# aniketntnu/WordDiffusion

Hardware: AMD Instinct MI355X
Metric: denoised 64x256 word images/sec (1000-step DDPM), whole job (higher is better)
Workload: dtype bf16x3; 1 GPU; BASELINE configs[1]: batch 64 per GPU of 64x256 crops = [64,4,8,32] latents, 1000-step DDPM (999 executed steps), base unet.py UNetModel (320 ch, mult (1,1), 4 heads, 339 writers), random-init synthetic weights; variant=base, batch_per_gpu=64, noise_steps=1000, executed_steps_per_image=999, precision=split-bf16 MFMA x3, fp32 accumulate (<=1e-4 of the fp32 reference), output_finite=True

## Files before the change

include/wdiff_hip.h:

```cpp
#ifndef WDIFF_HIP_H
#define WDIFF_HIP_H

#include <stdint.h>

#ifdef __cplusplus
extern "C" {
#endif

#define WD_OK 0
#define WD_EINVAL (-1)
#define WD_ELAUNCH (-2)
#define WD_ESTATE (-3)

#define WD_ACT_NONE 0
#define WD_ACT_SILU 1
#define WD_ACT_GEGLU 2

typedef uint16_t wd_bf16;

#define WD_MAX_KSPLIT 64

typedef struct wd_src {
    const wd_bf16* hi;
    const wd_bf16* lo;
    const int32_t* gather;
    int32_t ld;
    int32_t c;
    int32_t ntaps;
    int32_t hw_src;
} wd_src;

typedef struct wd_gemm_args {
    wd_src src[2];
    int32_t nsrc;
    int32_t npass;
    const wd_bf16* w_hi;
    const wd_bf16* w_lo;
    int32_t m, n, ktot;
    int32_t hw_out;
    const float* bias;
    const float* rowvec;
    int32_t rowvec_ld;
    const float* resid;
    int32_t resid_ld;
    const int64_t* resid_rows;
    int32_t act;
    float* out_f32;
    int32_t out_ld;
    wd_bf16* out_hi;
    wd_bf16* out_lo;
    int32_t out_pl_ld;
    int32_t tile;
    int32_t w_layout;
    int32_t slab_rows;
    int32_t ksplit;
    float* ws;
    int64_t ws_floats;
    double* stat_part;
    int32_t stat_cpg;
    int32_t dbg;
    int32_t* tickets;
    int32_t ntickets;
    const float* gn_gamma;
    const float* gn_beta;
    float gn_eps;
    int32_t gn_silu;
    int32_t gn_cpg;
    const float* a32;
    int32_t a32_ld;
    const double* a32_part;
    int32_t a32_nchunk;
    int32_t a32_pcpg;
    int32_t a32_cpg;
    const float* a32_gamma;
    const float* a32_beta;
    float a32_eps;
    int32_t a32_silu;
    const float* ln_gamma;
    const float* ln_beta;
    float ln_eps;
    int32_t w_ngroups;
    int64_t w_group_stride;
} wd_gemm_args;

int wd_gemm(const wd_gemm_args* args, void* stream);

int wd_gemm_check(const wd_gemm_args* args, wd_gemm_args* out);
const char* wd_gemm_check_kernel(const wd_gemm_args* args);

int wd_gemm_pack_w(const wd_bf16* hi, const wd_bf16* lo, int n, int ktot, wd_bf16* out_hi, wd_bf16* out_lo, void* stream);

typedef struct wd_ff_args {
    const wd_bf16* x_hi;
    const wd_bf16* x_lo;
    int32_t x_ld;
    int32_t m, c, inner;
    const wd_bf16* w1_hi;
    const wd_bf16* w1_lo;
    const float* b1;
    const wd_bf16* w2_hi;
    const wd_bf16* w2_lo;
    const float* b2;
    const float* resid;
    int32_t resid_ld;
    float* out_f32;
    int32_t out_ld;
    wd_bf16* out_hi;
    wd_bf16* out_lo;
    int32_t out_pl_ld;
    const wd_bf16* w3_hi;
    const wd_bf16* w3_lo;
    const float* b3;
    const float* resid3;
    int32_t resid3_ld;
    double* stat_part;
    int32_t stat_cpg;
    int32_t hw_out;
    int32_t npass;
    const float* x_in;
    int32_t x_in_ld;
    int32_t hw;
    const double* gn_part;
    int32_t gn_nchunk, gn_pcpg, gn_cpg;
    float gn_eps;
    const float* gn_gamma;
    const float* gn_beta;
    const wd_bf16* pi_hi;
    const wd_bf16* pi_lo;
    const float* pi_b;
    const float* ln2_gamma;
    const float* ln2_beta;
    const wd_bf16* mq_a;
    const wd_bf16* mot_a;
    const float* xb_a;
    const wd_bf16* mq_b;
    const wd_bf16* mot_b;
    const float* xb_b;
    const float* ln3_gamma;
    const float* ln3_beta;
    float ln_eps;
    int32_t heads, L;
    float* tok2;
} wd_ff_args;
int wd_ff_fused(const wd_ff_args* args, void* stream);
int wd_ff_supported(int c, int inner);
int wd_ff_args_bytes(void);

int wd_gemm_auto_ksplit(int m, int n, int ktot, int64_t ws_floats);
int wd_gemm_args_bytes(void);
int wd_gemm_experimental(void);

int wd_gn_nchunk(int hw);
int wd_gn_stats(const float* x, int ld, int batch, int hw, int c, int cpg, double* part, void* stream);
int wd_gn_fold_chunks(const double* part, int batch, int nchunk, int ngroups, double* out, void* stream);

int wd_gn_apply(const float* x, int ld, int batch, int hw, int c, int cpg, const double* part, int nchunk, int part_cpg,
                const float* gamma, const float* beta, float eps, int silu,
                wd_bf16* out_hi, wd_bf16* out_lo, int out_ld, int c_off,
                wd_bf16* raw_hi, wd_bf16* raw_lo, void* stream);

int wd_gn_apply2(const float* xa, int lda, int ca, const double* part_a, int nchunk_a, int part_cpg_a, int c_off_a,
                 const float* xb, int ldb, int cb, const double* part_b, int nchunk_b, int part_cpg_b, int c_off_b,
                 int batch, int hw, int cpg, const float* gamma, const float* beta, float eps, int silu,
                 wd_bf16* out_hi, wd_bf16* out_lo, int out_ld, wd_bf16* raw_hi, wd_bf16* raw_lo, const int32_t* perm_a, void* stream);

int wd_gn_conv3x3_few_supported(int c, int w, int oc);
int wd_gn_conv3x3_few(const float* x, int ld, int batch, int h, int w, int c, int cpg, const double* part, int nchunk, int part_cpg,
                      const float* gamma, const float* beta, float eps, int silu, const float* weight, const float* bias, int oc,
                      float* out, void* stream);

int wd_layernorm(const float* x, int ld, int rows, int c, const float* gamma, const float* beta, float eps,
                 wd_bf16* out_hi, wd_bf16* out_lo, int out_ld, void* stream);

int wd_split(const float* x, int ld, int rows, int c, int silu, wd_bf16* out_hi, wd_bf16* out_lo, int out_ld,
             void* stream);

int wd_attention(const float* q, int ldq, const float* k, int ldk, const float* v, int ldv,
                 int batch, int heads, int nq, int nk, int d, float scale,
                 float* out_f32, wd_bf16* out_hi, wd_bf16* out_lo, int out_ld, int out_rows, int out_row0,
                 void* stream);

int64_t wd_attention_packed_elems(int batch, int heads, int nk, int d);
int wd_attention_pack_kv(const float* k, int ldk, const float* v, int ldv, int batch, int heads, int nk, int d,
                         wd_bf16* img, void* stream);
int wd_attention_packed(const float* q, int ldq, const wd_bf16* img, int batch, int heads, int nq, int nk, int d,
                        float scale, float* out_f32, wd_bf16* out_hi, wd_bf16* out_lo, int out_ld, int out_rows,
                        int out_row0, void* stream);

int wd_timestep_embedding(const int64_t* t, int batch, const float* freqs, int half,
                          wd_bf16* out_hi, wd_bf16* out_lo, int out_ld, void* stream);

int wd_xattn_supported(int c, int heads, int L);
int wd_xattn_fold(const float* k, int ldk, const float* v, int ldv, int batch, int heads, int L, int d, float scale,
                  const float* wq, const float* wo, int c, float* mq, float* mo, wd_bf16* mq_pl, wd_bf16* mot_pl, void* stream);
int wd_xattn_fused(const float* x, int ld, int batch, int hw, int c, const float* gamma, const float* beta, float eps,
                   const float* mq, const float* mo, int heads, int L, const float* bias, float* out, int out_ld,
                   const float* gamma2, const float* beta2, float eps2, wd_bf16* n_hi, wd_bf16* n_lo, int n_ld,
                   const wd_bf16* mq_pl, const wd_bf16* mot_pl, void* stream);

int wd_emb_combine(const float* time, const float* label, const int64_t* y, int num_classes, int T, int B, int ted,
                   wd_bf16* out_hi, wd_bf16* out_lo, int out_ld, void* stream);
int wd_select_rows(const float* table, const int32_t* t_dev, int batch, int64_t row_floats, int chunk, float* out,
                   void* stream);

int wd_emb_combine_mix(const float* time, const float* label, const int32_t* pairs, const float* mix, int num_classes, int T, int B,
                       int ted, wd_bf16* out_hi, wd_bf16* out_lo, int out_ld, void* stream);
int wd_label_mix(const float* label, const int32_t* pairs, const float* mix, int num_classes, int B, int ted, float* out,
                 void* stream);

int wd_xattn_pair(const float* x, int ld, int batch, int hw, int c, float eps, int heads, int L, const float* gamma_a,
                  const float* beta_a, const wd_bf16* mq_pl_a, const wd_bf16* mot_pl_a, const float* bias_a, const float* gamma_b,
                  const float* beta_b, const wd_bf16* mq_pl_b, const wd_bf16* mot_pl_b, const float* bias_b, float* out, int out_ld,
                  const float* gamma2, const float* beta2, float eps2, wd_bf16* n_hi, wd_bf16* n_lo, int n_ld, void* stream);

int wd_embed_tokens(const void* ids, int ids_are_i64, int rows, int seq_len, const float* table, int vocab, int c,
                    const float* pe, wd_bf16* out_hi, wd_bf16* out_lo, int out_ld, void* stream);

int wd_im2col3x3(const float* x, int batch, int cin, int h, int w, wd_bf16* out_hi, wd_bf16* out_lo, int kpad,
                 void* stream);

int wd_conv3x3_in_supported(int cin, int h, int w, int cout);
int wd_conv3x3_in_nchunk(int hw);
int wd_conv3x3_in(const float* x, int batch, int cin, int h, int w, const float* weight, const float* bias, int cout, float* out,
                  int ld, double* part, int stat_cpg, void* stream);

int wd_nchw_to_tokens(const float* x, int batch, int c, int hw, float* out, int ld, void* stream);
int wd_tokens_to_nchw(const float* x, int ld, int batch, int c, int hw, float* out, void* stream);

int wd_ddpm_step(float* x, const float* eps, int batch, int n_per_sample, const float* ca, const float* cb,
                 const float* cs, const int32_t* t_dev, const float* noise, uint64_t seed, uint64_t sample_offset,
                 void* stream);

int wd_ddpm_step_cfg(float* x, const float* first, const float* second, float scale, float* eps_out, int batch, int n_per_sample,
                     const float* ca, const float* cb, const float* cs, const int32_t* t_dev, const float* noise, uint64_t seed,
                     uint64_t sample_offset, void* stream);

int wd_advance_timestep(int32_t* t_dev, int delta, int64_t* t64, int batch, void* stream);

int wd_ddim_step(float* x, const float* eps, const float* second, float scale, float* eps_out, int batch, int n_per_sample,
                 const float* c1, const float* c2, const float* c3, const float* c4, const float* c5, const int32_t* k_dev,
                 const int32_t* t_dev, const float* noise, uint64_t seed, uint64_t sample_offset, void* stream);

int wd_next_timestep(int32_t* k_dev, const int32_t* tau, int S, int32_t* t_dev, int64_t* t64, int batch, void* stream);

int wd_randn(float* out, int batch, int n_per_sample, uint64_t seed, uint64_t sample_offset, uint32_t stream_id,
             void* stream);

#define WD_VAE_MAX_LATENT 8
#define WD_STREAM_VAE_POSTERIOR 3
#define WD_STREAM_DROPOUT0 0x100
int wd_vae_posterior(const float* moments_tok, int ld, const float* w, const float* bias, int batch, int L, int hw, float* mean,
                     float* logvar, float* sample, float scale, const float* noise, uint64_t seed, uint64_t sample_offset,
                     void* stream);

int wd_posterior_sample(const float* mean, const float* logvar, int batch, int n_per_sample, float* sample, float scale,
                        const float* noise, uint64_t seed, uint64_t sample_offset, void* stream);

int wd_noise_images(const float* x, const float* eps, const int64_t* t, const float* sqrt_ah, const float* sqrt_1m_ah,
                    int batch, int n_per_sample, float* out, void* stream);

int wd_copy2d(void* dst, int64_t dst_pitch, const void* src, int64_t src_pitch, int64_t width_bytes, int64_t rows,
              void* stream);

int wd_ema_update(float* ema, const float* p, int64_t n, double beta, void* stream);

int wd_adamw_table_entry_bytes(void);
int wd_adamw_chunk(void);
int wd_adamw_multi(const void* table, int ntensor, int64_t total_chunks, double lr, double beta1, double beta2, double eps,
                   double weight_decay, int64_t step, int ema_mode, double ema_beta, void* stream);

int wd_repack_entry_bytes(void);
int wd_repack_tile(void);
int wd_repack_vchunk(void);
int wd_repack_multi(const void* table, int nentries, int64_t total_chunks, void* stream);

int wd_mse_loss(const float* pred, const float* target, int64_t n, float* grad, float* loss, double* scratch,
                int scratch_len, void* stream);


int wd_transpose_planes(const void* in_hi, const void* in_lo, int in_is_f32, int ld, int c, const int32_t* gather, int ntaps,
                        int hw_out, int hw_src, int m, int mpad, int tap_minor, wd_bf16* out_hi, wd_bf16* out_lo,
                        void* stream);

typedef struct wd_dw_item {
    const wd_bf16* d_hi;
    const wd_bf16* d_lo;
    const wd_bf16* x_hi;
    const wd_bf16* x_lo;
    float* grad;
    int32_t d_ld, x_ld, grad_ld, accumulate;
} wd_dw_item;
typedef struct wd_dw_args {
    const wd_bf16* d_hi;
    const wd_bf16* d_lo;
    const wd_bf16* x_hi;
    const wd_bf16* x_lo;
    const int32_t* gather;
    float* grad;
    float* ws;
    int64_t ws_floats;
    int32_t d_ld, x_ld, grad_ld;
    int32_t ntaps, hw_out, hw_src;
    int32_t m, n, c;
    int32_t npass;
    int32_t accumulate;
    int32_t nslice;
    int32_t dbg;
    int32_t reserved;
    void* stamps;
    const wd_dw_item* items;
    int32_t nitems;
    int32_t reserved2;
} wd_dw_args;
int wd_dw(const wd_dw_args* a, void* stream);
int wd_dw_group(const wd_dw_args* a, const wd_dw_item* items_host, const wd_dw_item* items_dev, int nitems, void* stream);
int wd_dw_group_slices(int m, int n, int c, int ntaps, int nitems);
int wd_dw_item_bytes(void);
int wd_dw_supported(int m, int n, int c, int ntaps, int hw_out);
int wd_dw_slices(int m, int n, int c, int ntaps);
int wd_dw_args_bytes(void);

int wd_colsum(const float* x, int ld, int rows, int c, int seg, float* out, int out_ld, int accumulate, float scale,
              float* scratch, int64_t scratch_floats, void* stream);

int wd_gn_bwd_nchunk(int hw);
int wd_gn_bwd_stats(const float* x, int ld, const float* dz, int dz_ld, int dz_off, int batch, int hw, int c, int cpg,
                    const double* part, int nchunk_f, int part_cpg, const float* gamma, const float* beta, int c_off, float eps,
                    int silu, float* sums, void* stream);
int wd_gn_bwd_apply(const float* x, int ld, const float* dz, int dz_ld, int dz_off, int batch, int hw, int c, int cpg,
                    const double* part, int nchunk_f, int part_cpg, const float* gamma, const float* beta, int c_off, float eps,
                    int silu, const float* sums, float* dx, int dx_ld, int accumulate, void* stream);

int wd_gn_bwd_fused_supported(int hw, int c, int cpg);
int wd_gn_bwd_fused(const float* x, int ld, const float* dz, int dz_ld, int dz_off, int batch, int hw, int c, int cpg,
                    const double* part, int nchunk_f, int part_cpg, const float* gamma, const float* beta, int c_off, float eps,
                    int silu, float* sums, float* dx, int dx_ld, int accumulate, void* stream);

typedef struct {
    uint64_t seed;
    uint64_t row_base;
    const uint64_t* row_base_dev;
    uint32_t tag, thr;
    float scale;
} wd_dropout;
int wd_gn_apply_dropout(const float* x, int ld, int batch, int hw, int c, int cpg, const double* part, int nchunk, int part_cpg,
                        const float* gamma, const float* beta, float eps, int silu,
                        wd_bf16* out_hi, wd_bf16* out_lo, int out_ld, int c_off,
                        wd_bf16* raw_hi, wd_bf16* raw_lo, const wd_dropout* d, void* stream);
int wd_gn_bwd_stats_dropout(const float* x, int ld, const float* dz, int dz_ld, int dz_off, int batch, int hw, int c, int cpg,
                            const double* part, int nchunk_f, int part_cpg, const float* gamma, const float* beta, int c_off, float eps,
                            int silu, float* sums, const wd_dropout* d, void* stream);
int wd_gn_bwd_apply_dropout(const float* x, int ld, const float* dz, int dz_ld, int dz_off, int batch, int hw, int c, int cpg,
                            const double* part, int nchunk_f, int part_cpg, const float* gamma, const float* beta, int c_off, float eps,
                            int silu, const float* sums, float* dx, int dx_ld, int accumulate, const wd_dropout* d, void* stream);
int wd_gn_bwd_fused_dropout(const float* x, int ld, const float* dz, int dz_ld, int dz_off, int batch, int hw, int c, int cpg,
                            const double* part, int nchunk_f, int part_cpg, const float* gamma, const float* beta, int c_off, float eps,
                            int silu, float* sums, float* dx, int dx_ld, int accumulate, const wd_dropout* d, void* stream);

int wd_layernorm_bwd_nblk(int rows);
int wd_layernorm_bwd(const float* x, int ld, const float* dy, int dy_ld, int rows, int c, const float* gamma, float eps,
                     float* dx, int dx_ld, int accumulate, float* colpart, void* stream);

int wd_attention_bwd_small_nwg(int heads, int nq, int nk, int d);
int wd_attention_bwd_small(const float* q, int ldq, const float* k, int ldk, const float* v, int ldv, const float* dout,
                           int ldo, int batch, int heads, int nq, int nk, int d, float scale, float* dq, int lddq,
                           float* dkv_part, int* nwg_out, void* stream);

int wd_dout_prep_rows(void);
int wd_dout_prep(const float* d, int ld, int m, int n, int npad, int mpad, wd_bf16* pl_hi, wd_bf16* pl_lo, wd_bf16* t_hi,
                 wd_bf16* t_lo, float* colpart, void* stream);
int wd_dout_prep_geglu(const float* u, int u_ld, const float* dh, int dh_ld, int m, int inner, int mpad, wd_bf16* pl_hi, wd_bf16* pl_lo,
                       wd_bf16* t_hi, wd_bf16* t_lo, float* colpart, void* stream);
int wd_colsum_finish(const float* part, int nblk, int c, int nseg, float* out, int out_ld, int accumulate, float scale,
                     void* stream);
int wd_colsum_entry_bytes(void);
int wd_colsum_finish_multi(const void* table, int n, int max_c, void* stream);

int64_t wd_attention_bwd_scratch_floats(int batch, int heads, int nq, int nk);
int wd_attention_bwd(const float* q, int ldq, const float* k, int ldk, const float* v, int ldv, const float* dout, int ldo,
                     int batch, int heads, int nq, int nk, int d, float scale, float* dq, int lddq, float* dk, int lddk,
                     float* dv, int lddv, float* scratch, int64_t scratch_floats, void* stream);

int wd_add(float* dst, const float* src, int64_t n, void* stream);

int wd_permute_dw(const float* packed, int ld, int n, int c, int ntaps, float* out, void* stream);
// ... 27 lines not shown
```

worddiffusion_amd/_native.py:

```python
from __future__ import annotations

import ctypes as C
import os
import re

_HERE = os.path.dirname(os.path.abspath(__file__))
LIB_PATH = os.environ.get("WDIFF_LIB") or os.path.join(_HERE, "libwdiff_hip.so")
HEADER_PATH = os.path.join(os.path.dirname(_HERE), "include", "wdiff_hip.h")

WD_OK, WD_EINVAL, WD_ELAUNCH, WD_ESTATE = 0, -1, -2, -3
ACT_NONE, ACT_SILU, ACT_GEGLU = 0, 1, 2
VAE_MAX_LATENT, STREAM_VAE_POSTERIOR = 8, 3
NCLASS = 13
CLASS_NAMES = ("gemm", "gn_stats", "gn_apply", "layernorm", "attention", "other", "gemm_other_tiles", "gemm_splitk_reduce",
               "gemm_two_per_cu", "gemm_weights_to_registers", "feed_forward_fused", "weight_gradient", "gemm_small_maps_whole_k")

_vp = C.c_void_p
_i = C.c_int
_f = C.c_float
_u64 = C.c_uint64


class WdSrc(C.Structure):
    _fields_ = [("hi", _vp), ("lo", _vp), ("gather", _vp), ("ld", C.c_int32), ("c", C.c_int32),
                ("ntaps", C.c_int32), ("hw_src", C.c_int32)]


class WdGemmArgs(C.Structure):
    _fields_ = [("src", WdSrc * 2), ("nsrc", C.c_int32), ("npass", C.c_int32), ("w_hi", _vp), ("w_lo", _vp),
                ("m", C.c_int32), ("n", C.c_int32), ("ktot", C.c_int32), ("hw_out", C.c_int32),
                ("bias", _vp), ("rowvec", _vp), ("rowvec_ld", C.c_int32), ("resid", _vp), ("resid_ld", C.c_int32),
                ("resid_rows", _vp), ("act", C.c_int32), ("out_f32", _vp), ("out_ld", C.c_int32),
                ("out_hi", _vp), ("out_lo", _vp), ("out_pl_ld", C.c_int32), ("tile", C.c_int32),
                ("w_layout", C.c_int32), ("slab_rows", C.c_int32), ("ksplit", C.c_int32), ("ws", _vp),
                ("ws_floats", C.c_int64), ("stat_part", _vp), ("stat_cpg", C.c_int32), ("dbg", C.c_int32),
                ("tickets", _vp), ("ntickets", C.c_int32), ("gn_gamma", _vp), ("gn_beta", _vp), ("gn_eps", C.c_float),
                ("gn_silu", C.c_int32), ("gn_cpg", C.c_int32), ("a32", _vp), ("a32_ld", C.c_int32), ("a32_part", _vp),
                ("a32_nchunk", C.c_int32), ("a32_pcpg", C.c_int32), ("a32_cpg", C.c_int32), ("a32_gamma", _vp), ("a32_beta", _vp),
                ("a32_eps", C.c_float), ("a32_silu", C.c_int32), ("ln_gamma", _vp), ("ln_beta", _vp), ("ln_eps", C.c_float),
                ("w_ngroups", C.c_int32), ("w_group_stride", C.c_int64)]


class WdFfArgs(C.Structure):
    _fields_ = [("x_hi", _vp), ("x_lo", _vp), ("x_ld", C.c_int32), ("m", C.c_int32), ("c", C.c_int32), ("inner", C.c_int32),
                ("w1_hi", _vp), ("w1_lo", _vp), ("b1", _vp), ("w2_hi", _vp), ("w2_lo", _vp), ("b2", _vp), ("resid", _vp),
                ("resid_ld", C.c_int32), ("out_f32", _vp), ("out_ld", C.c_int32), ("out_hi", _vp), ("out_lo", _vp),
                ("out_pl_ld", C.c_int32), ("w3_hi", _vp), ("w3_lo", _vp), ("b3", _vp), ("resid3", _vp), ("resid3_ld", C.c_int32),
                ("stat_part", _vp), ("stat_cpg", C.c_int32), ("hw_out", C.c_int32), ("npass", C.c_int32),
                ("x_in", _vp), ("x_in_ld", C.c_int32), ("hw", C.c_int32), ("gn_part", _vp), ("gn_nchunk", C.c_int32),
                ("gn_pcpg", C.c_int32), ("gn_cpg", C.c_int32), ("gn_eps", C.c_float), ("gn_gamma", _vp), ("gn_beta", _vp),
                ("pi_hi", _vp), ("pi_lo", _vp), ("pi_b", _vp), ("ln2_gamma", _vp), ("ln2_beta", _vp), ("mq_a", _vp), ("mot_a", _vp),
                ("xb_a", _vp), ("mq_b", _vp), ("mot_b", _vp), ("xb_b", _vp), ("ln3_gamma", _vp), ("ln3_beta", _vp),
                ("ln_eps", C.c_float), ("heads", C.c_int32), ("L", C.c_int32), ("tok2", _vp)]


class WdDwArgs(C.Structure):
    _fields_ = [("d_hi", _vp), ("d_lo", _vp), ("x_hi", _vp), ("x_lo", _vp), ("gather", _vp), ("grad", _vp), ("ws", _vp),
                ("ws_floats", C.c_int64), ("d_ld", C.c_int32), ("x_ld", C.c_int32), ("grad_ld", C.c_int32), ("ntaps", C.c_int32),
                ("hw_out", C.c_int32), ("hw_src", C.c_int32), ("m", C.c_int32), ("n", C.c_int32), ("c", C.c_int32),
                ("npass", C.c_int32), ("accumulate", C.c_int32), ("nslice", C.c_int32), ("dbg", C.c_int32), ("reserved", C.c_int32),
                ("stamps", _vp), ("items", _vp), ("nitems", C.c_int32), ("reserved2", C.c_int32)]


class WdDwItem(C.Structure):
    _fields_ = [("d_hi", _vp), ("d_lo", _vp), ("x_hi", _vp), ("x_lo", _vp), ("grad", _vp), ("d_ld", C.c_int32), ("x_ld", C.c_int32),
                ("grad_ld", C.c_int32), ("accumulate", C.c_int32)]


_SIGS = {
    "wd_gemm": (_i, [C.POINTER(WdGemmArgs), _vp]),
    "wd_gemm_check": (_i, [C.POINTER(WdGemmArgs), C.POINTER(WdGemmArgs)]),
    "wd_gemm_check_kernel": (C.c_char_p, [C.POINTER(WdGemmArgs)]),
    "wd_dw": (_i, [C.POINTER(WdDwArgs), _vp]),
    "wd_dw_supported": (_i, [_i, _i, _i, _i, _i]),
    "wd_dw_slices": (_i, [_i, _i, _i, _i]),
    "wd_dw_args_bytes": (_i, []),
    "wd_dw_group": (_i, [C.POINTER(WdDwArgs), _vp, _vp, _i, _vp]),
    "wd_dw_group_slices": (_i, [_i, _i, _i, _i, _i]),
    "wd_dw_item_bytes": (_i, []),
    "wd_gemm_auto_ksplit": (_i, [_i, _i, _i, C.c_int64]),
    "wd_gemm_pack_w": (_i, [_vp, _vp, _i, _i, _vp, _vp, _vp]),
    "wd_ff_fused": (_i, [C.POINTER(WdFfArgs), _vp]),
    "wd_ff_supported": (_i, [_i, _i]),
    "wd_ff_args_bytes": (_i, []),
    "wd_gemm_args_bytes": (_i, []),
    "wd_gemm_experimental": (_i, []),
    "wd_gn_nchunk": (_i, [_i]),
    "wd_gn_stats": (_i, [_vp, _i, _i, _i, _i, _i, _vp, _vp]),
    "wd_gn_fold_chunks": (_i, [_vp, _i, _i, _i, _vp, _vp]),
    "wd_gn_conv3x3_few_supported": (_i, [_i, _i, _i]),
    "wd_gn_conv3x3_few": (_i, [_vp, _i, _i, _i, _i, _i, _i, _vp, _i, _i, _vp, _vp, _f, _i, _vp, _vp, _i, _vp, _vp]),
    "wd_gn_apply": (_i, [_vp, _i, _i, _i, _i, _i, _vp, _i, _i, _vp, _vp, _f, _i, _vp, _vp, _i, _i, _vp, _vp, _vp]),
    "wd_gn_apply_dropout": (_i, [_vp, _i, _i, _i, _i, _i, _vp, _i, _i, _vp, _vp, _f, _i, _vp, _vp, _i, _i, _vp, _vp, _vp, _vp]),
    "wd_gn_apply2": (_i, [_vp, _i, _i, _vp, _i, _i, _i, _vp, _i, _i, _vp, _i, _i, _i, _i, _i, _i, _vp, _vp, _f, _i, _vp, _vp, _i, _vp,
                          _vp, _vp, _vp]),
    "wd_layernorm": (_i, [_vp, _i, _i, _i, _vp, _vp, _f, _vp, _vp, _i, _vp]),
    "wd_split": (_i, [_vp, _i, _i, _i, _i, _vp, _vp, _i, _vp]),
    "wd_attention": (_i, [_vp, _i, _vp, _i, _vp, _i, _i, _i, _i, _i, _i, _f, _vp, _vp, _vp, _i, _i, _i, _vp]),
    "wd_attention_packed_elems": (C.c_int64, [_i, _i, _i, _i]),
    "wd_attention_pack_kv": (_i, [_vp, _i, _vp, _i, _i, _i, _i, _i, _vp, _vp]),
    "wd_attention_packed": (_i, [_vp, _i, _vp, _i, _i, _i, _i, _i, _f, _vp, _vp, _vp, _i, _i, _i, _vp]),
    "wd_timestep_embedding": (_i, [_vp, _i, _vp, _i, _vp, _vp, _i, _vp]),
    "wd_embed_tokens": (_i, [_vp, _i, _i, _i, _vp, _i, _i, _vp, _vp, _vp, _i, _vp]),
    "wd_im2col3x3": (_i, [_vp, _i, _i, _i, _i, _vp, _vp, _i, _vp]),
    "wd_conv3x3_in_supported": (_i, [_i, _i, _i, _i]),
    "wd_conv3x3_in_nchunk": (_i, [_i]),
    "wd_conv3x3_in": (_i, [_vp, _i, _i, _i, _i, _vp, _vp, _i, _vp, _i, _vp, _i, _vp]),
    "wd_nchw_to_tokens": (_i, [_vp, _i, _i, _i, _vp, _i, _vp]),
    "wd_tokens_to_nchw": (_i, [_vp, _i, _i, _i, _i, _vp, _vp]),
    "wd_ddpm_step": (_i, [_vp, _vp, _i, _i, _vp, _vp, _vp, _vp, _vp, _u64, _u64, _vp]),
    "wd_advance_timestep": (_i, [_vp, _i, _vp, _i, _vp]),
    "wd_randn": (_i, [_vp, _i, _i, _u64, _u64, C.c_uint32, _vp]),
    "wd_vae_posterior": (_i, [_vp, _i, _vp, _vp, _i, _i, _i, _vp, _vp, _vp, _f, _vp, _u64, _u64, _vp]),
    "wd_posterior_sample": (_i, [_vp, _vp, _i, _i, _vp, _f, _vp, _u64, _u64, _vp]),
    "wd_noise_images": (_i, [_vp, _vp, _vp, _vp, _vp, _i, _i, _vp, _vp]),
    "wd_copy2d": (_i, [_vp, C.c_int64, _vp, C.c_int64, C.c_int64, C.c_int64, _vp]),
    "wd_ema_update": (_i, [_vp, _vp, C.c_int64, C.c_double, _vp]),
    "wd_adamw_table_entry_bytes": (_i, []),
    "wd_adamw_chunk": (_i, []),
    "wd_adamw_multi": (_i, [_vp, _i, C.c_int64, C.c_double, C.c_double, C.c_double, C.c_double, C.c_double, C.c_int64, _i,
                           C.c_double, _vp]),
    "wd_mse_loss": (_i, [_vp, _vp, C.c_int64, _vp, _vp, _vp, _i, _vp]),
    "wd_transpose_planes": (_i, [_vp, _vp, _i, _i, _i, _vp, _i, _i, _i, _i, _i, _i, _vp, _vp, _vp]),
    "wd_repack_entry_bytes": (_i, []),
    "wd_repack_tile": (_i, []),
    "wd_repack_vchunk": (_i, []),
    "wd_repack_multi": (_i, [_vp, _i, C.c_int64, _vp]),
    "wd_attention_bwd_scratch_floats": (C.c_int64, [_i, _i, _i, _i]),
    "wd_attention_bwd": (_i, [_vp, _i, _vp, _i, _vp, _i, _vp, _i, _i, _i, _i, _i, _i, _f, _vp, _i, _vp, _i, _vp, _i, _vp, C.c_int64, _vp]),
    "wd_xattn_supported": (_i, [_i, _i, _i]),
    "wd_xattn_fold": (_i, [_vp, _i, _vp, _i, _i, _i, _i, _i, _f, _vp, _vp, _i, _vp, _vp, _vp, _vp, _vp]),
    "wd_xattn_fused": (_i, [_vp, _i, _i, _i, _i, _vp, _vp, _f, _vp, _vp, _i, _i, _vp, _vp, _i, _vp, _vp, _f, _vp, _vp, _i, _vp, _vp, _vp]),
    "wd_dout_prep_rows": (_i, []),
    "wd_dout_prep": (_i, [_vp, _i, _i, _i, _i, _i, _vp, _vp, _vp, _vp, _vp, _vp]),
    "wd_dout_prep_geglu": (_i, [_vp, _i, _vp, _i, _i, _i, _i, _vp, _vp, _vp, _vp, _vp, _vp]),
    "wd_colsum_finish": (_i, [_vp, _i, _i, _i, _vp, _i, _i, _f, _vp]),
    "wd_colsum_entry_bytes": (_i, []),
    "wd_colsum_finish_multi": (_i, [_vp, _i, _i, _vp]),
    "wd_emb_combine": (_i, [_vp, _vp, _vp, _i, _i, _i, _i, _vp, _vp, _i, _vp]),
    "wd_select_rows": (_i, [_vp, _vp, _i, C.c_int64, _i, _vp, _vp]),
    "wd_emb_combine_mix": (_i, [_vp, _vp, _vp, _vp, _i, _i, _i, _i, _vp, _vp, _i, _vp]),
    "wd_label_mix": (_i, [_vp, _vp, _vp, _i, _i, _i, _vp, _vp]),
    "wd_ddpm_step_cfg": (_i, [_vp, _vp, _vp, _f, _vp, _i, _i, _vp, _vp, _vp, _vp, _vp, _u64, _u64, _vp]),
    "wd_ddim_step": (_i, [_vp, _vp, _vp, _f, _vp, _i, _i, _vp, _vp, _vp, _vp, _vp, _vp, _vp, _vp, _u64, _u64, _vp]),
    "wd_next_timestep": (_i, [_vp, _vp, _i, _vp, _vp, _i, _vp]),
    "wd_xattn_pair": (_i, [_vp, _i, _i, _i, _i, _f, _i, _i, _vp, _vp, _vp, _vp, _vp, _vp, _vp, _vp, _vp, _vp, _vp, _i, _vp, _vp, _f,
                           _vp, _vp, _i, _vp]),
    "wd_add": (_i, [_vp, _vp, C.c_int64, _vp]),
    "wd_permute_dw": (_i, [_vp, _i, _i, _i, _i, _vp, _vp]),
    "wd_colsum": (_i, [_vp, _i, _i, _i, _i, _vp, _i, _i, _f, _vp, C.c_int64, _vp]),
    "wd_gn_bwd_nchunk": (_i, [_i]),
    "wd_gn_bwd_stats": (_i, [_vp, _i, _vp, _i, _i, _i, _i, _i, _i, _vp, _i, _i, _vp, _vp, _i, _f, _i, _vp, _vp]),
    "wd_gn_bwd_apply": (_i, [_vp, _i, _vp, _i, _i, _i, _i, _i, _i, _vp, _i, _i, _vp, _vp, _i, _f, _i, _vp, _vp, _i, _i, _vp]),
    "wd_gn_bwd_fused_supported": (_i, [_i, _i, _i]),
    "wd_gn_bwd_fused": (_i, [_vp, _i, _vp, _i, _i, _i, _i, _i, _i, _vp, _i, _i, _vp, _vp, _i, _f, _i, _vp, _vp, _i, _i, _vp]),
    "wd_gn_bwd_stats_dropout": (_i, [_vp, _i, _vp, _i, _i, _i, _i, _i, _i, _vp, _i, _i, _vp, _vp, _i, _f, _i, _vp, _vp, _vp]),
    "wd_gn_bwd_apply_dropout": (_i, [_vp, _i, _vp, _i, _i, _i, _i, _i, _i, _vp, _i, _i, _vp, _vp, _i, _f, _i, _vp, _vp, _i, _i, _vp, _vp]),
    "wd_gn_bwd_fused_dropout": (_i, [_vp, _i, _vp, _i, _i, _i, _i, _i, _i, _vp, _i, _i, _vp, _vp, _i, _f, _i, _vp, _vp, _i, _i, _vp, _vp]),
    "wd_layernorm_bwd_nblk": (_i, [_i]),
    "wd_layernorm_bwd": (_i, [_vp, _i, _vp, _i, _i, _i, _vp, _f, _vp, _i, _i, _vp, _vp]),
    "wd_attention_bwd_small_nwg": (_i, [_i, _i, _i, _i]),
    "wd_attention_bwd_small": (_i, [_vp, _i, _vp, _i, _vp, _i, _vp, _i, _i, _i, _i, _i, _i, _f, _vp, _i, _vp,
                                   C.POINTER(_i), _vp]),
    "wd_geglu_fwd": (_i, [_vp, _i, C.c_int64, _i, _vp, _vp, _i, _vp]),
    "wd_geglu_bwd": (_i, [_vp, _i, _vp, _i, C.c_int64, _i, _vp, _i, _vp]),
    "wd_silu_bwd": (_i, [_vp, _vp, C.c_int64, _vp, _vp]),
    "wd_pool2x2_sum": (_i, [_vp, _i, _i, _i, _i, _vp, _vp]),
    "wd_embedding_bwd": (_i, [_vp, _i, _i, _vp, _i, _i, _i, _vp, _i, _vp]),
    "wd_graph_begin": (_i, [_vp]),
    "wd_graph_end": (_i, [_vp, C.POINTER(_vp)]),
    "wd_graph_launch": (_i, [_vp, _vp]),
    "wd_graph_destroy": (_i, [_vp]),
    "wd_prof_enable": (_i, [_i]),
    "wd_prof_collect": (_i, [C.POINTER(C.c_double), C.POINTER(C.c_int64), C.POINTER(C.c_double)]),
    "wd_prof_collect_flops": (_i, [C.POINTER(C.c_double), C.POINTER(C.c_int64), C.POINTER(C.c_double)]),
    "wd_version": (C.c_char_p, []),
    "wd_device_info": (_i, [C.POINTER(_i), C.POINTER(_i), C.c_char_p, _i]),
}


def header_symbols() -> list:
    txt = open(HEADER_PATH).read()
    txt = re.sub(r"/\*.*?\*/", "", txt, flags=re.S)
    return sorted(set(re.findall(r"\b(wd_[a-z0-9_]+)\s*\(", txt)))


class NativeError(RuntimeError):
    pass


_lib = None


def lib() -> C.CDLL:
    global _lib
    if _lib is not None:
        return _lib
    if not os.path.exists(LIB_PATH):
        raise NativeError(f"{LIB_PATH} is missing: build it with `python -m worddiffusion_amd.build` "
                          "(hipcc --offload-arch=gfx950); worddiffusion_amd has no CPU/eager fallback")
    l = C.CDLL(LIB_PATH)
    for name, (res, args) in _SIGS.items():
        fn = getattr(l, name)
        fn.restype = res
        fn.argtypes = args
    if l.wd_gemm_args_bytes() != C.sizeof(WdGemmArgs):
        raise NativeError(f"{LIB_PATH}: wd_gemm_args is {l.wd_gemm_args_bytes()} bytes in the library, {C.sizeof(WdGemmArgs)} in "
                          "worddiffusion_amd/_native.py - rebuild with `python -m worddiffusion_amd.build`")
    if l.wd_ff_args_bytes() != C.sizeof(WdFfArgs):
        raise NativeError(f"{LIB_PATH}: wd_ff_args is {l.wd_ff_args_bytes()} bytes in the library, {C.sizeof(WdFfArgs)} in "
                          "worddiffusion_amd/_native.py - rebuild with `python -m worddiffusion_amd.build`")
    if l.wd_dw_item_bytes() != C.sizeof(WdDwItem):
        raise NativeError(f"{LIB_PATH}: wd_dw_item is {l.wd_dw_item_bytes()} bytes in the library, {C.sizeof(WdDwItem)} in "
                          "worddiffusion_amd/_native.py - rebuild with `python -m worddiffusion_amd.build`")
    if l.wd_dw_args_bytes() != C.sizeof(WdDwArgs):
        raise NativeError(f"{LIB_PATH}: wd_dw_args is {l.wd_dw_args_bytes()} bytes in the library, {C.sizeof(WdDwArgs)} in "
                          "worddiffusion_amd/_native.py - rebuild with `python -m worddiffusion_amd.build`")
    _lib = l
    return l


_ERR = {WD_EINVAL: "invalid argument", WD_ELAUNCH: "HIP launch/runtime error", WD_ESTATE: "bad call order"}


def check(rc: int, what: str) -> None:
    if rc != WD_OK:
        raise NativeError(f"{what} failed: {_ERR.get(rc, rc)}")
```

worddiffusion_amd/csrc/wd_gemm.hip:

```cpp
#include <stdlib.h>

#include "wd_common.h"
#include "wd_gemm_epi.h"
#include "wd_gemm_priv.h"


namespace {

constexpr int BK = 32;

__device__ __forceinline__ int lds_off(int row, int ch) { return row * 64 + ((ch ^ ((row >> 2) & 3)) << 4); }
__device__ __forceinline__ int lds_off16(int row, int ch) { return row * 64 + ((ch ^ ((0 - (row >> 2)) & 3)) << 4); }


template <int BM, int BN, int TN, int NT>
__device__ __forceinline__ void wd_epilogue_lds(const wd_gemm_args& a, const f32x16 (&acc)[TN], char* smem, const int m0,
                                                const int n0, const int wm, const int wn, const int wcols, const int kh,
                                                const int nkh, const int tid, const int sidx = 0) {
    constexpr int LDE = BN + 4;
    float* ep = reinterpret_cast<float*>(smem);
    const int lane = tid & 63;
    const int frow = lane & 31, fhalf = lane >> 5;
    asm volatile("s_waitcnt vmcnt(0)" ::: "memory");
    __syncthreads();
// ... 1739 lines not shown
    const int r0w = (cw >> 1) * 32, c0w = (cw & 1) * 80;

    if (wave >= 8) {
        const int L = wave - 8;
        const int lrow = lane >> 2, lpos = lane & 3;
        const int sw = (lpos ^ ((0 - (lane >> 4)) & 3)) * 8;
        auto make_srd = [](const wd_bf16* p) {
            return __builtin_amdgcn_make_buffer_rsrc(const_cast<wd_bf16*>(p), 0, 0x7FFFFFF0, 0x00020000);
        };
        const int x_piece = NPL == 2 ? 8 + (L >> 1) : 8 + (L & 1), x_plane = NPL == 2 ? (L & 1) : 0;
        uint32_t b_voff[3];
        {
            const int pcs[3] = {L, L + 4, x_piece};
#pragma unroll
            for (int i = 0; i < 3; ++i) {
                const int n = n0 + pcs[i] * 16 + lrow;
                b_voff[i] = n < a.n ? (uint32_t)(((long)n * a.ktot + sw) * 2) : WD_OOB;
            }
        }
        const __amdgpu_buffer_rsrc_t srd_w_hi = make_srd(a.w_hi), srd_w_lo = make_srd(a.w_lo ? a.w_lo : a.w_hi);
        const __amdgpu_buffer_rsrc_t srd_w_x = (x_plane ? srd_w_lo : srd_w_hi);
        int s = 0, tap = 0, kc = 0;
        int cur_ld = a.src[0].ld, cur_cpt = a.src[0].c / BKS, cur_nt = a.src[0].ntaps;
        const wd_bf16* cur_hi = a.src[0].hi;
        const wd_bf16* cur_lo = a.src[0].lo;
        {
            const int cpt = a.src[0].c / BKS, n0st = a.src[0].ntaps * cpt;
            if (k_begin < n0st) {
                tap = k_begin / cpt;
                kc = k_begin - tap * cpt;
            } else {
                s = 1;
                kc = k_begin - n0st;
                cur_hi = a.src[1].hi;
                cur_lo = a.src[1].lo;
                cur_ld = a.src[1].ld;
                cur_cpt = a.src[1].c / BKS;
                cur_nt = a.src[1].ntaps;
            }
        }
        __amdgpu_buffer_rsrc_t srd_a_hi = make_srd(cur_hi), srd_a_lo = make_srd(cur_lo ? cur_lo : cur_hi);
        uint32_t a_voff[2];
        auto locate = [&]() {
#pragma unroll
            for (int i = 0; i < 2; ++i) {
                const int row = (2 * L + i) * 16 + lrow;
                int r;
                if (s == 0) r = s_tab[tap * BM + row];
                else r = (m0 + row < a.m) ? m0 + row : -1;
                a_voff[i] = r >= 0 ? (uint32_t)r * (uint32_t)(cur_ld * 2) + (uint32_t)(sw * 2) : WD_OOB;
            }
        };
        locate();
        int soff_a = kc * BKS * 2, soff_b = k_begin * BKS * 2;
        int wr_off = 0;
        auto issue_stage = [&]() {
            char* sbase = smem + wr_off;
#pragma unroll
            for (int i = 0; i < 2; ++i) {
                __builtin_amdgcn_raw_ptr_buffer_load_lds(srd_a_hi, (wd_lds_ptr)(sbase + (2 * L + i) * 1024), 16, a_voff[i], soff_a, 0, 0);
                if (NPL == 2)
                    __builtin_amdgcn_raw_ptr_buffer_load_lds(srd_a_lo, (wd_lds_ptr)(sbase + A_PL + (2 * L + i) * 1024), 16, a_voff[i],
                                                             soff_a, 0, 0);
            }
#pragma unroll
            for (int i = 0; i < 2; ++i) {
                __builtin_amdgcn_raw_ptr_buffer_load_lds(srd_w_hi, (wd_lds_ptr)(sbase + NPL * A_PL + (L + 4 * i) * 1024), 16, b_voff[i],
                                                         soff_b, 0, 0);
                if (NPL == 2)
                    __builtin_amdgcn_raw_ptr_buffer_load_lds(srd_w_lo, (wd_lds_ptr)(sbase + NPL * A_PL + B_PL + (L + 4 * i) * 1024), 16,
                                                             b_voff[i], soff_b, 0, 0);
            }
            __builtin_amdgcn_raw_ptr_buffer_load_lds(srd_w_x, (wd_lds_ptr)(sbase + NPL * A_PL + x_plane * B_PL + x_piece * 1024), 16,
                                                     b_voff[2], soff_b, 0, 0);
            soff_b += BKS * 2;
            soff_a += BKS * 2;
            wr_off += STAGE;
            if (wr_off == RING) wr_off = 0;
            ++kc;
            if (kc == cur_cpt) {
                kc = 0;
                soff_a = 0;
                ++tap;
                if (tap == cur_nt) {
                    tap = 0;
                    ++s;
                    if (s < a.nsrc) {
                        cur_hi = a.src[1].hi;
                        cur_lo = a.src[1].lo;
                        cur_ld = a.src[1].ld;
                        cur_cpt = a.src[1].c / BKS;
                        cur_nt = a.src[1].ntaps;
                        srd_a_hi = make_srd(cur_hi);
                        srd_a_lo = make_srd(cur_lo ? cur_lo : cur_hi);
                    }
                }
                if (s < a.nsrc) locate();
            }
        };
        auto wait_keep1 = [&]() {
            if (NPL == 2) asm volatile("s_waitcnt vmcnt(9)" ::: "memory");
            else asm volatile("s_waitcnt vmcnt(5)" ::: "memory");
        };
        __builtin_amdgcn_s_setprio(2);
        int issued = 0;
        for (; issued < 3 && issued < nk; ++issued) issue_stage();
        if (nk > 0) {
            if (issued >= 2) {
                if (issued == 3) {
                    if (NPL == 2) asm volatile("s_waitcnt vmcnt(18)" ::: "memory");
                    else asm volatile("s_waitcnt vmcnt(10)" ::: "memory");
                } else {
                    wait_keep1();
                }
            } else {
                asm volatile("s_waitcnt vmcnt(0)" ::: "memory");
            }
            __builtin_amdgcn_s_barrier();
        }
        int kit = 0;
        for (; kit + 3 < nk; ++kit) {
            wait_keep1();
            __builtin_amdgcn_s_barrier();
            issue_stage();
        }
        for (; kit < nk; ++kit) {
            if (kit + 1 < nk) {
                if (kit + 2 < nk) wait_keep1();
                else asm volatile("s_waitcnt vmcnt(0)" ::: "memory");
            }
            __builtin_amdgcn_s_barrier();
        }
    } else {
        const int ao0 = lds_off16(r0w + l15, lq), bo0 = NPL * A_PL + lds_off16(c0w + l15, lq);
        bf16x8 fa0[2][NPL], fb0[5][NPL], fa1[2][NPL], fb1[5][NPL];
        auto read_a = [&](auto& fa_, const char* base, int i) {
#pragma unroll
            for (int p = 0; p < NPL; ++p) fa_[i][p] = *reinterpret_cast<const bf16x8*>(base + ao0 + p * A_PL + i * 1024);
        };
        auto read_b = [&](auto& fb_, const char* base, int t) {
#pragma unroll
            for (int p = 0; p < NPL; ++p) fb_[t][p] = *reinterpret_cast<const bf16x8*>(base + bo0 + p * B_PL + t * 1024);
        };
        auto mfma_pass = [&](auto& fa_, auto& fb_, int pass, int g) {
            const int i = g / 5, t = g % 5;
            if (NPL == 2) {
                if (pass == 0) acc[i][t] = __builtin_amdgcn_mfma_f32_16x16x32_bf16(fa_[i][NPL - 1], fb_[t][0], acc[i][t], 0, 0, 0);
                else if (pass == 1) acc[i][t] = __builtin_amdgcn_mfma_f32_16x16x32_bf16(fa_[i][0], fb_[t][NPL - 1], acc[i][t], 0, 0, 0);
                else acc[i][t] = __builtin_amdgcn_mfma_f32_16x16x32_bf16(fa_[i][0], fb_[t][0], acc[i][t], 0, 0, 0);
            } else {
                if (pass == 2) acc[i][t] = __builtin_amdgcn_mfma_f32_16x16x32_bf16(fa_[i][0], fb_[t][0], acc[i][t], 0, 0, 0);
            }
        };
        if (nk > 0) {
            __builtin_amdgcn_s_barrier();
#pragma unroll
            for (int i = 0; i < 2; ++i) read_a(fa0, smem, i);
#pragma unroll
            for (int t = 0; t < 5; ++t) read_b(fb0, smem, t);
        }
        int rd_off = STAGE;
        auto step = [&](bool have1, auto& ma, auto& mb, auto& ra, auto& rb) {
            __builtin_amdgcn_s_barrier();
            const char* nb = smem + rd_off;
#pragma unroll
            for (int pass = (NPL == 2 ? 0 : 2); pass < 3; ++pass) {
#pragma unroll
                for (int g = 0; g < 10; ++g) {
                    if (have1 && pass == (NPL == 2 ? 0 : 2)) {
                        if (g < 2) read_a(ra, nb, g);
                        else if (g < 7) read_b(rb, nb, g - 2);
                    }
                    mfma_pass(ma, mb, pass, g);
                }
                __builtin_amdgcn_sched_barrier(0);
            }
            rd_off += STAGE;
            if (rd_off == RING) rd_off = 0;
        };
        for (int kit = 0; kit < nk; kit += 2) {
            step(kit + 1 < nk, fa0, fb0, fa1, fb1);
            if (kit + 1 < nk) step(kit + 2 < nk, fa1, fb1, fa0, fb0);
        }
    }

    constexpr int LDE = BN + 4;
    float* ep = reinterpret_cast<float*>(smem);
    asm volatile("s_waitcnt vmcnt(0)" ::: "memory");
    __syncthreads();
    if (wave < 8) {
#pragma unroll
        for (int i = 0; i < 2; ++i)
#pragma unroll
            for (int t = 0; t < 5; ++t)
#pragma unroll
                for (int r = 0; r < 4; ++r) ep[(r0w + i * 16 + 4 * lq + r) * LDE + c0w + t * 16 + l15] = acc[i][t][r];
    }
    __syncthreads();
    wd_epilogue_tail<BM, BN, 768>(a, ep, m0, n0, tid, sidx);
#endif
}

template <int NPASS>
int launch8(const wd_gemm_args& a, hipStream_t st) {
    constexpr int NPL = (NPASS == 1) ? 1 : 2;
    constexpr int loop_smem = 4 * NPL * (128 + 160) * 64 + 9 * 128 * 4;
    constexpr int red_smem = 128 * (160 + 4) * 4 + WD_STAT_SCRATCH;
    constexpr int smem = loop_smem > red_smem ? loop_smem : red_smem;
    static_assert(smem <= 160 * 1024, "LDS budget");
    static bool attr_done = false;
    if (!attr_done) {
        if (hipFuncSetAttribute(reinterpret_cast<const void*>(&wd_gemm8_kernel<NPASS>), hipFuncAttributeMaxDynamicSharedMemorySize,
                                smem) != hipSuccess)
            return WD_ELAUNCH;
        attr_done = true;
    }
    const int nbn = (a.n + 159) / 160, nbm = (a.m + 127) / 128;
    {
        WdLaunchScope scope(WD_CLS_GEMM, st, 2.0 * (double)a.m * (double)a.n * (double)a.ktot);
        hipLaunchKernelGGL((wd_gemm8_kernel<NPASS>), dim3(nbn * nbm * a.ksplit), dim3(768), smem, st, a, nbn, nbm);
    }
    if (a.ksplit > 1) return launch_reduce_any<128, 160>(a, st);
    return wd_check_launch();
}

#endif

}

int wd_gemm_launch_reduce(const wd_gemm_args& a, hipStream_t st, int bm) {
    if (bm == 64) {
        if (reduce_flat_ok(a)) return launch_reduce_any<64, 64>(a, st);
        const int cpg = a.stat_part ? a.stat_cpg : 1;
        if (40 % cpg == 0 && a.n % 40 == 0) return launch_reduce<64, 40>(a, st);
        if (32 % cpg == 0 && a.n % 32 == 0) return launch_reduce<64, 32>(a, st);
        return launch_reduce<64, 64>(a, st);
    }
    return launch_reduce_any<128, 160>(a, st);
}

static int wd_auto_ksplit(const int tile, const int m, const int n, const int nk64, const long ws_floats) {
    const int bn = tile % 1000, bm = tile / 1000;
    const long tiles = (long)((m + bm - 1) / bm) * ((n + bn - 1) / bn);
    if (!((tiles < 128 || (tiles == 128 && nk64 >= 32)) && nk64 >= 8)) return 1;
    long sp = 256 / tiles;
    if (sp > nk64 / 4) sp = nk64 / 4;
    static const long cap_env = getenv("WDIFF_KSPLIT_CAP") ? atol(getenv("WDIFF_KSPLIT_CAP")) : WD_MAX_KSPLIT;
    const long cap = nk64 >= 64 ? cap_env : 8;
    if (sp > cap) sp = cap;
    while (sp > 1 && sp * m * n > ws_floats) --sp;
    return sp > 1 ? (int)sp : 1;
}

static int wd_auto_tile(const int m, const int n, const int nk64, const bool can_split_base, const long ws_floats) {
    int tile = (n % 160 == 0) ? 128160 : 128064;
    const long tiles = (long)((m + 127) / 128) * ((n + (tile % 1000) - 1) / (tile % 1000));
    const bool can_split = can_split_base && nk64 >= 8 && (long)2 * m * n <= ws_floats;
    if (tiles < 128 && !can_split && m > 64) tile = 64064;
    return tile;
}

extern "C" int wd_gemm_experimental(void) {
#ifdef WDIFF_EXPERIMENTAL
    return 1;
#else
    return 0;
#endif
}

extern "C" int wd_gemm_args_bytes(void) { return (int)sizeof(wd_gemm_args); }

extern "C" int wd_gemm_auto_ksplit(int m, int n, int ktot, int64_t ws_floats) {
    if (m <= 0 || n <= 0 || ktot <= 0 || ktot % BK2 || ws_floats <= 0) return 1;
    const int nk64 = ktot / BK2;
    return wd_auto_ksplit(wd_auto_tile(m, n, nk64, true, (long)ws_floats), m, n, nk64, (long)ws_floats);
}

namespace {
enum WdKernel {
    K_GEMMQ,
    K_GEMMW,
    K_V4,
    K_M16,
    K_V2,
    K_V1,
    K_SLAB,
    K_CONV3,
    K_V8,
    K_PP,
};

struct WdResolved {
    wd_gemm_args a;
    WdKernel kernel;
    int ks;
};
}

static int wd_gemm_resolve(const wd_gemm_args& in, WdResolved& r) {
    wd_gemm_args a = in;
    static const int ks_env = getenv("WDIFF_GEMM_KS") ? atoi(getenv("WDIFF_GEMM_KS")) : 2;
    r.ks = ks_env == 1 ? 1 : 2;
    if (a.ksplit < 0 || a.ksplit > WD_MAX_KSPLIT) return WD_EINVAL;
    if (a.w_layout == 3) {
        if (a.n % 80 || a.act == WD_ACT_GEGLU || (a.tile && a.tile != 64320 && a.tile != 128160 && a.tile != 64080) || a.ktot % 64)
            return WD_EINVAL;
        if (a.tile == 0) a.tile = (a.a32 || a.ln_gamma) ? 64320 : 128160;
        if (a.n % (a.tile % 1000)) return WD_EINVAL;
        if (a.tile == 64080) a.ksplit = 1;
    }
    if (a.w_ngroups > 1) {
        if (a.w_layout != 3 || a.tile != 64320 || a.ksplit > 1 || a.hw_out % (64 * a.w_ngroups) || a.w_group_stride <= 0 || (a.w_group_stride & 7))
            return WD_EINVAL;
        a.ksplit = 1;
    }
    if (a.stat_part) {
        if (a.stat_cpg <= 0 || a.n % a.stat_cpg || a.act == WD_ACT_GEGLU) return WD_EINVAL;
        const int bn = (a.tile ? a.tile % 1000 : (a.n % 160 == 0 ? 160 : 64));
        const int bm = (a.tile ? a.tile / 1000 : 128);
        if (!((a.hw_out % bm == 0) || (bm % a.hw_out == 0 && bm / a.hw_out <= WD_STAT_MAXNS))) return WD_EINVAL;
        if ((bm != 128 && a.w_layout != 3) || bn % a.stat_cpg) return WD_EINVAL;
        if (!wd_epilogue_vec_ok(a)) return WD_EINVAL;
        if (a.tile == 0) a.tile = bm * 1000 + bn;
    }
    if (a.ksplit > 1 && (!a.ws || a.act == WD_ACT_GEGLU || a.w_layout == 1)) return WD_EINVAL;
    if (a.ln_gamma) {
        if (a.w_layout != 3 || (a.tile && a.tile != 64320) || a.n != 320 || a.ksplit > 1 || !a.ln_beta || !a.out_hi || (a.out_pl_ld & 3) ||
            ((reinterpret_cast<uintptr_t>(a.ln_gamma) | reinterpret_cast<uintptr_t>(a.ln_beta)) & 15) ||
            ((reinterpret_cast<uintptr_t>(a.out_hi) | reinterpret_cast<uintptr_t>(a.out_lo)) & 7) || a.act == WD_ACT_GEGLU)
            return WD_EINVAL;
        a.tile = 64320;
        a.ksplit = 1;
    }
    if (a.gn_gamma) {
        if (!a.gn_beta || !a.stat_part || !a.out_hi || (!a.ws && a.tile != 64080) || a.hw_out != 64 || a.m % 64 || a.n % 160 || a.gn_cpg <= 0 ||
            40 % a.gn_cpg || a.stat_cpg <= 0 || a.gn_cpg % a.stat_cpg || a.act != WD_ACT_NONE || a.resid_rows || a.w_layout == 1)
            return WD_EINVAL;
        if (!wd_epilogue_vec_ok(a) ||
            ((reinterpret_cast<uintptr_t>(a.ws) | reinterpret_cast<uintptr_t>(a.gn_gamma) | reinterpret_cast<uintptr_t>(a.gn_beta)) & 15))
            return WD_EINVAL;
        a.tickets = nullptr;
    }
    if (a.w_layout == 1) {
        a.ksplit = 1;
        a.tickets = nullptr;
    }
    if (a.nsrc < 1 || a.nsrc > 2 || (a.npass != 1 && a.npass != 3)) return WD_EINVAL;
    if (a.m <= 0 || a.n <= 0 || a.hw_out <= 0 || !a.w_hi || (a.npass == 3 && !a.w_lo)) return WD_EINVAL;
    if (!a.out_f32 && !a.out_hi) return WD_EINVAL;
    long k = 0;
    for (int s = 0; s < a.nsrc; ++s) {
        const wd_src& q = a.src[s];
        if (s == 0 && a.a32) {
            if (a.w_layout != 3 || a.npass != 3 || (a.tile && a.tile != 64320) || a.n % 320 || a.hw_out % 64 || !a.a32_part || !a.a32_gamma ||
                !a.a32_beta || a.a32_nchunk <= 0 || a.a32_pcpg <= 0 || a.a32_cpg <= 0 || a.a32_cpg % a.a32_pcpg || q.c % a.a32_cpg ||
                q.c > 1024 || a.a32_ld < q.c || (a.a32_ld & 3) || (reinterpret_cast<uintptr_t>(a.a32) & 15) || q.hw_src <= 0)
                return WD_EINVAL;
        } else if (!q.hi || (a.npass == 3 && !q.lo)) return WD_EINVAL;
        if (q.c <= 0 || q.c % BK || q.ld % 8 || q.ntaps < 1) return WD_EINVAL;
        if (!q.gather && q.ntaps != 1) return WD_EINVAL;
        if (q.gather && q.hw_src <= 0) return WD_EINVAL;
        k += (long)q.ntaps * q.c;
    }
    if (k != a.ktot) return WD_EINVAL;
    {
        const long lim = 0x7FFFFFF0L;
        if ((long)a.n * a.ktot * 2 >= lim) return WD_EINVAL;
        for (int s = 0; s < a.nsrc; ++s) {
            const wd_src& q = a.src[s];
            const long rows = q.gather ? (long)((a.m + a.hw_out - 1) / a.hw_out) * q.hw_src : (long)a.m;
            if ((s == 0 && a.a32) ? rows * a.a32_ld * 4 >= lim : rows * q.ld * 2 >= lim) return WD_EINVAL;
        }
    }
    if (a.act == WD_ACT_GEGLU && (a.n % 64 || a.tile == 0)) return WD_EINVAL;
    if (a.rowvec && a.rowvec_ld <= 0) return WD_EINVAL;
    if (a.resid && a.resid_ld <= 0) return WD_EINVAL;
    {
        const int nout = a.act == WD_ACT_GEGLU ? a.n / 2 : a.n;
        if ((a.out_f32 && a.out_ld < nout) || (a.out_hi && a.out_pl_ld < nout) || (a.resid && a.resid_ld < nout) ||
            (a.rowvec && a.rowvec_ld < nout))
            return WD_EINVAL;
        for (int s = 0; s < a.nsrc; ++s)
            if (!(s == 0 && a.a32) && a.src[s].ld < a.src[s].c) return WD_EINVAL;
    }

    if (a.w_layout == 3) {
        bool ok = a.src[0].ntaps <= 9 && (a.nsrc == 1 || (a.src[1].gather == nullptr && a.src[1].ntaps == 1));
        for (int s = 0; s < a.nsrc; ++s) ok = ok && (a.src[s].c % 64 == 0);
        if (!ok) return WD_EINVAL;
        const wd_src& q0 = a.src[0];
        const bool same3 = q0.ntaps == 9 && q0.gather && a.slab_rows > 0 && q0.hw_src == a.hw_out && a.hw_out % a.slab_rows == 0;
        const bool down3 = a.tile == 64080 && q0.ntaps == 9 && q0.gather && a.slab_rows > 0 && q0.hw_src == 4 * a.hw_out;
        if (!same3 && !down3) a.slab_rows = 0;
        a.tickets = nullptr;
        if (a.tile == 64080) {
            if (!wd_gemmq_applies(a)) return WD_EINVAL;
            if (a.gn_gamma && (40 % a.gn_cpg || 80 % a.gn_cpg)) return WD_EINVAL;
            r.a = a, r.kernel = K_GEMMQ;
            return WD_OK;
        }
        const int nk64 = a.ktot / 64;
        if (a.ksplit == 0) a.ksplit = a.ws ? wd_auto_ksplit(a.tile, a.m, a.n, nk64, a.ws_floats) : 1;
        if (a.ksplit > 1 && (nk64 < a.ksplit || (long)a.ksplit * a.m * a.n > a.ws_floats)) a.ksplit = 1;
        if (a.gn_gamma && a.ksplit <= 1) return WD_EINVAL;
        r.a = a, r.kernel = K_GEMMW;
        return WD_OK;
    }
#ifndef WDIFF_EXPERIMENTAL
    if (a.w_layout == 1) return WD_EINVAL;
#else
    if (a.w_layout == 1) {
        if (a.src[0].ntaps > 9 || a.slab_rows <= 0) return WD_EINVAL;
        if (a.nsrc == 2 && (a.src[1].gather || a.src[1].ntaps != 1)) return WD_EINVAL;
        if (a.tile == 0) a.tile = (a.act == WD_ACT_GEGLU || a.n % 160) ? 128064 : 128160;
        if (a.act == WD_ACT_GEGLU && a.n % (a.tile % 1000)) return WD_EINVAL;
        if (a.slab_rows > 192) return WD_EINVAL;
        if (a.tile != 128064 && a.tile != 128128 && a.tile != 128160) return WD_EINVAL;
        r.a = a, r.kernel = K_SLAB;
        return WD_OK;
    }
#endif
    bool conv3 = false;
    if (a.w_layout == 2) {
        const wd_src& q0 = a.src[0];
        static const int conv3_mode = getenv("WDIFF_CONV3") ? atoi(getenv("WDIFF_CONV3")) : 0;
#ifdef WDIFF_EXPERIMENTAL
        const bool conv3_env = conv3_mode != 0 || (a.dbg & 0x1000);
#else
        const bool conv3_env = false;
        (void)conv3_mode;
#endif
        const bool same3 = q0.ntaps == 9 && q0.gather && a.slab_rows > 0 && q0.hw_src == a.hw_out && a.hw_out % a.slab_rows == 0;
        conv3 = conv3_env && same3 && q0.c % 64 == 0 && a.act != WD_ACT_GEGLU && (a.tile == 0 || a.tile == 128160) &&
                (a.nsrc == 1 || (!a.src[1].gather && a.src[1].ntaps == 1 && a.src[1].c % 64 == 0));
        if (conv3) a.tile = 128160;
        a.w_layout = 0;
        static const bool arith_env = getenv("WDIFF_GEMM_ARITH_TAB") ? atoi(getenv("WDIFF_GEMM_ARITH_TAB")) != 0 : true;
        if (!same3 || !arith_env) a.slab_rows = 0;
    } else if (a.w_layout == 0) {
        a.slab_rows = 0;
    } else if (a.w_layout != 0) {
        return WD_EINVAL;
    }
    bool v2ok = (a.ktot % BK2 == 0) && !getenv("WDIFF_GEMM_V1");
    for (int s = 0; s < a.nsrc; ++s) v2ok = v2ok && (a.src[s].c % BK2 == 0);
    v2ok = v2ok && a.src[0].ntaps <= 9 && (a.nsrc == 1 || (a.src[1].gather == nullptr && a.src[1].ntaps == 1));
    const int nk64 = a.ktot / BK2;
    int tile = a.tile;
    if (tile == 0)
        tile = wd_auto_tile(a.m, a.n, nk64, v2ok && a.ws && a.ksplit == 0 && a.act != WD_ACT_GEGLU, a.ws_floats);
    if (a.ksplit == 0) {
        a.ksplit = (v2ok && a.ws && a.act != WD_ACT_GEGLU) ? wd_auto_ksplit(tile, a.m, a.n, nk64, a.ws_floats) : 1;
    }
    if (a.act == WD_ACT_GEGLU && a.n % (tile % 1000)) return WD_EINVAL;
    if (a.ksplit > 1 && (!v2ok || nk64 < a.ksplit || (long)a.ksplit * a.m * a.n > a.ws_floats)) a.ksplit = 1;
    bool use_v4 = false;
    if (tile == 128160) {
        static const int v4_env = getenv("WDIFF_GEMM_V4") ? atoi(getenv("WDIFF_GEMM_V4")) : 2;
        const long wgs = (long)((a.m + 127) / 128) * ((a.n + 159) / 160) * a.ksplit;
        use_v4 = v2ok && !a.stat_part && (v4_env == 1 || (v4_env == 2 && wgs >= 512) || (a.dbg & 0x400));
    }
    {
        static const bool fuse_env = getenv("WDIFF_GEMM_FUSE_COMBINE") ? atoi(getenv("WDIFF_GEMM_FUSE_COMBINE")) != 0 : false;
        const int bn = tile % 1000, bm = tile / 1000;
        const long ntile = (long)((a.m + bm - 1) / bm) * ((a.n + bn - 1) / bn);
        const bool aligned = (a.n & 3) == 0 && a.n % bn == 0 && wd_epilogue_vec_ok(a) && (reinterpret_cast<uintptr_t>(a.ws) & 15) == 0;
        if (!((fuse_env || (a.dbg & 0x2000)) && a.tickets && a.ksplit > 1 && v2ok && !use_v4 && !conv3 && aligned && ntile <= a.ntickets))
            a.tickets = nullptr;
    }
    if (a.gn_gamma && !(a.ksplit > 1 && tile == 128160 && v2ok && !use_v4 && !conv3)) return WD_EINVAL;
    static const int stagger_min = getenv("WDIFF_GEMM_STAGGER_MIN") ? atoi(getenv("WDIFF_GEMM_STAGGER_MIN")) : 10;
    static const bool stagger = getenv("WDIFF_GEMM_STAGGER") ? atoi(getenv("WDIFF_GEMM_STAGGER")) != 0 : true;
    static const bool m16 = getenv("WDIFF_GEMM_M16") ? atoi(getenv("WDIFF_GEMM_M16")) != 0 : true;
    static const bool pp = getenv("WDIFF_GEMM_PP") ? atoi(getenv("WDIFF_GEMM_PP")) != 0 : false;
    a.tile = tile;
#ifdef WDIFF_EXPERIMENTAL
    if (conv3 && v2ok) return r.a = a, r.kernel = K_CONV3, WD_OK;
#endif
    if (tile != 128064 && tile != 128160 && tile != 128128 && tile != 64064) return WD_EINVAL;
    if (tile == 128160) {
        if (use_v4) return r.a = a, r.kernel = K_V4, WD_OK;
#ifdef WDIFF_EXPERIMENTAL
        static const int v8_env = getenv("WDIFF_GEMM_V8") ? atoi(getenv("WDIFF_GEMM_V8")) : 0;
        bool v8ok = a.ktot % 32 == 0 && a.src[0].ntaps <= 9 && !a.stat_part && !a.gn_gamma && a.act != WD_ACT_GEGLU &&
                    (a.nsrc == 1 || (a.src[1].gather == nullptr && a.src[1].ntaps == 1));
        for (int s8 = 0; s8 < a.nsrc; ++s8) v8ok = v8ok && (a.src[s8].c % 32 == 0);
        if (v8ok && (v8_env == 1 || (a.dbg & 0x80000))) {
            if (a.ksplit > 1 && (a.ktot / 32 < a.ksplit || (long)a.ksplit * a.m * a.n > a.ws_floats)) a.ksplit = 1;
            a.tickets = nullptr;
            return r.a = a, r.kernel = K_V8, WD_OK;
        }
#endif
        if (v2ok && r.ks == 2 && m16 && stagger && nk64 / a.ksplit >= stagger_min) a.dbg |= 0x200;
        if (v2ok && r.ks == 2 && m16) return r.a = a, r.kernel = K_M16, WD_OK;
    }
#ifdef WDIFF_EXPERIMENTAL
    if (v2ok && r.ks == 2 && pp) return r.a = a, r.kernel = K_PP, WD_OK;
#else
    (void)pp;
#endif
    if (v2ok) return r.a = a, r.kernel = K_V2, WD_OK;
    a.ksplit = 1;
    a.tickets = nullptr;
    r.a = a, r.kernel = K_V1;
    return WD_OK;
}

extern "C" int wd_gemm_check(const wd_gemm_args* in, wd_gemm_args* out) {
    if (!in) return WD_EINVAL;
    WdResolved r;
    const int rc = wd_gemm_resolve(*in, r);
    if (rc == WD_OK && out) *out = r.a;
    return rc;
}

extern "C" const char* wd_gemm_check_kernel(const wd_gemm_args* in) {
    if (!in) return nullptr;
    WdResolved r;
    if (wd_gemm_resolve(*in, r) != WD_OK) return nullptr;
    switch (r.kernel) {
        case K_GEMMQ: return "K_GEMMQ";
        case K_GEMMW: return "K_GEMMW";
        case K_V4: return "K_V4";
        case K_M16: return "K_M16";
        case K_V2: return "K_V2";
        case K_V1: return "K_V1";
        case K_SLAB: return "K_SLAB";
        case K_CONV3: return "K_CONV3";
        case K_V8: return "K_V8";
        case K_PP: return "K_PP";
    }
    return nullptr;
}

extern "C" int wd_gemm(const wd_gemm_args* pa, void* stream) {
    if (!pa) return WD_EINVAL;
    WdResolved r;
    const int rc = wd_gemm_resolve(*pa, r);
    if (rc != WD_OK) return rc;
    const wd_gemm_args& a = r.a;
    const bool p3 = a.npass == 3;
    hipStream_t st = reinterpret_cast<hipStream_t>(stream);
    if (r.kernel == K_GEMMQ) return wd_gemmq_launch(a, st);
    if (r.kernel == K_GEMMW) return wd_gemmw_launch(a, st);
#ifdef WDIFF_EXPERIMENTAL
    if (r.kernel == K_SLAB) {
#define WD_DISPATCH3(BM_, BN_)                                                                                   \
    if (r.ks == 1) return p3 ? launch3<BM_, BN_, 3, 192, 1>(a, st) : launch3<BM_, BN_, 1, 192, 1>(a, st); \
    return p3 ? launch3<BM_, BN_, 3, 192, 2>(a, st) : launch3<BM_, BN_, 1, 192, 2>(a, st)
        switch (a.tile) {
            case 128064: WD_DISPATCH3(128, 64);
            case 128128: WD_DISPATCH3(128, 128);
            case 128160: WD_DISPATCH3(128, 160);
            default: return WD_EINVAL;
        }
#undef WD_DISPATCH3
    }
    if (r.kernel == K_CONV3) return p3 ? launch_conv3<3>(a, st) : launch_conv3<1>(a, st);
#define WD_DISPATCH_PP(BM_, BN_) \
    if (r.kernel == K_PP) return p3 ? launch2<BM_, BN_, 3, 2, true>(a, st) : launch2<BM_, BN_, 1, 2, true>(a, st);
#else
#define WD_DISPATCH_PP(BM_, BN_)
#endif
#define WD_DISPATCH(BM_, BN_)                                                                       \
    WD_DISPATCH_PP(BM_, BN_)                                                                        \
    if (r.kernel == K_V2 && r.ks == 2) return p3 ? launch2<BM_, BN_, 3, 2>(a, st) : launch2<BM_, BN_, 1, 2>(a, st); \
    if (r.kernel == K_V2) return p3 ? launch2<BM_, BN_, 3, 1>(a, st) : launch2<BM_, BN_, 1, 1>(a, st);             \
    return p3 ? launch<BM_, BN_, 3>(a, st) : launch<BM_, BN_, 1>(a, st)
    switch (a.tile) {
        case 128064: WD_DISPATCH(128, 64);
        case 128160:
            if (r.kernel == K_V4) return p3 ? launch4<3>(a, st) : launch4<1>(a, st);
#ifdef WDIFF_EXPERIMENTAL
            if (r.kernel == K_V8) return p3 ? launch8<3>(a, st) : launch8<1>(a, st);
#endif
            if (r.kernel == K_M16) return p3 ? launch2<128, 160, 3, 2, false, true>(a, st) : launch2<128, 160, 1, 2, false, true>(a, st);
            WD_DISPATCH(128, 160);
        case 128128: WD_DISPATCH(128, 128);
        case 64064: WD_DISPATCH(64, 64);
        default: return WD_EINVAL;
    }
#undef WD_DISPATCH
#undef WD_DISPATCH_PP
}
```

worddiffusion_amd/csrc/wd_gemmq.hip:

```cpp
#include "wd_gemm_epi.h"
#include "wd_gemm_priv.h"

namespace {

constexpr int QNT = 512;
constexpr int QBM = 64, QBN = 80;
constexpr int QLDE = QBN + 4;
constexpr uint32_t Q_OOB = 0x80000000u;

typedef __attribute__((ext_vector_type(4))) unsigned q_u32x4;

__device__ __forceinline__ int q_lds_off(int row, int ch) { return row * 128 + ((ch ^ ((row >> 1) & 7)) << 4); }

__global__ void __launch_bounds__(QNT, 1) wd_gemmq_kernel(const wd_gemm_args a, const int nbn, const int nbm, const int nchp) {
#if defined(__HIP_DEVICE_COMPILE__)
    extern __shared__ __attribute__((aligned(16))) char smem[];
    const int ntile = nbn * nbm;
    int wg;
    {
        const int bid = blockIdx.x;
        const int q = ntile >> 3, r = ntile & 7, xcd = bid & 7, loc = bid >> 3;
        wg = (xcd < r ? xcd * (q + 1) : r * (q + 1) + (xcd - r) * q) + loc;
    }
    const int bn_i = wg % nbn, bm_i = wg / nbn;
    const int m0 = bm_i * QBM, n0 = bn_i * QBN;
    const int tid = threadIdx.x;
    const int lane = tid & 63;
    const int wave = __builtin_amdgcn_readfirstlane(tid >> 6);
    const int l15 = lane & 15, lq = lane >> 4;

    const int W = a.src[0].ntaps == 9 ? a.slab_rows : 0;
    const int wsh = W ? __builtin_ctz(W) : 0;
    const int ST = (W && a.src[0].hw_src == 4 * a.hw_out) ? 2 : 1;
    const int Ws = W * ST, wss = wsh + ST - 1;
    const int Hs = W ? (a.hw_out >> wsh) * ST : 0;
    const int TR = W ? QBM >> wsh : 0;
    const int NR = W ? (TR - 1) * ST + 3 : 0;
    const int SW = Ws + 2;
    const int bsm = m0 / a.hw_out;
    const int y0 = W ? (m0 - bsm * a.hw_out) >> wsh : 0;

    auto make_srd = [](const void* p) {
        return __builtin_amdgcn_make_buffer_rsrc(const_cast<void*>(p), 0, 0x7FFFFFF0, 0x00020000);
    };
    const __amdgpu_buffer_rsrc_t srd_w_hi = make_srd(a.w_hi), srd_w_lo = make_srd(a.w_lo);

    const int nct = a.n >> 4;
    const uint32_t b_voff = (uint32_t)((n0 >> 4) * 1024 + lane * 16);
    const uint32_t kstep_bytes = (uint32_t)nct * 1024u;
    auto load_b = [&](bf16x8 (&fb)[5][2], const int kabs, const bool live) {
        const uint32_t so = live ? (uint32_t)kabs * kstep_bytes : 0u;
        const uint32_t vo = live ? b_voff : Q_OOB;
#pragma unroll
        for (int t = 0; t < 5; ++t)
#pragma unroll
            for (int p = 0; p < 2; ++p)
                fb[t][p] = __builtin_bit_cast(bf16x8, __builtin_amdgcn_raw_buffer_load_b128(p ? srd_w_lo : srd_w_hi, vo + t * 1024, so, 0));
    };
    f32x4 acc[4][5];
#pragma unroll
    for (int i = 0; i < 4; ++i)
#pragma unroll
        for (int t = 0; t < 5; ++t)
#pragma unroll
            for (int r = 0; r < 4; ++r) acc[i][t][r] = 0.0f;
    auto mfma_step = [&](const char* base, const int cpl, const int (&rb)[4], const int shift0, const int lm, const int half,
                         const bf16x8 (&fb)[5][2], const int skip) {
        const int ach = half * 4 + lq;
        const int shift = shift0 + lm * l15 - l15;
        bf16x8 xa[2][2];
        {
            const int ao = q_lds_off(rb[0] + shift + l15, ach);
            xa[0][0] = *reinterpret_cast<const bf16x8*>(base + ao);
            xa[0][1] = *reinterpret_cast<const bf16x8*>(base + cpl + ao);
        }
#pragma unroll
        for (int i = 0; i < 4; ++i) {
            if (i < 3) {
                const int ao = q_lds_off(rb[i + 1] + shift + l15, ach);
                xa[(i + 1) & 1][0] = *reinterpret_cast<const bf16x8*>(base + ao);
                xa[(i + 1) & 1][1] = *reinterpret_cast<const bf16x8*>(base + cpl + ao);
            }
            if (skip & (1 << i)) continue;
#pragma unroll
            for (int t = 0; t < 5; ++t) {
                acc[i][t] = __builtin_amdgcn_mfma_f32_16x16x32_bf16(xa[i & 1][1], fb[t][0], acc[i][t], 0, 0, 0);
                acc[i][t] = __builtin_amdgcn_mfma_f32_16x16x32_bf16(xa[i & 1][0], fb[t][1], acc[i][t], 0, 0, 0);
                acc[i][t] = __builtin_amdgcn_mfma_f32_16x16x32_bf16(xa[i & 1][0], fb[t][0], acc[i][t], 0, 0, 0);
            }
        }
    };
#ifdef WD_Q_STAMPS
    unsigned long long* qst = (a.dbg & 0x100) && a.ws && blockIdx.x == 0 ? reinterpret_cast<unsigned long long*>(a.ws) + wave * 8 : nullptr;
#define Q_STAMP(i) if (qst && lane == 0) qst[i] = __builtin_amdgcn_s_memtime()
#else
#define Q_STAMP(i)
#endif
    Q_STAMP(0);
    bf16x8 xb[5][2], yb[5][2];
    bool first_pass = true;

    auto run_source = [&](const wd_src& q, const bool conv, const int kbase) {
        const int cpt = q.c >> 6;
        const int slr = conv ? NR * SW : QBM;
        const int cpl = slr * 128, chb = 2 * cpl;
        const int pchunks = min(conv ? 5 : 8, (140 * 1024) / chb);
        const int kpc = conv ? 18 : 2;
        const int ntok = conv ? NR * Ws : QBM;
        const int lm = conv ? ST : 1;
        const __amdgpu_buffer_rsrc_t srd_a_hi = make_srd(q.hi), srd_a_lo = make_srd(q.lo);
        int rb[4];
        int skm0 = 0, skm2 = 0;
#pragma unroll
        for (int i = 0; i < 4; ++i) {
            const int p = 16 * i;
            rb[i] = conv ? ST * (p >> wsh) * SW + ST * (p & (W - 1)) : p;
            if (conv) {
                const int ys = ST * (y0 + (p >> wsh)) - 1;
                if (ys < 0) skm0 |= 1 << i;
                if (ys + 2 >= Hs) skm2 |= 1 << i;
            }
        }
        for (int c_lo = 0; c_lo < cpt; c_lo += pchunks) {
            const int nch = min(pchunks, cpt - c_lo);
            const int nks = kpc * nch;
            if (!first_pass) __syncthreads();
            first_pass = false;
            auto kabs_of = [&](const int c, const int r) {
                return kbase + (conv ? 2 * ((r >> 1) * cpt + c_lo + c) + (r & 1) : 2 * (c_lo + c) + r);
            };
            auto advance = [&](int& c, int& r) {
                if (conv) {
                    r += 8;
                    const bool wrap = r >= 18;
                    r = __builtin_amdgcn_readfirstlane(wrap ? r - 18 : r);
                    c = __builtin_amdgcn_readfirstlane(wrap ? c + 1 : c);
                } else {
                    c += 4;
                }
            };
            auto skip_of = [&](const int r) {
                if (!conv) return 0;
                const int ky = (r >> 1) / 3;
                return __builtin_amdgcn_readfirstlane(ky == 0 ? skm0 : ky == 2 ? skm2 : 0);
            };
            auto shift_of = [&](const int r) {
                if (!conv) return 0;
                const int tap = r >> 1, ky = tap / 3;
                return ky * SW + (tap - 3 * ky);
            };
            int nc = conv ? 0 : wave >> 1, nr = conv ? wave : wave & 1;
            int cc = nc, cr = nr;
            load_b(xb, kabs_of(nc, nr), kpc * nc + nr < nks);
            advance(nc, nr);
            if (conv) {
                for (int i = tid; i < nch * 2 * NR * 2 * 8; i += QNT) {
                    const int pc = i & 7, side = (i >> 3) & 1;
                    int rest = i >> 4;
                    const int ry = rest % NR;
                    rest /= NR;
                    const int pl = rest & 1, ch = rest >> 1;
                    const int row = ry * SW + (side ? SW - 1 : 0);
                    *reinterpret_cast<q_u32x4*>(smem + ch * chb + pl * cpl + row * 128 + pc * 16) = q_u32x4{0u, 0u, 0u, 0u};
                }
            }
            const int nitems = nch * ntok * 8;
            for (int i0 = 0; i0 < nitems; i0 += 8 * QNT) {
                q_u32x4 v[2][8];
                int dst[8];
#pragma unroll
                for (int k = 0; k < 8; ++k) {
                    const int i = i0 + k * QNT + tid;
                    const int pc = i & 7;
                    const int rest = i >> 3;
                    const int chl = rest / ntok, tq = rest - chl * ntok;
                    int grow, srow;
                    bool ok = i < nitems;
                    if (conv) {
                        const int ry = tq >> wss, x = tq & (Ws - 1);
                        const int gy = ST * y0 - 1 + ry;
                        ok = ok && gy >= 0 && gy < Hs;
                        grow = bsm * q.hw_src + gy * Ws + x;
                        srow = ry * SW + x + 1;
                    } else {
                        grow = m0 + tq;
                        srow = tq;
                    }
                    const uint32_t vo = ok ? (uint32_t)grow * (uint32_t)(q.ld * 2) + (uint32_t)((c_lo + chl) * 128 + pc * 16) : Q_OOB;
                    v[0][k] = __builtin_amdgcn_raw_buffer_load_b128(srd_a_hi, vo, 0, 0);
                    v[1][k] = __builtin_amdgcn_raw_buffer_load_b128(srd_a_lo, vo, 0, 0);
                    dst[k] = i < nitems ? chl * chb + q_lds_off(srow, pc) : -1;
                }
#pragma unroll
                for (int k = 0; k < 8; ++k)
                    if (dst[k] >= 0) {
                        *reinterpret_cast<q_u32x4*>(smem + dst[k]) = v[0][k];
                        *reinterpret_cast<q_u32x4*>(smem + dst[k] + cpl) = v[1][k];
                    }
            }
            __syncthreads();
            Q_STAMP(1);
            for (int ks = wave; ks < nks; ks += 16) {
                load_b(yb, kabs_of(nc, nr), kpc * nc + nr < nks);
                advance(nc, nr);
                __builtin_amdgcn_sched_barrier(0);
                mfma_step(smem + cc * chb, cpl, rb, shift_of(cr), lm, cr & 1, xb, skip_of(cr));
                __builtin_amdgcn_sched_barrier(0);
                advance(cc, cr);
                load_b(xb, kabs_of(nc, nr), kpc * nc + nr < nks);
                advance(nc, nr);
                __builtin_amdgcn_sched_barrier(0);
                if (kpc * cc + cr < nks) mfma_step(smem + cc * chb, cpl, rb, shift_of(cr), lm, cr & 1, yb, skip_of(cr));
                __builtin_amdgcn_sched_barrier(0);
                advance(cc, cr);
            }
        }
    };
    const bool conv0 = a.src[0].ntaps == 9;
    run_source(a.src[0], conv0, 0);
    if (a.nsrc > 1) run_source(a.src[1], false, 2 * a.src[0].ntaps * (a.src[0].c >> 6));

    Q_STAMP(4);
    __syncthreads();
    Q_STAMP(5);
    constexpr int IMG = QBM * QLDE;
    constexpr int CLD = QBM + 4;
    constexpr int PIMG = QBN * CLD;
    float* res = reinterpret_cast<float*>(smem);
    float* part = res + IMG;
    auto pcol = [&](float* b, const int i, const int t) -> f32x4* {
        return reinterpret_cast<f32x4*>(b + (t * 16 + l15) * CLD + i * 16 + 4 * lq);
    };
    if (wave >= 4) {
        float* b = part + (wave - 4) * PIMG;
#pragma unroll
        for (int i = 0; i < 4; ++i)
#pragma unroll
            for (int t = 0; t < 5; ++t) *pcol(b, i, t) = acc[i][t];
    }
    __syncthreads();
    if (wave < 4) {
        float* b = part + wave * PIMG;
#pragma unroll
        for (int i = 0; i < 4; ++i)
#pragma unroll
            for (int t = 0; t < 5; ++t) {
                acc[i][t] += *pcol(b, i, t);
                *pcol(b, i, t) = acc[i][t];
            }
    }
    __syncthreads();
    for (int e = tid; e < QBN * (QBM / 4); e += QNT) {
        const int col = e >> 4, r4 = (e & 15) * 4;
        const float* p = part + col * CLD + r4;
        f32x4 v = *reinterpret_cast<const f32x4*>(p);
        v += *reinterpret_cast<const f32x4*>(p + PIMG);
        v += *reinterpret_cast<const f32x4*>(p + 2 * PIMG);
        v += *reinterpret_cast<const f32x4*>(p + 3 * PIMG);
#pragma unroll
        for (int r = 0; r < 4; ++r) res[(r4 + r) * QLDE + col] = v[r];
    }
    __syncthreads();
    float* buf = res;
    Q_STAMP(6);
    if (a.gn_gamma) wd_gn_tile<QBN, QNT, false>(a, buf, buf + IMG, m0, n0, tid);
    else wd_epilogue_tail<QBM, QBN, QNT>(a, buf, m0, n0, tid, 0);
    Q_STAMP(7);
#endif
}

}

bool wd_gemmq_applies(const wd_gemm_args& a) {
    const int W = a.slab_rows;
    if (!(a.w_layout == 3 && a.tile == 64080 && !a.a32 && !a.ln_gamma && a.npass == 3 && a.ksplit <= 1 && a.m % 64 == 0 && a.n % QBN == 0 &&
          a.act == WD_ACT_NONE && !a.resid_rows && a.nsrc >= 1 && a.nsrc <= 2))
        return false;
    for (int s = 0; s < a.nsrc; ++s) {
        const wd_src& q = a.src[s];
        if (!q.hi || !q.lo || q.c % 64 || (q.ld & 7)) return false;
        const bool conv = s == 0 && q.ntaps == 9 && q.gather && a.hw_out == 64 &&
                          (((W == 16 || W == 32) && q.hw_src == 64) || (W == 16 && q.hw_src == 256));
        const bool ident = q.ntaps == 1 && !q.gather;
        if (!conv && !ident) return false;
    }
    return true;
}

int wd_gemmq_launch(const wd_gemm_args& a, hipStream_t st) {
    const int loop_smem = 140 * 1024;
    const int red_smem = (QBM * QLDE + 4 * QBN * (QBM + 4)) * 4 + WD_STAT_SCRATCH;
    const int smem = loop_smem > red_smem ? loop_smem : red_smem;
    const int nchp = 0;
    static int attr_max = 0;
    if (smem > attr_max) {
        if (hipFuncSetAttribute(reinterpret_cast<const void*>(&wd_gemmq_kernel), hipFuncAttributeMaxDynamicSharedMemorySize, smem) != hipSuccess)
            return WD_ELAUNCH;
        attr_max = smem;
    }
    const int nbn = a.n / QBN, nbm = a.m / QBM;
    {
        WdLaunchScope scope(WD_CLS_GEMM_Q, st, 2.0 * (double)a.m * (double)a.n * (double)a.ktot);
        hipLaunchKernelGGL(wd_gemmq_kernel, dim3(nbn * nbm), dim3(QNT), smem, st, a, nbn, nbm, nchp);
    }
    return wd_check_launch();
}
```

worddiffusion_amd/csrc/wd_gemmw.hip:

```cpp
#include "wd_gemm_epi.h"
#include "wd_gemm_priv.h"

namespace {

constexpr int WNT = 512;

typedef __attribute__((ext_vector_type(4))) unsigned w_u32x4;

__device__ __forceinline__ int w_lds_off(int row, int ch) { return row * 128 + ((ch ^ ((row >> 1) & 7)) << 4); }

template <int NPASS, int RH, bool A32>
__global__ void __launch_bounds__(WNT, 1) wd_gemmw_kernel(const wd_gemm_args a, const int nbn, const int nbm) {
#if defined(__HIP_DEVICE_COMPILE__)
    constexpr int NPL = (NPASS == 1) ? 1 : 2;
    constexpr int BM = 64 * RH, BN = 320 / RH;
    constexpr int A_PL = BM * 128;
    constexpr int STAGE = NPL * A_PL;
    constexpr uint32_t WD_OOB = 0x80000000u;

    extern __shared__ __attribute__((aligned(16))) char smem[];
    int* s_tab = reinterpret_cast<int*>(smem + 2 * STAGE);

    const int ntile = nbn * nbm;
    const int nwg = ntile * a.ksplit;
    int wg;
    {
        const int bid = blockIdx.x;
        const int q = nwg >> 3, r = nwg & 7, xcd = bid & 7, loc = bid >> 3;
        wg = (xcd < r ? xcd * (q + 1) : r * (q + 1) + (xcd - r) * q) + loc;
    }
    const int sidx = wg % a.ksplit;
    wg /= a.ksplit;
    const int bn_i = wg % nbn, bm_i = wg / nbn;
    const int m0 = bm_i * BM, n0 = bn_i * BN;

    const int tid = threadIdx.x;
    const int lane = tid & 63;
    const int wave = __builtin_amdgcn_readfirstlane(tid >> 6);
    const int kh = wave >> 2;
    const int rh = RH == 2 ? (wave >> 1) & 1 : 0;
    const int cg = RH == 2 ? wave & 1 : wave & 3;
    const int l15 = lane & 15, lq = lane >> 4;

    {
        const int nt0 = a.src[0].ntaps;
        const int32_t* g0 = a.src[0].gather;
        const int hw_src0 = a.src[0].hw_src;
        const int Wimg = a.slab_rows;
        for (int idx = tid; idx < nt0 * BM; idx += WNT) {
            const int t = idx / BM, row = idx - t * BM;
            const int m = m0 + row;
            int v = -1;
            if (m < a.m) {
                if (g0 && Wimg > 0) {
                    const int b = m / a.hw_out, p = m - b * a.hw_out;
                    const int y = p / Wimg, x = p - y * Wimg;
                    const int ky = t / 3, dy = ky - 1, dx = t - ky * 3 - 1;
                    const int sy = y + dy, sx = x + dx;
                    if (sy >= 0 && sy * Wimg < a.hw_out && sx >= 0 && sx < Wimg) v = b * hw_src0 + sy * Wimg + sx;
                } else if (g0) {
                    const int b = m / a.hw_out, p = m - b * a.hw_out;
                    const int g = g0[t * a.hw_out + p];
                    if (g >= 0) v = b * hw_src0 + g;
                } else {
                    v = m;
                }
            }
            s_tab[idx] = v;
        }
    }
    float* s_aff = reinterpret_cast<float*>(s_tab + 9 * BM);
    if constexpr (A32) {
        const int c0 = a.src[0].c;
        const int b = m0 / a.hw_out;
        const int ngp = c0 / a.a32_pcpg, ratio = a.a32_cpg / a.a32_pcpg;
        for (int c = tid; c < c0; c += WNT) {
            const int g = c / a.a32_cpg;
            double su = 0.0, sq = 0.0;
            for (int k = 0; k < ratio; ++k)
                for (int ck = 0; ck < a.a32_nchunk; ++ck) {
                    const double* pp = a.a32_part + (((long)b * a.a32_nchunk + ck) * ngp + g * ratio + k) * 2;
                    su += pp[0];
                    sq += pp[1];
                }
            const double n = (double)a.src[0].hw_src * a.a32_cpg;
            const double mu = su / n;
            double var = sq / n - mu * mu;
            if (var < 0.0) var = 0.0;
            const float rstd = (float)(1.0 / sqrt(var + (double)a.a32_eps));
            const float sc = rstd * a.a32_gamma[c];
            s_aff[2 * c] = sc;
            s_aff[2 * c + 1] = a.a32_beta[c] - (float)mu * sc;
        }
    }
    __syncthreads();
    unsigned long long skipmask = 0;
    if (RH == 1 && a.src[0].gather) {
        for (int t = 0; t < a.src[0].ntaps; ++t) {
            const unsigned long long oob = __ballot(s_tab[t * BM + lane] < 0);
#pragma unroll
            for (int i = 0; i < 4; ++i)
                if (((oob >> (16 * i)) & 0xFFFFull) == 0xFFFFull) skipmask |= 1ull << (4 * t + i);
        }
    }

    auto make_srd = [](const wd_bf16* p) {
        return __builtin_amdgcn_make_buffer_rsrc(const_cast<wd_bf16*>(p), 0, 0x7FFFFFF0, 0x00020000);
    };
    const int nct = a.n >> 4;
    const long wgrp = a.w_ngroups > 1 ? (long)((m0 % a.hw_out) / (a.hw_out / a.w_ngroups)) * a.w_group_stride : 0;
    const __amdgpu_buffer_rsrc_t srd_w_hi = make_srd(a.w_hi + wgrp), srd_w_lo = make_srd((a.w_lo ? a.w_lo : a.w_hi) + wgrp);
    const uint32_t b_voff = (uint32_t)(((n0 >> 4) + 5 * cg) * 1024 + lane * 16);
    const uint32_t kstep_bytes = (uint32_t)nct * 1024u;

    const int arow = tid >> 3, ach = tid & 7;
    const int a_dst = w_lds_off(arow, ach);

    const int nk_all = a.ktot / 64;
    const int k_begin = __builtin_amdgcn_readfirstlane((int)((long)nk_all * sidx / a.ksplit));
    const int k_end = __builtin_amdgcn_readfirstlane((int)((long)nk_all * (sidx + 1) / a.ksplit));
    const int nk = k_end - k_begin;
    const int cpt0 = a.src[0].c >> 6, n0st = a.src[0].ntaps * cpt0;
    int s = 0, tap = 0, kc = 0, left;
    int cur_ld = a.src[0].ld, cur_cpt = cpt0;
    if (k_begin < n0st) {
        tap = __builtin_amdgcn_readfirstlane(k_begin / cpt0);
        kc = k_begin - tap * cpt0;
        left = n0st - k_begin;
    } else {
        s = 1;
        kc = k_begin - n0st;
        cur_ld = a.src[1].ld;
        cur_cpt = a.src[1].c >> 6;
        left = cur_cpt - kc;
    }
    const __amdgpu_buffer_rsrc_t srd0_hi = make_srd(A32 ? reinterpret_cast<const wd_bf16*>(a.a32) : a.src[0].hi),
                                 srd0_lo = make_srd(A32 ? reinterpret_cast<const wd_bf16*>(a.a32) : (a.src[0].lo ? a.src[0].lo : a.src[0].hi));
    const wd_bf16* p1h = a.nsrc > 1 ? a.src[1].hi : a.src[0].hi;
    const wd_bf16* p1l = a.nsrc > 1 ? (a.src[1].lo ? a.src[1].lo : a.src[1].hi) : p1h;
    const __amdgpu_buffer_rsrc_t srd1_hi = make_srd(p1h), srd1_lo = make_srd(p1l);
    uint32_t a_voff[RH];
    auto locate = [&]() {
        int ln;
        asm volatile("v_mbcnt_lo_u32_b32 %0, -1, 0\n\tv_mbcnt_hi_u32_b32 %0, -1, %0" : "=v"(ln));
#pragma unroll
        for (int j = 0; j < RH; ++j) {
            const int row = wave * 8 + (ln >> 3) + 64 * j;
            int r;
            if (s == 0) r = s_tab[tap * BM + row];
            else r = (m0 + row < a.m) ? m0 + row : -1;
            if (A32 && s == 0) a_voff[j] = r >= 0 ? (uint32_t)r * (uint32_t)(a.a32_ld * 4) + (uint32_t)(ach * 32) : WD_OOB;
            else a_voff[j] = r >= 0 ? (uint32_t)r * (uint32_t)(cur_ld * 2) + (uint32_t)(ach * 16) : WD_OOB;
        }
    };
    locate();
    auto kabs = [&]() { return s == 0 ? tap * cpt0 + kc : n0st + kc; };
    auto advance = [&]() {
        --left;
        const bool sw1 = left == 0 && (s + 1 < a.nsrc);
        ++kc;
        bool relocate = false;
        if (kc == cur_cpt) {
            kc = 0;
            ++tap;
            relocate = true;
        }
        if (sw1) {
            s = 1;
            tap = 0;
            kc = 0;
            cur_ld = a.src[1].ld;
            cur_cpt = a.src[1].c >> 6;
            left = cur_cpt;
            relocate = true;
        }
        if (relocate) locate();
    };
    int kb = 0;

    w_u32x4 ra[RH][NPL];
    int ra_ch = 0;
    bool ra_ok[RH];
    auto load_a = [&](const bool live) {
        if (A32) ra_ch = (s == 0) ? kc * 64 + ach * 8 : -1;
#pragma unroll
        for (int j = 0; j < RH; ++j) {
            const uint32_t vo = live ? a_voff[j] : WD_OOB;
            if (A32) ra_ok[j] = vo != WD_OOB;
            if (A32 && s == 0) {
                static_assert(!A32 || NPL == 2, "the fp32 source path holds eight floats in the two plane registers");
                ra[j][0] = __builtin_amdgcn_raw_buffer_load_b128(srd0_hi, vo, kc * 256, 0);
                ra[j][NPL - 1] = __builtin_amdgcn_raw_buffer_load_b128(srd0_hi, vo + 16, kc * 256, 0);
            } else {
#pragma unroll
                for (int p = 0; p < NPL; ++p) {
                    if (s == 0) ra[j][p] = __builtin_amdgcn_raw_buffer_load_b128(p ? srd0_lo : srd0_hi, vo, kc * 128, 0);
                    else ra[j][p] = __builtin_amdgcn_raw_buffer_load_b128(p ? srd1_lo : srd1_hi, vo, kc * 128, 0);
                }
            }
        }
    };
    auto store_a = [&](char* base) {
        if (A32 && ra_ch >= 0) {
            const float4* tab = reinterpret_cast<const float4*>(s_aff + 2 * ra_ch);
            const float4 t0 = tab[0], t1 = tab[1], t2 = tab[2], t3 = tab[3];
            const bool silu = a.a32_silu != 0;
#pragma unroll
            for (int j = 0; j < RH; ++j) {
                const float4 x0 = __builtin_bit_cast(float4, ra[j][0]), x1 = __builtin_bit_cast(float4, ra[j][NPL - 1]);
                float4 y0, y1;
                y0.x = x0.x * t0.x + t0.y; y0.y = x0.y * t0.z + t0.w; y0.z = x0.z * t1.x + t1.y; y0.w = x0.w * t1.z + t1.w;
                y1.x = x1.x * t2.x + t2.y; y1.y = x1.y * t2.z + t2.w; y1.z = x1.z * t3.x + t3.y; y1.w = x1.w * t3.z + t3.w;
                if (silu) {
                    y0.x = wd_silu(y0.x); y0.y = wd_silu(y0.y); y0.z = wd_silu(y0.z); y0.w = wd_silu(y0.w);
                    y1.x = wd_silu(y1.x); y1.y = wd_silu(y1.y); y1.z = wd_silu(y1.z); y1.w = wd_silu(y1.w);
                }
                if (!ra_ok[j]) y0 = y1 = make_float4(0.f, 0.f, 0.f, 0.f);
                uint2 h0, l0, h1, l1;
                wd_split4(y0, h0, l0);
                wd_split4(y1, h1, l1);
                *reinterpret_cast<w_u32x4*>(base + j * 8192 + a_dst) = w_u32x4{h0.x, h0.y, h1.x, h1.y};
                *reinterpret_cast<w_u32x4*>(base + (NPL - 1) * A_PL + j * 8192 + a_dst) = w_u32x4{l0.x, l0.y, l1.x, l1.y};
            }
        } else {
#pragma unroll
            for (int j = 0; j < RH; ++j)
#pragma unroll
                for (int p = 0; p < NPL; ++p) *reinterpret_cast<w_u32x4*>(base + p * A_PL + j * 8192 + a_dst) = ra[j][p];
        }
    };
    auto load_b = [&](bf16x8 (&fb)[5][NPL], const bool live) {
        const uint32_t so = live ? (uint32_t)(2 * kb + kh) * kstep_bytes : 0u;
        const uint32_t vo = live ? b_voff : WD_OOB;
#pragma unroll
        for (int t = 0; t < 5; ++t)
#pragma unroll
            for (int p = 0; p < NPL; ++p)
                fb[t][p] = __builtin_bit_cast(bf16x8, __builtin_amdgcn_raw_buffer_load_b128(p ? srd_w_lo : srd_w_hi, vo + t * 1024, so, 0));
    };

    f32x4 acc[4][5];
#pragma unroll
    for (int i = 0; i < 4; ++i)
#pragma unroll
        for (int t = 0; t < 5; ++t)
#pragma unroll
            for (int r = 0; r < 4; ++r) acc[i][t][r] = 0.0f;

    bf16x8 xb[5][NPL], yb[5][NPL];
    bf16x8 xa[4][NPL];
    auto read_a = [&](const char* base) {
        const int ch = kh * 4 + lq;
#pragma unroll
        for (int i = 0; i < 4; ++i) {
            const int ao = w_lds_off(rh * 64 + i * 16 + l15, ch);
#pragma unroll
            for (int p = 0; p < NPL; ++p) xa[i][p] = *reinterpret_cast<const bf16x8*>(base + p * A_PL + ao);
        }
    };
    auto mfma_all = [&](const bf16x8 (&fb)[5][NPL], const int skip) {
        if constexpr (RH == 1) {
#pragma unroll
            for (int i = 0; i < 4; ++i) {
                if (skip & (1 << i)) continue;
#pragma unroll
                for (int t = 0; t < 5; ++t) {
                    if (NPL == 2) {
                        acc[i][t] = __builtin_amdgcn_mfma_f32_16x16x32_bf16(xa[i][NPL - 1], fb[t][0], acc[i][t], 0, 0, 0);
                        acc[i][t] = __builtin_amdgcn_mfma_f32_16x16x32_bf16(xa[i][0], fb[t][NPL - 1], acc[i][t], 0, 0, 0);
                    }
                    acc[i][t] = __builtin_amdgcn_mfma_f32_16x16x32_bf16(xa[i][0], fb[t][0], acc[i][t], 0, 0, 0);
                }
            }
        } else {
#pragma unroll
            for (int t = 0; t < 5; ++t) {
#pragma unroll
                for (int i = 0; i < 4; ++i) {
                    if (NPL == 2) {
                        acc[i][t] = __builtin_amdgcn_mfma_f32_16x16x32_bf16(xa[i][NPL - 1], fb[t][0], acc[i][t], 0, 0, 0);
                        acc[i][t] = __builtin_amdgcn_mfma_f32_16x16x32_bf16(xa[i][0], fb[t][NPL - 1], acc[i][t], 0, 0, 0);
                    }
                    acc[i][t] = __builtin_amdgcn_mfma_f32_16x16x32_bf16(xa[i][0], fb[t][0], acc[i][t], 0, 0, 0);
                }
            }
        }
    };
    const uint32_t cpt0_inv = (65536u + (uint32_t)cpt0 - 1u) / (uint32_t)cpt0;
    auto skip_of = [&](const int kit) {
        if constexpr (RH != 1) return 0;
        const int ka = k_begin + kit;
        const int tp = (int)(((uint32_t)ka * cpt0_inv) >> 16);
        int sk = (ka < n0st && ka < 1024) ? (int)((skipmask >> (4 * tp)) & 15ull) : 0;
        if (kit >= nk) sk = 15;
        return __builtin_amdgcn_readfirstlane(sk);
    };

    kb = kabs();
    load_a(nk > 0);
    if (nk > 0) advance();
    load_b(xb, nk > 0);
    store_a(smem);
    kb = kabs();
    load_a(nk > 1);
    if (nk > 1) advance();
#ifdef WD_GEMMW_STAMPS
    const bool stamp = (a.dbg & 0x100) && blockIdx.x == 0 && lane == 0 && a.ws;
    unsigned long long* sb = reinterpret_cast<unsigned long long*>(a.ws) + (long)wave * ((nk + 1) & ~1) * 4;
#define WD_STAMP(i) if (stamp) sb[kit * 4 + (i)] = __builtin_amdgcn_s_memtime()
#define WD_STAMP_LGKM() if (stamp) asm volatile("s_waitcnt lgkmcnt(0)" ::: "memory")
#else
#define WD_STAMP(i)
#define WD_STAMP_LGKM()
#endif
    if (kh == 0 || (a.dbg & 0x4000)) {
        auto half_step = [&](const int kit, const bf16x8 (&bcur)[5][NPL], bf16x8 (&bnext)[5][NPL]) {
            __builtin_amdgcn_sched_barrier(0);
            WD_STAMP(0);
            __syncthreads();
            WD_STAMP(1);
            const char* base = smem + (kit & 1) * STAGE;
            char* nbase = smem + ((kit + 1) & 1) * STAGE;
            store_a(nbase);
            load_b(bnext, kit + 1 < nk);
            kb = kabs();
            load_a(kit + 2 < nk);
            if (kit + 2 < nk) advance();
            read_a(base);
            __builtin_amdgcn_sched_barrier(0);
            WD_STAMP_LGKM();
            WD_STAMP(2);
            mfma_all(bcur, skip_of(kit));
            __builtin_amdgcn_sched_barrier(0);
            WD_STAMP(3);
        };
        for (int kit = 0; kit < nk; kit += 2) {
            half_step(kit, xb, yb);
            half_step(kit + 1, yb, xb);
        }
    } else {
        auto late_step = [&](const int kit, bf16x8 (&bset)[5][NPL]) {
            __builtin_amdgcn_sched_barrier(0);
            WD_STAMP(0);
            __syncthreads();
            WD_STAMP(1);
            const char* base = smem + (kit & 1) * STAGE;
            char* nbase = smem + ((kit + 1) & 1) * STAGE;
            if (kit > 0) mfma_all(bset, skip_of(kit - 1));
            __builtin_amdgcn_sched_barrier(0);
            WD_STAMP(2);
            store_a(nbase);
            load_b(bset, kit + 1 < nk);
            kb = kabs();
            load_a(kit + 2 < nk);
            if (kit + 2 < nk) advance();
            read_a(base);
            __builtin_amdgcn_sched_barrier(0);
            WD_STAMP_LGKM();
            WD_STAMP(3);
        };
        for (int kit = 0; kit < nk; kit += 2) {
            late_step(kit, yb);
            late_step(kit + 1, xb);
        }
        if (nk > 0) mfma_all(yb, skip_of(((nk + 1) & ~1) - 1));
    }
#undef WD_STAMP
#undef WD_STAMP_LGKM

    constexpr int LDE = BN + 4;
    float* ep = reinterpret_cast<float*>(smem);
    __syncthreads();
    for (int hh = 0; hh < 2; ++hh) {
        if (kh == hh) {
#pragma unroll
            for (int i = 0; i < 4; ++i)
#pragma unroll
                for (int t = 0; t < 5; ++t)
#pragma unroll
                    for (int r = 0; r < 4; ++r) {
                        float* pe = ep + (rh * 64 + i * 16 + 4 * lq + r) * LDE + cg * 80 + t * 16 + l15;
                        *pe = (hh == 0) ? acc[i][t][r] : *pe + acc[i][t][r];
                    }
        }
        __syncthreads();
    }
    wd_epilogue_tail<BM, BN, WNT>(a, ep, m0, n0, tid, sidx);
#endif
}

__global__ void __launch_bounds__(256) wd_pack_w_kernel(const wd_bf16* __restrict__ hi, const wd_bf16* __restrict__ lo, const int n,
                                                        const int ktot, wd_bf16* __restrict__ out_hi, wd_bf16* __restrict__ out_lo) {
    const long i = (long)blockIdx.x * 256 + threadIdx.x;
    const long total = (long)n * ktot / 8;
    if (i >= total) return;
    const int nct = n >> 4;
    const int l = (int)(i & 63);
    const long blk = i >> 6;
    const int ct = (int)(blk % nct);
    const long ks = blk / nct;
    const long src = (long)(ct * 16 + (l & 15)) * ktot + ks * 32 + (l >> 4) * 8;
    reinterpret_cast<uint4*>(out_hi)[i] = *reinterpret_cast<const uint4*>(hi + src);
    if (lo) reinterpret_cast<uint4*>(out_lo)[i] = *reinterpret_cast<const uint4*>(lo + src);
}

template <int NPASS, int RH, bool A32 = false>
int launchw(const wd_gemm_args& a, hipStream_t st) {
    constexpr int NPL = (NPASS == 1) ? 1 : 2;
    constexpr int BM = 64 * RH, BN = 320 / RH;
    constexpr int loop_smem = 2 * NPL * BM * 128 + 9 * BM * 4 + (A32 ? 2 * 1024 * 4 : 0);
    constexpr int red_smem = BM * (BN + 4) * 4 + WD_STAT_SCRATCH;
    constexpr int smem = loop_smem > red_smem ? loop_smem : red_smem;
    static bool attr_done = false;
    if (!attr_done) {
        if (hipFuncSetAttribute(reinterpret_cast<const void*>(&wd_gemmw_kernel<NPASS, RH, A32>), hipFuncAttributeMaxDynamicSharedMemorySize,
                                smem) != hipSuccess)
            return WD_ELAUNCH;
        attr_done = true;
    }
    const int nbn = a.n / BN, nbm = (a.m + BM - 1) / BM;
    {
        WdLaunchScope scope(WD_CLS_GEMM_WDIRECT, st, 2.0 * (double)a.m * (double)a.n * (double)a.ktot);
        hipLaunchKernelGGL((wd_gemmw_kernel<NPASS, RH, A32>), dim3(nbn * nbm * a.ksplit), dim3(WNT), smem, st, a, nbn, nbm);
    }
    if (a.ksplit > 1) return wd_gemm_launch_reduce(a, st, BM);
    return wd_check_launch();
}

}

int wd_gemmw_launch(const wd_gemm_args& a, hipStream_t st) {
    if (a.a32) return launchw<3, 1, true>(a, st);
    if (a.tile == 128160) return a.npass == 3 ? launchw<3, 2>(a, st) : launchw<1, 2>(a, st);
    return a.npass == 3 ? launchw<3, 1>(a, st) : launchw<1, 1>(a, st);
}

extern "C" int wd_gemm_pack_w(const wd_bf16* hi, const wd_bf16* lo, int n, int ktot, wd_bf16* out_hi, wd_bf16* out_lo, void* stream) {
    if (!hi || !out_hi || (lo && !out_lo) || n <= 0 || ktot <= 0 || n % 16 || ktot % 32) return WD_EINVAL;
    const long total = (long)n * ktot / 8;
    hipStream_t st = reinterpret_cast<hipStream_t>(stream);
    WdLaunchScope scope(WD_CLS_OTHER, st);
    hipLaunchKernelGGL(wd_pack_w_kernel, dim3((unsigned)((total + 255) / 256)), dim3(256), 0, st, hi, lo, n, ktot, out_hi, out_lo);
    return wd_check_launch();
}
```

worddiffusion_amd/engine.py:

```python
from __future__ import annotations

import ctypes as C
import math
import os
from typing import Dict, List, Optional, Tuple

import numpy as np
import torch

from . import _native as N
from .layers import (DownsampleParams, ResBlockParams, SpatialTransformerParams, UpsampleParams)


def conv_gather_table(h: int, w: int, mode: str) -> Tuple[np.ndarray, int, int]:
    if mode == "same":
        ho, wo = h, w
    elif mode == "down":
        ho, wo = (h + 2 - 3) // 2 + 1, (w + 2 - 3) // 2 + 1
    elif mode == "up":
        ho, wo = 2 * h, 2 * w
    elif mode == "down_rb":
        ho, wo = (h - 2) // 2 + 1, (w - 2) // 2 + 1
    else:
        raise ValueError(mode)
    yy, xx = np.meshgrid(np.arange(ho), np.arange(wo), indexing="ij")
    tab = np.full((9, ho * wo), -1, dtype=np.int32)
    for tap in range(9):
        dy, dx = tap // 3 - 1, tap % 3 - 1
        if mode == "same":
            sy, sx = yy + dy, xx + dx
            ok = (sy >= 0) & (sy < h) & (sx >= 0) & (sx < w)
        elif mode == "down":
            sy, sx = 2 * yy + dy, 2 * xx + dx
            ok = (sy >= 0) & (sy < h) & (sx >= 0) & (sx < w)
        elif mode == "down_rb":
            sy, sx = 2 * yy + dy + 1, 2 * xx + dx + 1
            ok = (sy < h) & (sx < w)
        else:
            uy, ux = yy + dy, xx + dx
            ok = (uy >= 0) & (uy < ho) & (ux >= 0) & (ux < wo)
            sy, sx = uy // 2, ux // 2
        idx = sy * w + sx
        tab[tap] = np.where(ok, idx, -1).reshape(-1)
    return tab, ho, wo


def upsample_phase_tables(h: int, w: int) -> Tuple[np.ndarray, np.ndarray]:
    hw = h * w
    tab = np.full((4, 4 * hw), -1, dtype=np.int32)
    yy, xx = np.meshgrid(np.arange(h), np.arange(w), indexing="ij")
    for py in range(2):
        for px in range(2):
            ph = 2 * py + px
            for dy in range(2):
                for dx in range(2):
                    sy, sx = yy + dy - 1 + py, xx + dx - 1 + px
                    ok = (sy >= 0) & (sy < h) & (sx >= 0) & (sx < w)
                    tab[2 * dy + dx, ph * hw:(ph + 1) * hw] = np.where(ok, sy * w + sx, -1).reshape(-1)
    Y, X = np.meshgrid(np.arange(2 * h), np.arange(2 * w), indexing="ij")
    perm = ((2 * (Y % 2) + (X % 2)) * hw + (Y // 2) * w + (X // 2)).reshape(-1).astype(np.int32)
    return tab, perm


def upsample_phase_weights(w: torch.Tensor) -> torch.Tensor:
    sel = torch.tensor([[[1., 0., 0.], [0., 1., 1.]], [[1., 1., 0.], [0., 0., 1.]]], dtype=torch.float32, device=w.device)
    out = torch.einsum("pdk,qel,nckl->pqdenc", sel, sel, w.detach().float())
    n, c = w.shape[0], w.shape[1]
    return out.reshape(4, 4, n, c).contiguous()


def geglu_interleave(w: torch.Tensor, g: int = 32) -> torch.Tensor:
    inner = w.shape[0] // 2
    assert inner % g == 0
    x = w[:inner].reshape(inner // g, g, *w.shape[1:])
    gt = w[inner:].reshape(inner // g, g, *w.shape[1:])
    return torch.stack([x, gt], dim=1).reshape(w.shape)


def wdirect_fills_chip(m: int, n: int) -> bool:
    return ((m + 63) // 64) * (n // 320) >= 256


def geglu_tile(inner: int) -> int:
    return 128160 if inner % 80 == 0 else 128064


def slab_order(wp: torch.Tensor, ntaps0: int, c0: int, c1: int = 0) -> torch.Tensor:
    lead = wp.shape[:-2]
    n = wp.shape[-2]
    k0 = ntaps0 * c0
    w0 = wp[..., :k0].reshape(*lead, n, ntaps0, c0 // 32, 32)
    nl = len(lead)
    w0 = w0.permute(*range(nl), nl + 2, nl + 1, nl, nl + 3).reshape(*lead, (c0 // 32) * ntaps0, n, 32)
    if c1:
        w1 = wp[..., k0:].reshape(*lead, n, c1 // 32, 32).permute(*range(nl), nl + 1, nl, nl + 2)
        w0 = torch.cat([w0, w1], dim=nl)
    return w0.contiguous()


def slab_span(tab: Optional[np.ndarray], hw_out: int, hw_src: int, m: int, bm: int = 128) -> int:
    if tab is None:
        return bm
    period = int(np.lcm(bm, hw_out))
    mt = min(m, 2 * period)
    rows = np.arange(mt)
    b, p = rows // hw_out, rows % hw_out
    src = np.where(tab[:, p] >= 0, b[None, :] * hw_src + tab[:, p], -1)
    span = 0
    for r0 in range(0, mt, bm):
        blk = src[:, r0:r0 + bm]
        valid = blk[blk >= 0]
        if valid.size:
            span = max(span, int(valid.max() - valid.min() + 1))
    return span


_PARAM_GEN = [0]
_NATIVE_WRITES = [0]


def note_native_write():
    _NATIVE_WRITES[0] += 1

PLAN_CACHE_SIZE = int(os.environ.get("WDIFF_PLAN_CACHE", "4"))


def _bump_param_gen(*_a):
    _PARAM_GEN[0] += 1


torch.nn.modules.module.register_module_parameter_registration_hook(_bump_param_gen)

FILM_CHUNK_ROWS = int(os.environ.get("WDIFF_FILM_CHUNK_ROWS", "8192"))


class _Recipe:
    __slots__ = ("name", "planes", "rows", "cols", "shape", "pieces")

    def __init__(self, name, planes, rows=0, cols=0, shape=None):
        self.name, self.planes, self.rows, self.cols, self.shape, self.pieces = name, planes, rows, cols, shape, []

    @staticmethod
    def _nct(w):
        return w.shape[0], w.shape[1], (w.shape[2] * w.shape[3] if w.dim() == 4 else 1)

    def fwd(self, w, row_off=0, col_off=0, g=0):
        n, c, t = self._nct(w)
        assert row_off + n <= self.rows and col_off + t * c <= self.cols, self.name
        self.pieces.append((0, w, None, n, c, t, row_off, col_off, 0, g))
        return self

    def bwd(self, w, col_off=0, npad=None):
        n, c, t = self._nct(w)
        npad = n if npad is None else npad
        assert c <= self.rows and col_off + t * npad <= self.cols, self.name
        self.pieces.append((1, w, None, n, c, t, 0, col_off, npad, 0))
        return self

    def vec(self, p, p2=None, off=0, g=0):
        self.pieces.append((2, p, p2, p.numel(), 1, 1, 0, off, 0, g))
        return self

    def host(self) -> torch.Tensor:
        first = self.pieces[0][1]
        out = torch.zeros((self.rows, self.cols) if self.planes else (int(torch.tensor(self.shape).prod()),),
                          dtype=torch.float32, device=first.device)
        for (mode, p, p2, n, c, t, row_off, col_off, npad, g) in self.pieces:
            src = p.detach().float()
            if mode == 2:
                v = src.reshape(-1) + (p2.detach().float().reshape(-1) if p2 is not None else 0)
                out[col_off:col_off + n] = geglu_interleave(v, g) if g else v
                continue
            w3 = src.reshape(n, c, t)
            if mode == 0:
                blk = w3.permute(0, 2, 1).reshape(n, t * c)
                out[row_off:row_off + n, col_off:col_off + t * c] = geglu_interleave(blk, g) if g else blk
            else:
                blk = torch.zeros(c, t, npad, dtype=torch.float32, device=first.device)
                blk[:, :, :n] = w3.permute(1, 2, 0)
                out[:c, col_off:col_off + t * npad] = blk.reshape(c, t * npad)
        return out if self.planes else out.reshape(self.shape)


class RecipeBook(dict):

    def matrix(self, name, rows, cols) -> _Recipe:
        self[name] = _Recipe(name, True, rows, cols)
        return self[name]

    def vector(self, name, p, p2=None, g=0) -> _Recipe:
        self[name] = _Recipe(name, False, shape=tuple(p.shape)).vec(p, p2, 0, g)
        return self[name]

    def vector_cat(self, name, ps) -> _Recipe:
        r = _Recipe(name, False, shape=(sum(p.numel() for p in ps),))
        off = 0
        for p in ps:
            r.vec(p, None, off)
            off += p.numel()
        self[name] = r
        return r

    def linear(self, name, lin):
        self.matrix(name + ".w", lin.weight.shape[0], lin.weight.shape[1]).fwd(lin.weight)
        if lin.bias is not None:
            self.vector(name + ".b", lin.bias)

    @staticmethod
    def frag_ok(r) -> bool:
        return r.planes and r.rows % 16 == 0 and r.cols % 32 == 0 and all(
            mode == 0 and c % 32 == 0 and t in (1, 9) and col_off % 2 == 0 and row_off >= 0
            for (mode, p, p2, n, c, t, row_off, col_off, npad, g) in r.pieces)

    def device_table(self, lib, dst: Dict[str, torch.Tensor], dev, frag: Optional[Dict[str, torch.Tensor]] = None):
        import struct
        assert lib.wd_repack_entry_bytes() == 80
        tile, vchunk = lib.wd_repack_tile(), lib.wd_repack_vchunk()
        recs, c0 = [], 0
        for name, r in self.items():
            d = dst[name]
            for (mode, p, p2, n, c, t, row_off, col_off, npad, g) in r.pieces:
                assert p.is_cuda and p.dtype == torch.float32 and p.is_contiguous(), name
                if mode == 2:
                    hi, lo, ld, ntc = d.data_ptr() + 4 * col_off, 0, 0, 1
                    nch = (n + vchunk - 1) // vchunk
                else:
                    ld = r.cols
                    o = 2 * (row_off * ld + col_off)
                    hi, lo = d[0].data_ptr() + o, d[1].data_ptr() + o
                    ntc = (c + tile - 1) // tile
                    nch = (((npad if mode == 1 else n) + tile - 1) // tile) * ntc
                recs.append(struct.pack("<QQQQiiiiiiiiqii", p.data_ptr(), p2.data_ptr() if p2 is not None else 0, hi, lo, n, c, t,
                                        mode, npad, ld, g, ntc, c0, 0, 0))
                c0 += nch
                if frag is not None and name in frag and self.frag_ok(r):
                    f = frag[name]
                    recs.append(struct.pack("<QQQQiiiiiiiiqii", p.data_ptr(), 0, f[0].data_ptr(), f[1].data_ptr(), n, c, t, 3, 0,
                                            r.rows, g, ntc, c0, row_off, col_off))
                    c0 += nch
        raw = torch.frombuffer(bytearray(b"".join(recs)), dtype=torch.uint8).to(dev)
        return raw, c0, len(recs)


class Act:
    __slots__ = ("t", "c", "h", "w", "stats", "prod", "perm")

    def __init__(self, t, c, h, w, stats=None, prod=None, perm=None):
        self.t, self.c, self.h, self.w = t, c, h, w
        self.perm = perm
        self.stats = stats
        self.prod = prod


class Plan:
    def __init__(self):
        self.cond: List[tuple] = []
        self.step: List[tuple] = []
        self.keep: List[object] = []
        self.out: Optional[torch.Tensor] = None

    @staticmethod
    def _run(ops, stream):
        for fn, args, what in ops:
            rc = fn(*args, stream)
            if rc != 0:
                N.check(rc, what)

    def run_cond(self, stream):
        self._run(self.cond, stream)

    def run_film(self, stream):
        self._run(getattr(self, "film", []), stream)
        self.film_loaded = -1

    @staticmethod
    def film_prepare(t, stream):
        return False

    def run_step(self, stream):
        self._run(self.step, stream)

    def run_step1(self, stream):
        self._run(self.step1, stream)


def _ptr(t: Optional[torch.Tensor], byte_off: int = 0):
    return None if t is None else t.data_ptr() + byte_off


class UNetEngine:

    def __init__(self, model, variant: str):
        self.model = model
        self.variant = variant
        self.lib = N.lib()
        self.npass = 3
        self._sig = None
        self._ps, self._ps_gen = None, -1
        self._pack = None
        self._w: Dict[str, torch.Tensor] = {}
        self._w3: Dict[str, torch.Tensor] = {}
        self._w3_meta: Dict[str, tuple] = {}
        self._wf: Dict[str, torch.Tensor] = {}
        self.use_wdirect = os.environ.get("WDIFF_GEMM_WDIRECT", "1") != "0"
        self.use_up_phases = os.environ.get("WDIFF_UPSAMPLE_PHASES", "1") != "0"
        self._derived: Dict[str, tuple] = {}
        self.use_smallmap = os.environ.get("WDIFF_GEMM_SMALLMAP", "1") != "0"
        self.fuse_ff = os.environ.get("WDIFF_FUSE_FF", "1") != "0"
        self.fuse_proj = os.environ.get("WDIFF_FUSE_PROJ", "1") != "0"
        self.fuse_ln = os.environ.get("WDIFF_FUSE_LN", "1") != "0"
        self.fuse_gn_in = int(os.environ.get("WDIFF_FUSE_GN_IN", "1"))
        self.use_slab = os.environ.get("WDIFF_SLAB", "0") != "0"
        self.fuse_stats = os.environ.get("WDIFF_FUSE_STATS", "1") != "0"
        self.fuse_xattn = os.environ.get("WDIFF_FUSE_XATTN", "1") != "0"
        self.use_conv3 = os.environ.get("WDIFF_CONV3", "0") != "0"
        if (self.use_slab or self.use_conv3) and not self.lib.wd_gemm_experimental():
            raise N.NativeError("WDIFF_SLAB / WDIFF_CONV3 need a library built with WDIFF_EXPERIMENTAL=1 "
                                "(python -m worddiffusion_amd.build --force)")
        self.fuse_xattn_pair = os.environ.get("WDIFF_FUSE_XATTN_PAIR", "1") != "0"
        self.fuse_st = os.environ.get("WDIFF_FUSE_ST", "1") != "0"
        self.fuse_out = os.environ.get("WDIFF_FUSE_OUT", "1") != "0"
        self.fuse_in = os.environ.get("WDIFF_FUSE_IN", "1") != "0"
        self.pack_kv = os.environ.get("WDIFF_PACK_KV", "1") != "0"
        self.fuse_gn2 = os.environ.get("WDIFF_FUSE_GN2", "1") != "0"
        self.fuse_gn = os.environ.get("WDIFF_FUSE_GN", "1") != "0"
        self.fuse_split = os.environ.get("WDIFF_FUSE_SPLIT", "1") != "0"
        self._plans: Dict[tuple, Plan] = {}
        self._tabs: Dict[tuple, torch.Tensor] = {}
        self._tab_np: Dict[int, np.ndarray] = {}
        self._same_w: Dict[int, int] = {}
        self._down_w: Dict[int, int] = {}
        self._ws = None
        self.device = None

    def set_precision(self, mode: str):
        npass = {"bf16x3": 3, "fp32": 3, "bf16": 1}[mode]
        if npass != self.npass:
            self.npass = npass
            self._plans.clear()

    def _recipes(self) -> "RecipeBook":
        m = self.model
        R = RecipeBook()
        film_w = []
        self.film_off = {}
        off = 0
        cin_conv = m.input_blocks[0][0]
        self.kpad_in = ((9 * cin_conv.in_channels + 31) // 32) * 32
        R.matrix("in.w", cin_conv.out_channels, self.kpad_in).fwd(cin_conv.weight)
        R.vector("in.b", cin_conv.bias)
        R.vector("in.w.f32", cin_conv.weight)
        R.linear("te0", m.time_embed[0])
        R.linear("te2", m.time_embed[2])
        if m.num_classes is not None:
            R.vector("label", m.label_emb.weight)
        we = m.word_emb
        cd = we.embedding.weight.shape[1]
        R.vector("we.table", we.embedding.weight)
        qkv = (we.attention.linear_query, we.attention.linear_key, we.attention.linear_value)
        R.matrix("we.qkv.w", 3 * cd, cd)
        R.vector_cat("we.qkv.b", [l.bias for l in qkv])
        for i, l in enumerate(qkv):
            R["we.qkv.w"].fwd(l.weight, row_off=i * cd)
        kv_w = []
        self.kv_off = {}
        kvo = 0
        for name, mod in self._walk():
            if isinstance(mod, ResBlockParams):
                R.vector(name + ".gn1.g", mod.in_layers[0].weight)
                R.vector(name + ".gn1.b", mod.in_layers[0].bias)
                R.matrix(name + ".c1.w", mod.cout, 9 * mod.cin).fwd(mod.in_layers[2].weight)
                R.vector(name + ".c1.b", mod.in_layers[2].bias)
                R.vector(name + ".gn2.g", mod.out_layers[0].weight)
                R.vector(name + ".gn2.b", mod.out_layers[0].bias)
                if mod.cin != mod.cout:
                    R.matrix(name + ".c2.w", mod.cout, 9 * mod.cout + mod.cin).fwd(mod.out_layers[3].weight) \
                        .fwd(mod.skip_connection.weight, col_off=9 * mod.cout)
                    R.vector(name + ".c2.b", mod.out_layers[3].bias, mod.skip_connection.bias)
                else:
                    R.matrix(name + ".c2.w", mod.cout, 9 * mod.cout).fwd(mod.out_layers[3].weight)
                    R.vector(name + ".c2.b", mod.out_layers[3].bias)
                film_w.append(mod.emb_layers[1])
                self.film_off[name] = off
                off += mod.cout
            elif isinstance(mod, (DownsampleParams, UpsampleParams)):
                conv = mod.op if isinstance(mod, DownsampleParams) else mod.conv
                R.matrix(name + ".w", mod.cout, 9 * mod.cin).fwd(conv.weight)
                R.vector(name + ".b", conv.bias)
                if isinstance(mod, UpsampleParams) and self._up_phases_ok(mod):
                    key = name + ".wph"
                    if key not in self._derived or self._derived[key][0].device != conv.weight.device:
                        self._derived[key] = (torch.empty((4, 4, mod.cout, mod.cin), dtype=torch.float32, device=conv.weight.device),
                                              (lambda cv=conv: upsample_phase_weights(cv.weight)))
                    wph = self._derived[key][0]
                    for ph in range(4):
                        r = R.matrix(f"{name}.wph{ph}", mod.cout, 4 * mod.cin)
                        for t in range(4):
                            r.fwd(wph[ph, t], col_off=t * mod.cin)
            elif isinstance(mod, SpatialTransformerParams):
                inner = mod.heads * mod.d_head
                R.vector(name + ".gn.g", mod.norm.weight)
                R.vector(name + ".gn.b", mod.norm.bias)
                R.matrix(name + ".pi.w", inner, mod.ch).fwd(mod.proj_in.weight)
                R.vector(name + ".pi.b", mod.proj_in.bias)
                R.matrix(name + ".po.w", mod.ch, inner).fwd(mod.proj_out.weight)
                R.vector(name + ".po.b", mod.proj_out.bias)
                for d, tb in enumerate(mod.transformer_blocks):
                    p = f"{name}.tb{d}"
                    for ln in ("norm1", "norm2", "norm3"):
                        R.vector(f"{p}.{ln}.g", getattr(tb, ln).weight)
                        R.vector(f"{p}.{ln}.b", getattr(tb, ln).bias)
                    if self.variant == "phosc":
                        R.matrix(p + ".a1.qkv.w", 3 * inner, inner)
                        for i, l in enumerate((tb.attn1.to_q, tb.attn1.to_k, tb.attn1.to_v)):
                            R[p + ".a1.qkv.w"].fwd(l.weight, row_off=i * inner)
                        cross = [("a2", tb.attn2)]
                    else:
                        R.matrix(p + ".a1.q.w", inner, inner).fwd(tb.attn1.to_q.weight)
                        cross = [("a1", tb.attn1), ("a2", tb.attn2)]
                    R.matrix(p + ".a2.q.w", inner, inner).fwd(tb.attn2.to_q.weight)
                    for tag, at in cross:
                        kv_w.append(at)
                        self.kv_off[f"{p}.{tag}"] = kvo
                        kvo += 2 * at.to_k.weight.shape[0]
                        R.vector(f"{p}.{tag}.q.f32", at.to_q.weight)
                        R.vector(f"{p}.{tag}.o.f32", at.to_out[0].weight)
                    for tag, at in (("a1", tb.attn1), ("a2", tb.attn2)):
                        R.linear(f"{p}.{tag}.o", at.to_out[0])
                    ffi = tb.ff.net[2].in_features
                    g = geglu_tile(ffi) % 1000 // 2
                    R.matrix(p + ".ff1.w", 2 * ffi, inner).fwd(tb.ff.net[0].proj.weight, g=g)
                    R.vector(p + ".ff1.b", tb.ff.net[0].proj.bias, g=g)
                    R.linear(p + ".ff2", tb.ff.net[2])
                    if N.lib().wd_ff_supported(inner, ffi):
                        R.matrix(p + ".ff1f.w", 2 * ffi, inner).fwd(tb.ff.net[0].proj.weight, g=16)
                        R.vector(p + ".ff1f.b", tb.ff.net[0].proj.bias, g=16)
        self.film_total = off
        self.kv_total = kvo
        ted = m.time_embed[2].out_features
        R.matrix("film.w", off, ted)
        R.vector_cat("film.b", [l.bias for l in film_w])
        r0 = 0
        for l in film_w:
            R["film.w"].fwd(l.weight, row_off=r0)
            r0 += l.weight.shape[0]
        if kv_w:
            R.matrix("kv.w", kvo, kv_w[0].to_k.weight.shape[1])
            r0 = 0
            for at in kv_w:
                for l in (at.to_k, at.to_v):
                    R["kv.w"].fwd(l.weight, row_off=r0)
                    r0 += l.weight.shape[0]
        self._film_mods, self._kv_mods = film_w, kv_w
        R.vector("out.gn.g", m.out[0].weight)
        R.vector("out.gn.b", m.out[0].bias)
        R.matrix("out.w", m.out[2].out_channels, 9 * m.out[2].in_channels).fwd(m.out[2].weight)
        R.vector("out.b", m.out[2].bias)
        R.vector("out.w.f32", m.out[2].weight)
        return R

    def _walk(self):
        m = self.model
        for i, blk in enumerate(m.input_blocks):
            for j, mod in enumerate(blk):
                yield f"in{i}.{j}", mod
        for j, mod in enumerate(m.middle_block):
            yield f"mid.{j}", mod
        for i, blk in enumerate(m.output_blocks):
            for j, mod in enumerate(blk):
                yield f"out{i}.{j}", mod

    def _signature(self):
        if self._ps is None or self._ps_gen != _PARAM_GEN[0]:
            self._ps, self._ps_gen = list(self.model.parameters()), _PARAM_GEN[0]
        ps = self._ps
        return (sum(p._version for p in ps) + (_NATIVE_WRITES[0] << 32), hash(tuple(p.data_ptr() for p in ps)), str(ps[0].device))

    def refresh_weights(self, force: bool = False):
        sig = self._signature()
        if not force and sig == self._sig:
            return
        dev = next(self.model.parameters()).device
        if dev.type != "cuda":
            raise N.NativeError("worddiffusion_amd runs on an MI355X only: move the model to cuda "
                                "(there is no CPU / eager fallback)")
        if self.device is not None and dev != self.device:
            self._w.clear()
            self._w3.clear()
            self._wf.clear()
            self._w3_meta.clear()
            self._plans.clear()
            self._tabs.clear()
            self._tab_np.clear()
            self._ws = None
            self._pack = None
        self.device = dev
        if self._pack is None or self._pack[0] != sig[1:]:
            book = self._recipes()
            for p in self.model.parameters():
                if p.dtype != torch.float32 or not p.is_contiguous():
                    raise N.NativeError("parameters must be contiguous fp32 (the reference never retypes them, unet.py:415)")
            for name, r in book.items():
                if name not in self._w:
                    self._w[name] = (torch.zeros((2, r.rows, r.cols), dtype=torch.bfloat16, device=dev) if r.planes
                                     else torch.zeros(r.shape, dtype=torch.float32, device=dev))
            table, chunks, n = book.device_table(self.lib, self._w, dev, self._wf)
            self._pack = (sig[1:], table, chunks, n, [k for k in self._wf if k not in book or not book.frag_ok(book[k])])
        _, table, chunks, n, wf_left = self._pack
        stream = torch.cuda.current_stream(dev).cuda_stream
        with torch.no_grad():
            for buf, fn in self._derived.values():
                buf.copy_(fn())
        N.check(self.lib.wd_repack_multi(table.data_ptr(), n, chunks, stream), "wd_repack_multi")
        for name in wf_left:
            self._pack_wf(name, self._wf[name], stream)
        with torch.no_grad():
            for name, meta in self._w3_meta.items():
                self._w3[name].copy_(slab_order(self._w[name], *meta))
            if "freqs" not in self._w and hasattr(self.model, "word_emb"):
                half = self.model.model_channels // 2
                freqs = torch.exp(-math.log(10000) * torch.arange(0, half, dtype=torch.float32) / half)
                self._w["freqs"] = freqs.to(dev)
                self._w["pe"] = self.model.word_emb.positional_encoding.to(dev).contiguous()
        self._sig = sig

    def _pack_wf(self, name, wf, stream):
        wp = self._w[name]
        N.check(self.lib.wd_gemm_pack_w(wp[0].data_ptr(), wp[1].data_ptr(), wp.shape[1], wp.shape[2], wf[0].data_ptr(),
                                        wf[1].data_ptr(), stream), "wd_gemm_pack_w")

    def _table(self, h, w, mode):
        key = (h, w, mode)
        if key not in self._tabs:
            tab, ho, wo = conv_gather_table(h, w, mode)
            dt = torch.from_numpy(tab).to(self.device)
            self._tabs[key] = (dt, ho, wo)
            self._tab_np[dt.data_ptr()] = tab
            if mode == "down":
                self._down_w[dt.data_ptr()] = wo
            if mode == "same":
                self._same_w[dt.data_ptr()] = w
        return self._tabs[key]

    def _f32(self, P: Plan, *shape):
        t = torch.empty(shape, dtype=torch.float32, device=self.device)
        P.keep.append(t)
        return t

    def _planes(self, P: Plan, rows, ld):
        t = torch.zeros((2, rows, ld), dtype=torch.bfloat16, device=self.device)
        P.keep.append(t)
        return t

    def _hilo(self, planes: Optional[torch.Tensor], byte_off: int = 0):
        if planes is None:
            return None, None
        return planes[0].data_ptr() + byte_off, (planes[1].data_ptr() + byte_off if self.npass == 3 else None)

    def _src(self, planes: torch.Tensor, c: int, ntaps: int = 1, gather: Optional[torch.Tensor] = None,
             hw_src: int = 0, col_off: int = 0) -> N.WdSrc:
        s = N.WdSrc()
        s._tab_np = self._tab_np.get(gather.data_ptr()) if gather is not None else None
        s._same_w = self._same_w.get(gather.data_ptr(), 0) if gather is not None else 0
        s._down_w = self._down_w.get(gather.data_ptr(), 0) if gather is not None else 0
        ld = planes.shape[2]
        s.hi = planes[0].data_ptr() + 2 * col_off
        s.lo = planes[1].data_ptr() + 2 * col_off
        s.gather = _ptr(gather)
        s.ld, s.c, s.ntaps, s.hw_src = ld, c, ntaps, hw_src
        return s

    def _gemm(self, ops, what, srcs, wname, m, hw_out, bias=None, rowvec=None, rowvec_ld=0, resid=None,
              resid_ld=0, resid_rows=None, act=N.ACT_NONE, out_f32=None, out_ld=0, out_pl=None, n=None, tile=0,
              w_row_off=0, want_stats=False, a32=None, ln=None, w_groups=None):
        a = N.WdGemmArgs()
        for i, s in enumerate(srcs):
            a.src[i] = s
        a.nsrc = len(srcs)
        a.npass = self.npass
        wp = self._w[wname]
        ktot = wp.shape[2]
        assert ktot == sum(s.ntaps * s.c for s in srcs), (what, ktot, [(s.ntaps, s.c) for s in srcs])
        nrows = wp.shape[1] if n is None else n
        a.w_hi = wp[0].data_ptr() + 2 * w_row_off * ktot
        a.w_lo = wp[1].data_ptr() + 2 * w_row_off * ktot
        a.m, a.n, a.ktot, a.hw_out = m, nrows, ktot, hw_out
        a.bias = _ptr(bias)
        a.rowvec, a.rowvec_ld = rowvec, rowvec_ld
        a.resid, a.resid_ld, a.resid_rows = resid, resid_ld, resid_rows
        a.act = act
        a.out_f32, a.out_ld = _ptr(out_f32), out_ld
        if out_pl is not None:
            a.out_hi, a.out_lo, a.out_pl_ld = out_pl[0].data_ptr(), out_pl[1].data_ptr(), out_pl.shape[2]
        if a32 is not None:
            self._set_a32(a, *a32)
        if w_groups is not None:
            a.w_ngroups, a.w_group_stride = w_groups
        a.tile = tile
        if self._ws is None:
            self._ws = torch.empty(128 * 128 * 160 * 8, dtype=torch.float32, device=self.device)
        a.ksplit, a.ws, a.ws_floats = 0, self._ws.data_ptr(), self._ws.numel()
        self._give_tickets(a, m, nrows)
        span = 0
        if self.use_slab and w_row_off == 0 and (len(srcs) == 1 or (srcs[1].ntaps == 1 and not srcs[1].gather)):
            tabnp = getattr(srcs[0], "_tab_np", None)
            span = slab_span(tabnp, hw_out, srcs[0].hw_src, m)
            if span > 192 or ((m + 127) // 128) * max(1, nrows // 160) < 96:
                span = 0
        s0 = srcs[0]
        frag = not span and not self.use_conv3 and w_row_off == 0 and n is None and act == N.ACT_NONE and tile == 0
        width = (getattr(s0, "_down_w", 0) or getattr(s0, "_same_w", 0)) if s0.ntaps == 9 else 0
        wdirect = (frag and self.use_wdirect and wdirect_fills_chip(m, nrows) and
                   self._legal(a, w_layout=3, tile=64320, slab_rows=getattr(s0, "_same_w", 0) if s0.ntaps == 9 else 0))
        smallmap = (frag and not wdirect and self.use_smallmap and hw_out == 64 and 128 <= (m // 64) * (nrows // 80) <= 512 and
                    self._legal(a, w_layout=3, tile=64080, slab_rows=width))
        assert (a32 is None and w_groups is None) or wdirect, what
        if wdirect or smallmap:
            wf = self._wfrag(wname)
            a.w_hi, a.w_lo = wf[0].data_ptr(), wf[1].data_ptr()
        elif span:
            meta = (srcs[0].ntaps, srcs[0].c, srcs[1].c if len(srcs) > 1 else 0)
            if wname not in self._w3:
                self._w3[wname] = slab_order(wp, *meta)
                self._w3_meta[wname] = meta
            assert self._w3_meta[wname] == meta, wname
            w3 = self._w3[wname]
            a.w_hi, a.w_lo = w3[0].data_ptr(), w3[1].data_ptr()
            a.w_layout, a.slab_rows = 1, span
        else:
            same_w = getattr(srcs[0], "_same_w", 0)
            if (same_w and srcs[0].ntaps == 9 and srcs[0].c % 64 == 0 and act == N.ACT_NONE and tile == 0 and
                    (len(srcs) == 1 or (srcs[1].ntaps == 1 and not srcs[1].gather and srcs[1].c % 64 == 0))):
                a.w_layout, a.slab_rows = 2, same_w
        a._ln_pl = None
        if ln is not None and self.fuse_ln and not self.use_slab:
            pl = torch.zeros((2, m, nrows), dtype=torch.bfloat16, device=self.device)
            if self._legal(a, out_hi=pl[0].data_ptr(), out_lo=pl[1].data_ptr(), out_pl_ld=nrows, ln_gamma=self._w[ln + ".g"].data_ptr(),
                           ln_beta=self._w[ln + ".b"].data_ptr(), ln_eps=1e-5):
                self._cur_plan.keep.append(pl)
                a._ln_pl = pl
        stats = None
        if want_stats and self.fuse_stats and nrows % 32 == 0 and (hw_out % 128 == 0 or hw_out == 64) and not span:
            cpg = nrows // 32
            r = self._resolved(a, stat_part=a.ws, stat_cpg=cpg)
            if r is not None:
                nchunk = max(1, hw_out // (r.tile // 1000))
                part = torch.zeros((m // hw_out, nchunk, 32, 2), dtype=torch.float64, device=self.device)
                self._cur_plan.keep.append(part)
                a.stat_part, a.stat_cpg = part.data_ptr(), cpg
                stats = (part, nchunk, cpg)
        a._stats = stats
        self._cur_plan.keep.append(a)
        ops.append((self.lib.wd_gemm, (C.byref(a),), what))
        return a

    def _resolved(self, a, **fields) -> Optional[N.WdGemmArgs]:
        b = N.WdGemmArgs.from_buffer_copy(a)
        for k, v in fields.items():
            setattr(b, k, v)
        out = N.WdGemmArgs()
        return out if self.lib.wd_gemm_check(C.byref(b), C.byref(out)) == N.WD_OK else None

    def _legal(self, a, apply=True, **fields) -> bool:
        if self._resolved(a, **fields) is None:
            return False
        if apply:
            for k, v in fields.items():
                setattr(a, k, v)
        return True

    def _set_a32(self, a, x32: "Act", gname, eps, silu):
        part, nchunk, pc = x32.stats
        a.a32, a.a32_ld, a.a32_part = x32.t.data_ptr(), x32.c, part.data_ptr()
        a.a32_nchunk, a.a32_pcpg, a.a32_cpg = nchunk, pc, x32.c // 32
        a.a32_gamma, a.a32_beta = self._w[gname + ".g"].data_ptr(), self._w[gname + ".b"].data_ptr()
        a.a32_eps, a.a32_silu = float(eps), int(silu)

    def _wdirect_ok(self, srcs, m, n, hw_out, a32=None, **fields) -> bool:
        a = N.WdGemmArgs()
        for i, s in enumerate(srcs):
            a.src[i] = s
        a.nsrc, a.npass, a.m, a.n, a.ktot, a.hw_out = len(srcs), self.npass, m, n, sum(s.ntaps * s.c for s in srcs), hw_out
        a.w_layout, a.tile = 3, 64320
        a.w_hi = a.w_lo = a.out_f32 = 16
        a.out_ld = n
        if a32 is not None:
            self._set_a32(a, *a32)
        return self._legal(a, apply=False, **fields)

    def _give_tickets(self, a, m, n):
        ntick = ((m + 63) // 64) * ((n + 63) // 64)
        if ntick > 2048:
            return
        P = self._cur_plan
        tk = getattr(P, "_tickets", None)
        if tk is None or P._ticket_off + ntick > tk.numel():
            tk = torch.zeros(1 << 16, dtype=torch.int32, device=self.device)
            P.keep.append(tk)
            P._tickets, P._ticket_off = tk, 0
        a.tickets, a.ntickets = tk.data_ptr() + 4 * P._ticket_off, ntick
        P._ticket_off += ntick

    def _gn(self, P, ops, what, srcs: List[Act], gname, eps, silu, want_raw=False, dropout=None):
        B = self._B
        h, w = srcs[0].h, srcs[0].w
        hw = h * w
        ctot = sum(s.c for s in srcs)
        cpg = ctot // 32
        has_perm = any(s.perm is not None for s in srcs)
        if has_perm and not (len(srcs) == 2 and srcs[1].perm is None and self.fuse_gn2 and not any(s.c % cpg for s in srcs)):
            raise NotImplementedError(f"{what}: a phase-major map (Upsample) is read by the two-source GroupNorm of a decoder block only")
        if any(s.c % cpg for s in srcs):
            cat = self._f32(P, B * hw, ctot)
            coff = 0
            for s in srcs:
                ops.append((self.lib.wd_copy2d, (cat.data_ptr() + 4 * coff, 4 * ctot, s.t.data_ptr(), 4 * s.c, 4 * s.c,
                                                 B * hw), what + ":concat"))
                coff += s.c
            srcs = [Act(cat, ctot, h, w)]
        pl = self._planes(P, B * hw, ctot)
        raw = self._planes(P, B * hw, ctot) if want_raw else None
        for s in srcs:
            self._gn_stats(P, ops, what, s)
        coff = 0
        gam, bet = self._w[gname + ".g"], self._w[gname + ".b"]
        todo = []
        for s in srcs:
            part, nchunk, pc = s.stats
            assert cpg % pc == 0, (what, cpg, pc)
            if nchunk > 8:
                ngs = s.c // pc
                folded = torch.empty((B, 1, ngs, 2), dtype=torch.float64, device=self.device)
                P.keep.append(folded)
                ops.append((self.lib.wd_gn_fold_chunks, (part.data_ptr(), B, nchunk, ngs, folded.data_ptr()), what + ":fold chunks"))
                part, nchunk = folded, 1
                s.stats = (part, nchunk, pc)
            if has_perm or dropout is not None or not self._gn_in_combine(s, raw, gam, bet, eps, silu, cpg, pl, coff):
                todo.append((s, part, nchunk, pc, coff))
            coff += s.c
        hi, lo = self._hilo(pl)
        rhi, rlo = self._hilo(raw)
        if len(todo) == 2 and self.fuse_gn2:
            (sa, pa, na, pca, ca), (sb, pb, nb_, pcb, cb) = todo
            ops.append((self.lib.wd_gn_apply2,
                        (sa.t.data_ptr(), sa.c, sa.c, pa.data_ptr(), na, pca, ca, sb.t.data_ptr(), sb.c, sb.c, pb.data_ptr(), nb_, pcb, cb,
                         B, hw, cpg, gam.data_ptr(), bet.data_ptr(), eps, int(silu), hi, lo, ctot, rhi, rlo,
                         sa.perm.data_ptr() if sa.perm is not None else None),
                        what + ":apply"))
        elif dropout is not None:
            assert not has_perm and len(srcs) == 1, what
            (s, part, nchunk, pc, c0), = todo
            ops.append((self.lib.wd_gn_apply_dropout,
                        (s.t.data_ptr(), s.c, B, hw, s.c, cpg, part.data_ptr(), nchunk, pc, gam.data_ptr(), bet.data_ptr(), eps,
                         int(silu), hi, lo, ctot, c0, rhi, rlo, C.byref(dropout)), what + ":apply+dropout"))
        else:
            assert not has_perm, what
            for s, part, nchunk, pc, c0 in todo:
                ops.append((self.lib.wd_gn_apply,
                            (s.t.data_ptr(), s.c, B, hw, s.c, cpg, part.data_ptr(), nchunk, pc, gam.data_ptr(), bet.data_ptr(), eps,
                             int(silu), hi, lo, ctot, c0, rhi, rlo), what + ":apply"))
        return pl, raw

    def _gn_stats(self, P, ops, what, s: Act):
        if s.stats is None:
            B, hw = self._B, s.h * s.w
            nchunk = self.lib.wd_gn_nchunk(hw)
            pc = s.c // 32
            part = torch.empty((B, nchunk, 32, 2), dtype=torch.float64, device=self.device)
            P.keep.append(part)
            ops.append((self.lib.wd_gn_stats, (s.t.data_ptr(), s.c, B, hw, s.c, pc, part.data_ptr()), what + ":stats"))
            s.stats = (part, nchunk, pc)
        return s.stats

    def _gn_in_consumer(self, P, ops, what, srcs: List[Act], want_raw, M, hw, ncols, taps=1, gather=None) -> bool:
        if not (self.fuse_gn_in and self.use_wdirect and len(srcs) == 1 and not want_raw and not self.use_conv3):
            return False
        if taps > 1 and self.fuse_gn_in < 2:
            return False
        if not wdirect_fills_chip(M, ncols):
            return False
        s = srcs[0]
        self._gn_stats(P, ops, what, s)
        return self._wdirect_ok([self._src32(s, taps, gather, hw)], M, ncols, hw, a32=(s, what, 0.0, False))

    def _src32(self, x: Act, ntaps=1, gather=None, hw_src=0) -> N.WdSrc:
        s = N.WdSrc()
        s._tab_np = self._tab_np.get(gather.data_ptr()) if gather is not None else None
        s._same_w = self._same_w.get(gather.data_ptr(), 0) if gather is not None else 0
        s.hi, s.lo, s.gather = None, None, _ptr(gather)
        s.ld, s.c, s.ntaps, s.hw_src = x.c, x.c, ntaps, hw_src
        return s

    def _gn_in_combine(self, s: Act, raw, gam, bet, eps, silu, cpg, pl, coff) -> bool:
        pr = s.prod
        if pr is None or not isinstance(pr, N.WdGemmArgs) or not self.fuse_gn or raw is not None or self.use_conv3:
            return False
        if pr.out_f32 != s.t.data_ptr() or pr.out_hi or pr.gn_gamma or pr.n != s.c:
            return False
        hi, lo = self._hilo(pl, 2 * coff)
        return self._legal(pr, gn_gamma=gam.data_ptr() + 4 * coff, gn_beta=bet.data_ptr() + 4 * coff, gn_eps=float(eps),
                           gn_silu=int(silu), gn_cpg=cpg, out_hi=hi, out_lo=lo, out_pl_ld=pl.shape[2])

    def _ln(self, P, ops, what, x: torch.Tensor, rows, c, name):
        pl = self._planes(P, rows, c)
        ops.append((self.lib.wd_layernorm,
                    (x.data_ptr(), c, rows, c, self._w[name + ".g"].data_ptr(), self._w[name + ".b"].data_ptr(), 1e-5,
                     *self._hilo(pl), c), what))
        return pl

    def _resblock(self, P, name, mod: ResBlockParams, srcs: List[Act]) -> Act:
        ops = P.step
        B = self._B
        h, w = srcs[0].h, srcs[0].w
        hw, M = h * w, B * h * w
        cin, cout = mod.cin, mod.cout
        assert cin == sum(s.c for s in srcs)
        tab, _, _ = self._table(h, w, "same")
        need_raw = cin != cout
        h1 = self._f32(P, M, cout)
        if self._gn_in_consumer(P, ops, name + ".gn1", srcs, need_raw, M, hw, cout, taps=9, gather=tab):
            s1, in1 = self._src32(srcs[0], 9, tab, hw), (srcs[0], name + ".gn1", 1e-5, True)
            raw = None
        else:
            a1, raw = self._gn(P, ops, name + ".gn1", srcs, name + ".gn1", 1e-5, True, want_raw=need_raw)
            s1, in1 = self._src(a1, cin, 9, tab, hw), None
        g1 = self._gemm(ops, name + ".conv1", [s1], name + ".c1.w", M, hw,
                        bias=self._w[name + ".c1.b"], rowvec=self._film.data_ptr() + 4 * self.film_off[name],
                        rowvec_ld=self.film_total, out_f32=h1, out_ld=cout, want_stats=True, a32=in1)
        h1a = Act(h1, cout, h, w, g1._stats, prod=g1)
        if self._gn_in_consumer(P, ops, name + ".gn2", [h1a], False, M, hw, cout, taps=9, gather=tab):
            s2, in2 = self._src32(h1a, 9, tab, hw), (h1a, name + ".gn2", 1e-5, True)
        else:
            a2, _ = self._gn(P, ops, name + ".gn2", [h1a], name + ".gn2", 1e-5, True)
            s2, in2 = self._src(a2, cout, 9, tab, hw), None
        out = self._f32(P, M, cout)
        if need_raw:
            g2 = self._gemm(ops, name + ".conv2+skip", [s2, self._src(raw, cin)],
                            name + ".c2.w", M, hw, bias=self._w[name + ".c2.b"], out_f32=out, out_ld=cout,
                            want_stats=True, a32=in2)
        else:
            g2 = self._gemm(ops, name + ".conv2", [s2], name + ".c2.w", M, hw,
                            bias=self._w[name + ".c2.b"], resid=srcs[0].t.data_ptr(), resid_ld=cout, out_f32=out,
                            out_ld=cout, want_stats=True, a32=in2)
        return Act(out, cout, h, w, g2._stats, prod=g2)

    def _up_phases_ok(self, mod) -> bool:
        return (getattr(self, "use_up_phases", False) and self.use_wdirect and self.fuse_gn2 and self.npass == 3 and not self.use_slab and
                not self.use_conv3)

    def _resample(self, P, name, mod, x: Act, mode: str, tile: int = 0) -> Act:
        ops = P.step
        B = self._B
        assert x.perm is None, name
        tab, ho, wo = self._table(x.h, x.w, mode)
        pl = self._planes(P, B * x.h * x.w, x.c)
        pr = x.prod
        if (pr is not None and self.fuse_split and not pr.out_hi and pr.out_f32 == x.t.data_ptr() and
                (pr.n if isinstance(pr, N.WdGemmArgs) else pr.c) == x.c):
            pr.out_hi, pr.out_lo = self._hilo(pl)
            pr.out_pl_ld = x.c
        else:
            ops.append((self.lib.wd_split, (x.t.data_ptr(), x.c, B * x.h * x.w, x.c, 0, *self._hilo(pl), x.c), name + ":split"))
        out = self._f32(P, B * ho * wo, mod.cout)
        hw = x.h * x.w
        src4 = None
        if mode == "up" and tile == 0 and (name + ".wph0") in self._w and self._up_phases_ok(mod) and wdirect_fills_chip(B * 4 * hw, mod.cout):
            key = (x.h, x.w, "up4")
            if key not in self._tabs:
                t4, pm = upsample_phase_tables(x.h, x.w)
                dt, dp = torch.from_numpy(t4).to(self.device), torch.from_numpy(pm).to(self.device)
                self._tabs[key] = (dt, dp)
                self._tab_np[dt.data_ptr()] = t4
            tab4, perm = self._tabs[key]
            src4 = self._src(pl, x.c, 4, tab4, hw)
            groups = (4, mod.cout * 4 * x.c)
            if not self._wdirect_ok([src4], B * 4 * hw, mod.cout, 4 * hw, w_ngroups=groups[0], w_group_stride=groups[1]):
                src4 = None
        if src4 is not None:
            if (name + ".wph0") not in self._wf:
                grp = torch.empty((2, 4, mod.cout, 4 * x.c), dtype=torch.bfloat16, device=self.device)
                st = torch.cuda.current_stream(self.device).cuda_stream
                for ph in range(4):
                    self._wf[f"{name}.wph{ph}"] = grp[:, ph]
                    self._pack_wf(f"{name}.wph{ph}", grp[:, ph], st)
                self._pack = None
            gg = self._gemm(ops, name + ".conv (4 phases)", [src4], name + ".wph0", B * 4 * hw, 4 * hw,
                            bias=self._w[name + ".b"], out_f32=out, out_ld=mod.cout, want_stats=True, w_groups=groups)
            return Act(out, mod.cout, ho, wo, gg._stats, prod=None, perm=perm)
        gg = self._gemm(ops, name + ".conv", [self._src(pl, x.c, 9, tab, x.h * x.w)], name + ".w", B * ho * wo, ho * wo,
                        bias=self._w[name + ".b"], out_f32=out, out_ld=mod.cout, want_stats=True, tile=tile)
        return Act(out, mod.cout, ho, wo, gg._stats, prod=gg)

    def _attention(self, ops, what, q, ldq, k, ldk, v, ldv, heads, nq, nk, d, scale, out_pl, out_f32=None,
                   out_rows=None, out_row0=0):
        B = self._B
        ops.append((self.lib.wd_attention,
                    (q, ldq, k, ldk, v, ldv, B, heads, nq, nk, d, float(scale), _ptr(out_f32), *self._hilo(out_pl),
                     out_pl.shape[2] if out_pl is not None else out_f32.shape[-1],
                     nq if out_rows is None else out_rows, out_row0), what))

    def _xattn_fold(self, P, at, heads, d):
        B, L, inner = self._B, self._ctx_len, heads * d
        ko = self.kv_off[at]
        mq = self._f32(P, B, heads * L, inner)
        mo = self._f32(P, B, heads * L, inner)
        mq_pl = torch.zeros((B, 2, 64, inner), dtype=torch.bfloat16, device=self.device)
        mot_pl = torch.zeros((B, 2, inner, 64), dtype=torch.bfloat16, device=self.device)
        P.keep += [mq_pl, mot_pl]
        P.cond.append((self.lib.wd_xattn_fold,
                       (self._kv.data_ptr() + 4 * ko, self.kv_total, self._kv.data_ptr() + 4 * (ko + inner), self.kv_total, B,
                        heads, L, d, float(d ** -0.5), self._w[at + ".q.f32"].data_ptr(), self._w[at + ".o.f32"].data_ptr(), inner,
                        mq.data_ptr(), mo.data_ptr(), mq_pl.data_ptr(), mot_pl.data_ptr()), at + ":fold"))
        return mq, mo, mq_pl, mot_pl

    def _transformer(self, P, name, mod: SpatialTransformerParams, x: Act) -> Act:
        ops = P.step
        B = self._B
        h, w, c = x.h, x.w, x.c
        hw, M = h * w, B * h * w
        heads, d = mod.heads, mod.d_head
        inner = heads * d
        L = self._ctx_len
        if (self.fuse_st and self.variant != "phosc" and len(mod.transformer_blocks) == 1 and inner == c == 320 and
                self.npass == 3 and self.fuse_xattn and self.fuse_xattn_pair and self.fuse_ff and self.fuse_proj and
                bool(self.lib.wd_xattn_supported(inner, heads, L)) and (M + 63) // 64 >= 192 and hw % 64 == 0 and
                (name + ".tb0.ff1f.w") in self._w and
                self._gn_in_consumer(P, ops, name + ".gn", [x], False, M, hw, inner)):
            return self._transformer_fused(P, name, mod, x)
        tok = self._f32(P, M, inner)
        ln1 = f"{name}.tb0.norm1" if self.variant == "phosc" else None
        if self._gn_in_consumer(P, ops, name + ".gn", [x], False, M, hw, inner):
            g_in = self._gemm(ops, name + ".proj_in", [self._src32(x, hw_src=hw)], name + ".pi.w", M, hw, bias=self._w[name + ".pi.b"],
                              out_f32=tok, out_ld=inner, a32=(x, name + ".gn", 1e-6, False), ln=ln1)
        else:
            g, _ = self._gn(P, ops, name + ".gn", [x], name + ".gn", 1e-6, False)
            g_in = self._gemm(ops, name + ".proj_in", [self._src(g, c)], name + ".pi.w", M, hw, bias=self._w[name + ".pi.b"],
                              out_f32=tok, out_ld=inner, ln=ln1)
        n1_pre = g_in._ln_pl
        xpl = None
        fuse = self.fuse_xattn and bool(self.lib.wd_xattn_supported(inner, heads, L))

        def folded(tag, p, x_in, x_out, ln_name, next_ln=None):
            mq, mo, mq_pl, mot_pl = self._xattn_fold(P, f"{p}.{tag}", heads, d)
            npl = self._planes(P, M, inner) if next_ln else None
            ops.append((self.lib.wd_xattn_fused,
                        (x_in.data_ptr(), inner, B, hw, inner, self._w[f"{p}.{ln_name}.g"].data_ptr(),
                         self._w[f"{p}.{ln_name}.b"].data_ptr(), 1e-5, mq.data_ptr(), mo.data_ptr(), heads, L,
                         self._w[f"{p}.{tag}.o.b"].data_ptr(), x_out.data_ptr(), inner,
                         self._w[f"{p}.{next_ln}.g"].data_ptr() if next_ln else None,
                         self._w[f"{p}.{next_ln}.b"].data_ptr() if next_ln else None, 1e-5, *self._hilo(npl), inner,
                         mq_pl.data_ptr(), mot_pl.data_ptr()),
                        f"{p}.{tag}:folded"))
            return npl

        def folded_pair(p, x_in, x_out):
            _, _, qa, oa = self._xattn_fold(P, p + ".a1", heads, d)
            _, _, qb, ob = self._xattn_fold(P, p + ".a2", heads, d)
            npl = self._planes(P, M, inner)
            g2, b2 = self._w[f"{p}.norm2.g"].data_ptr(), self._w[f"{p}.norm2.b"].data_ptr()
            ops.append((self.lib.wd_xattn_pair,
                        (x_in.data_ptr(), inner, B, hw, inner, 1e-5, heads, L, g2, b2, qa.data_ptr(), oa.data_ptr(),
                         self._w[f"{p}.a1.o.b"].data_ptr(), g2, b2, qb.data_ptr(), ob.data_ptr(),
                         self._w[f"{p}.a2.o.b"].data_ptr(), x_out.data_ptr(), inner, self._w[f"{p}.norm3.g"].data_ptr(),
                         self._w[f"{p}.norm3.b"].data_ptr(), 1e-5, *self._hilo(npl), inner), f"{p}.a1+a2:folded"))
            return npl

        for di, tb in enumerate(mod.transformer_blocks):
            p = f"{name}.tb{di}"
            scale = d ** -0.5
            n3 = None
            if fuse and self.variant != "phosc" and self.fuse_xattn_pair:
                tok2 = self._f32(P, M, inner)
                n3 = folded_pair(p, tok, tok2)
            tok1 = self._f32(P, M, inner) if n3 is None else None
            if n3 is not None:
                pass
            elif self.variant == "phosc":
                n1 = n1_pre if (di == 0 and n1_pre is not None) else self._ln(P, ops, p + ".norm1", tok, M, inner, p + ".norm1")
                qkv = self._f32(P, M, 3 * inner)
                self._gemm(ops, p + ".a1.qkv", [self._src(n1, inner)], p + ".a1.qkv.w", M, hw, out_f32=qkv,
                           out_ld=3 * inner)
                o1 = self._planes(P, M, inner)
                self._attention(ops, p + ".a1", qkv.data_ptr(), 3 * inner, qkv.data_ptr() + 4 * inner, 3 * inner,
                                qkv.data_ptr() + 8 * inner, 3 * inner, heads, hw, hw, d, scale, o1)
                n2_pre = self._gemm(ops, p + ".a1.out", [self._src(o1, inner)], p + ".a1.o.w", M, hw, bias=self._w[p + ".a1.o.b"],
                                    resid=tok.data_ptr(), resid_ld=inner, out_f32=tok1, out_ld=inner,
                                    ln=None if fuse else p + ".norm2")._ln_pl
            elif fuse:
                folded("a1", p, tok, tok1, "norm2")
            else:
                n1 = self._ln(P, ops, p + ".norm2a", tok, M, inner, p + ".norm2")
                q1 = self._f32(P, M, inner)
                self._gemm(ops, p + ".a1.q", [self._src(n1, inner)], p + ".a1.q.w", M, hw, out_f32=q1, out_ld=inner)
                ko = self.kv_off[p + ".a1"]
                o1 = self._planes(P, M, inner)
                self._attention(ops, p + ".a1", q1.data_ptr(), inner, self._kv.data_ptr() + 4 * ko, self.kv_total,
                                self._kv.data_ptr() + 4 * (ko + inner), self.kv_total, heads, hw, L, d, scale, o1)
                self._gemm(ops, p + ".a1.out", [self._src(o1, inner)], p + ".a1.o.w", M, hw, bias=self._w[p + ".a1.o.b"],
                           resid=tok.data_ptr(), resid_ld=inner, out_f32=tok1, out_ld=inner)
            if n3 is not None:
                pass
            elif fuse:
                tok2 = self._f32(P, M, inner)
                n3 = folded("a2", p, tok1, tok2, "norm2", next_ln="norm3")
            else:
                tok2 = self._f32(P, M, inner)
                n2 = n2_pre if (self.variant == "phosc" and n2_pre is not None) else \
                    self._ln(P, ops, p + ".norm2", tok1, M, inner, p + ".norm2")
                q2 = self._f32(P, M, inner)
                self._gemm(ops, p + ".a2.q", [self._src(n2, inner)], p + ".a2.q.w", M, hw, out_f32=q2, out_ld=inner)
                ko = self.kv_off[p + ".a2"]
                o2 = self._planes(P, M, inner)
                kp, vp = self._kv.data_ptr() + 4 * ko, self._kv.data_ptr() + 4 * (ko + inner)
                nimg = self.lib.wd_attention_packed_elems(B, heads, L, d) if self.pack_kv else 0
                if nimg > 0:
                    img = torch.empty(nimg, dtype=torch.bfloat16, device=self.device)
                    P.keep.append(img)
                    P.cond.append((self.lib.wd_attention_pack_kv,
                                   (kp, self.kv_total, vp, self.kv_total, B, heads, L, d, img.data_ptr()), p + ".a2:pack kv"))
                    ops.append((self.lib.wd_attention_packed,
                                (q2.data_ptr(), inner, img.data_ptr(), B, heads, hw, L, d, float(scale), None, *self._hilo(o2), inner,
                                 hw, 0), p + ".a2"))
                else:
                    self._attention(ops, p + ".a2", q2.data_ptr(), inner, kp, self.kv_total, vp, self.kv_total, heads, hw, L, d,
                                    scale, o2)
                n3 = self._gemm(ops, p + ".a2.out", [self._src(o2, inner)], p + ".a2.o.w", M, hw, bias=self._w[p + ".a2.o.b"],
                                resid=tok1.data_ptr(), resid_ld=inner, out_f32=tok2, out_ld=inner, ln=p + ".norm3")._ln_pl
            if n3 is None:
                n3 = self._ln(P, ops, p + ".norm3", tok2, M, inner, p + ".norm3")
            last = di == len(mod.transformer_blocks) - 1
            tok = self._f32(P, M, inner)
            xpl = self._planes(P, M, inner) if last else None
            ffi = tb.ff.net[2].in_features
            if self.fuse_ff and (p + ".ff1f.w") in self._w and (M + 63) // 64 >= 192:
                if last and self.fuse_proj and inner == c:
                    out = self._f32(P, M, c)
                    fa = self._ff_fused(ops, p, n3, tok2, M, inner, ffi, out, None,
                                        proj=(name + ".po.w", self._w[name + ".po.b"], x.t, hw))
                    return Act(out, c, h, w, fa._stats, prod=fa)
                self._ff_fused(ops, p, n3, tok2, M, inner, ffi, None if last else tok, xpl)
            else:
                ffh = self._planes(P, M, ffi)
                self._gemm(ops, p + ".ff1", [self._src(n3, inner)], p + ".ff1.w", M, hw, bias=self._w[p + ".ff1.b"],
                           act=N.ACT_GEGLU, out_pl=ffh, tile=geglu_tile(ffi))
                self._gemm(ops, p + ".ff2", [self._src(ffh, ffi)], p + ".ff2.w", M, hw, bias=self._w[p + ".ff2.b"],
                           resid=tok2.data_ptr(), resid_ld=inner, out_f32=None if last else tok, out_ld=inner,
                           out_pl=xpl)
        out = self._f32(P, M, c)
        gg = self._gemm(ops, name + ".proj_out", [self._src(xpl, inner)], name + ".po.w", M, hw,
                        bias=self._w[name + ".po.b"], resid=x.t.data_ptr(), resid_ld=c, out_f32=out, out_ld=c,
                        want_stats=True)
        return Act(out, c, h, w, gg._stats, prod=gg)

    def _transformer_fused(self, P, name, mod: SpatialTransformerParams, x: Act) -> Act:
        M, hw, c = self._B * x.h * x.w, x.h * x.w, x.c
        heads, d, L = mod.heads, mod.d_head, self._ctx_len
        p = name + ".tb0"
        folds = [self._xattn_fold(P, f"{p}.{tag}", heads, d)[2:] for tag in ("a1", "a2")]
        tok2 = self._f32(P, M, c)
        out = self._f32(P, M, c)
        part, nchunk, pc = x.stats
        pw = self._wfrag(name + ".pi.w")
        front = dict(x_in=x.t.data_ptr(), x_in_ld=c, hw=hw, gn_part=part.data_ptr(), gn_nchunk=nchunk, gn_pcpg=pc, gn_cpg=c // 32,
                     gn_eps=1e-6, gn_gamma=self._w[name + ".gn.g"].data_ptr(), gn_beta=self._w[name + ".gn.b"].data_ptr(),
                     pi_hi=pw[0].data_ptr(), pi_lo=pw[1].data_ptr(), pi_b=self._w[name + ".pi.b"].data_ptr(),
                     ln2_gamma=self._w[p + ".norm2.g"].data_ptr(), ln2_beta=self._w[p + ".norm2.b"].data_ptr(),
                     mq_a=folds[0][0].data_ptr(), mot_a=folds[0][1].data_ptr(), xb_a=self._w[p + ".a1.o.b"].data_ptr(),
                     mq_b=folds[1][0].data_ptr(), mot_b=folds[1][1].data_ptr(), xb_b=self._w[p + ".a2.o.b"].data_ptr(),
                     ln3_gamma=self._w[p + ".norm3.g"].data_ptr(), ln3_beta=self._w[p + ".norm3.b"].data_ptr(), ln_eps=1e-5,
                     heads=heads, L=L, tok2=tok2.data_ptr())
        ffi = mod.transformer_blocks[0].ff.net[2].in_features
        fa = self._ff_fused(P.step, p, None, tok2, M, c, ffi, out, None, proj=(name + ".po.w", self._w[name + ".po.b"], x.t, hw),
                            front=front)
        return Act(out, c, x.h, x.w, fa._stats, prod=fa)

    def _wfrag(self, wname):
        if wname not in self._wf:
            self._wf[wname] = torch.empty_like(self._w[wname])
            self._pack_wf(wname, self._wf[wname], torch.cuda.current_stream(self.device).cuda_stream)
            self._pack = None
        return self._wf[wname]

    def _ff_fused(self, ops, p, n3, resid, M, inner, ffi, out_f32, out_pl, proj=None, front=None):
        a = N.WdFfArgs()
        if front is None:
            (a.x_hi, a.x_lo), a.x_ld = self._hilo(n3), n3.shape[2]
        else:
            for k, v in front.items():
                setattr(a, k, v)
        a.m, a.c, a.inner = M, inner, ffi
        w1, w2 = self._wfrag(p + ".ff1f.w"), self._wfrag(p + ".ff2.w")
        a.w1_hi, a.w1_lo, a.b1 = w1[0].data_ptr(), w1[1].data_ptr(), self._w[p + ".ff1f.b"].data_ptr()
        a.w2_hi, a.w2_lo, a.b2 = w2[0].data_ptr(), w2[1].data_ptr(), self._w[p + ".ff2.b"].data_ptr()
        a.resid, a.resid_ld = resid.data_ptr(), inner
        if out_f32 is not None:
            a.out_f32, a.out_ld = out_f32.data_ptr(), inner
        if out_pl is not None:
            (a.out_hi, a.out_lo), a.out_pl_ld = self._hilo(out_pl), out_pl.shape[2]
        a.hw_out, a.npass = 1, self.npass
        stats = None
        if proj is not None:
            wname, b3, x_in, hw = proj
            w3 = self._wfrag(wname)
            a.w3_hi, a.w3_lo, a.b3 = w3[0].data_ptr(), w3[1].data_ptr(), b3.data_ptr()
            a.resid3, a.resid3_ld = x_in.data_ptr(), inner
            if self.fuse_stats and inner % 32 == 0 and hw % 64 == 0:
                nchunk = hw // 64
                part = torch.zeros((M // hw, nchunk, 32, 2), dtype=torch.float64, device=self.device)
                self._cur_plan.keep.append(part)
                a.stat_part, a.stat_cpg, a.hw_out = part.data_ptr(), inner // 32, hw
                stats = (part, nchunk, inner // 32)
        self._cur_plan.keep.append(a)
        what = ".ff (fused)" if proj is None else ".ff + proj_out (fused)" if front is None else ": gn + proj_in + a1 + a2 + ff + proj_out (fused)"
        ops.append((self.lib.wd_ff_fused, (C.byref(a),), p + what))
        a._stats = stats
        return a

    @staticmethod
    def _cached_plan(plans: Dict[tuple, Plan], key, room: int = 0) -> Optional[Plan]:
        if key in plans:
            plans[key] = plans.pop(key)
            return plans[key]
        while room and len(plans) >= room:
            plans.pop(next(iter(plans)))
        return None

    def _begin_plan(self, P: Plan, B: int) -> Plan:
        self._cur_plan = P
        self._B = B
        return P

    def _inputs(self, P: Plan, H, W, ctx_len, phosc_len):
        m, B, dev = self.model, self._B, self.device
        P.x_in = torch.zeros((B, m.in_channels, H, W), dtype=torch.float32, device=dev)
        P.t_in = torch.zeros((B,), dtype=torch.int64, device=dev)
        P.y_in = torch.zeros((B,), dtype=torch.int64, device=dev)
        P.ctx_in = torch.zeros((B, max(ctx_len, 1)), dtype=torch.int64, device=dev)
        P.phosc_in = torch.zeros((B, max(phosc_len, 1)), dtype=torch.int32, device=dev)

    def _conditioning(self, P: Plan, ops, ctx_len, phosc_len) -> List[tuple]:
        m, lib, B = self.model, self.lib, self._B
        cd = m.context_dim
# ... 293 lines not shown
```

Measured before the change: 35.17 images/s.

## Read fp32 skip-connection maps directly in conv2+skip GEMM, splitting in-kernel

For resblocks whose input and output channel counts differ, the 1x1 skip source of the conv2+skip GEMM can now be read straight from the fp32 input maps, including up to two concatenated maps with optional row permutations. The hi/lo bf16 split happens inside the wdirect and small-map kernels. The GroupNorm pass therefore no longer has to write a raw hi/lo plane copy of the input, which saves that memory traffic. In exchange the skip operand moves twice as many bytes per element as fp32, it is split in the GEMM load path, and the path forbids split-K, which may reduce parallelism.

```diff
diff --git a/include/wdiff_hip.h b/include/wdiff_hip.h
--- a/include/wdiff_hip.h
+++ b/include/wdiff_hip.h
@@ -81,6 +81,10 @@
     float ln_eps;
     int32_t w_ngroups;
     int64_t w_group_stride;
+    const float* f32_x[2];
+    const int32_t* f32_perm[2];
+    int32_t f32_ld[2];
+    int32_t f32_c[2];
 } wd_gemm_args;
 
 int wd_gemm(const wd_gemm_args* args, void* stream);
diff --git a/worddiffusion_amd/_native.py b/worddiffusion_amd/_native.py
--- a/worddiffusion_amd/_native.py
+++ b/worddiffusion_amd/_native.py
@@ -38,7 +38,8 @@
                 ("gn_silu", C.c_int32), ("gn_cpg", C.c_int32), ("a32", _vp), ("a32_ld", C.c_int32), ("a32_part", _vp),
                 ("a32_nchunk", C.c_int32), ("a32_pcpg", C.c_int32), ("a32_cpg", C.c_int32), ("a32_gamma", _vp), ("a32_beta", _vp),
                 ("a32_eps", C.c_float), ("a32_silu", C.c_int32), ("ln_gamma", _vp), ("ln_beta", _vp), ("ln_eps", C.c_float),
-                ("w_ngroups", C.c_int32), ("w_group_stride", C.c_int64)]
+                ("w_ngroups", C.c_int32), ("w_group_stride", C.c_int64), ("f32_x", _vp * 2), ("f32_perm", _vp * 2),
+                ("f32_ld", C.c_int32 * 2), ("f32_c", C.c_int32 * 2)]
 
 
 class WdFfArgs(C.Structure):
diff --git a/worddiffusion_amd/csrc/wd_gemm.hip b/worddiffusion_amd/csrc/wd_gemm.hip
--- a/worddiffusion_amd/csrc/wd_gemm.hip
+++ b/worddiffusion_amd/csrc/wd_gemm.hip
@@ -2065,6 +2065,8 @@
     static const int ks_env = getenv("WDIFF_GEMM_KS") ? atoi(getenv("WDIFF_GEMM_KS")) : 2;
     r.ks = ks_env == 1 ? 1 : 2;
     if (a.ksplit < 0 || a.ksplit > WD_MAX_KSPLIT) return WD_EINVAL;
+    const bool f32 = a.f32_x[0] != nullptr;
+    if ((f32 && a.w_layout != 3) || (!f32 && (a.f32_x[1] || a.f32_c[0] || a.f32_c[1]))) return WD_EINVAL;
     if (a.w_layout == 3) {
         if (a.n % 80 || a.act == WD_ACT_GEGLU || (a.tile && a.tile != 64320 && a.tile != 128160 && a.tile != 64080) || a.ktot % 64)
             return WD_EINVAL;
@@ -2119,6 +2121,10 @@
                 !a.a32_beta || a.a32_nchunk <= 0 || a.a32_pcpg <= 0 || a.a32_cpg <= 0 || a.a32_cpg % a.a32_pcpg || q.c % a.a32_cpg ||
                 q.c > 1024 || a.a32_ld < q.c || (a.a32_ld & 3) || (reinterpret_cast<uintptr_t>(a.a32) & 15) || q.hw_src <= 0)
                 return WD_EINVAL;
+        } else if (s == 1 && f32) {
+            if (q.c <= 0 || q.c % BK || q.ntaps != 1 || q.gather) return WD_EINVAL;
+            k += q.c;
+            continue;
         } else if (!q.hi || (a.npass == 3 && !q.lo)) return WD_EINVAL;
         if (q.c <= 0 || q.c % BK || q.ld % 8 || q.ntaps < 1) return WD_EINVAL;
         if (!q.gather && q.ntaps != 1) return WD_EINVAL;
@@ -2132,6 +2138,7 @@
         for (int s = 0; s < a.nsrc; ++s) {
             const wd_src& q = a.src[s];
             const long rows = q.gather ? (long)((a.m + a.hw_out - 1) / a.hw_out) * q.hw_src : (long)a.m;
+            if (s == 1 && f32) continue;
             if ((s == 0 && a.a32) ? rows * a.a32_ld * 4 >= lim : rows * q.ld * 2 >= lim) return WD_EINVAL;
         }
     }
@@ -2144,7 +2151,7 @@
             (a.rowvec && a.rowvec_ld < nout))
             return WD_EINVAL;
         for (int s = 0; s < a.nsrc; ++s)
-            if (!(s == 0 && a.a32) && a.src[s].ld < a.src[s].c) return WD_EINVAL;
+            if (!(s == 0 && a.a32) && !(s == 1 && f32) && a.src[s].ld < a.src[s].c) return WD_EINVAL;
     }
 
     if (a.w_layout == 3) {
@@ -2156,6 +2163,22 @@
         const bool down3 = a.tile == 64080 && q0.ntaps == 9 && q0.gather && a.slab_rows > 0 && q0.hw_src == 4 * a.hw_out;
         if (!same3 && !down3) a.slab_rows = 0;
         a.tickets = nullptr;
+        if (f32) {
+            if ((a.tile != 64320 && a.tile != 64080) || a.npass != 3 || a.nsrc != 2 || a.a32 || a.hw_out % 64) return WD_EINVAL;
+            const long rows = (long)((a.m + a.hw_out - 1) / a.hw_out) * a.hw_out;
+            int cs = 0;
+            for (int i = 0; i < 2; ++i) {
+                if (!a.f32_x[i]) {
+                    if (i == 0 || a.f32_c[i]) return WD_EINVAL;
+                    continue;
+                }
+                if (a.f32_c[i] <= 0 || a.f32_c[i] % 64 || a.f32_ld[i] < a.f32_c[i] || (a.f32_ld[i] & 3) ||
+                    (reinterpret_cast<uintptr_t>(a.f32_x[i]) & 15) || rows * a.f32_ld[i] * 4 >= 0x7FFFFFF0L)
+                    return WD_EINVAL;
+                cs += a.f32_c[i];
+            }
+            if (cs != a.src[1].c) return WD_EINVAL;
+        }
         if (a.tile == 64080) {
             if (!wd_gemmq_applies(a)) return WD_EINVAL;
             if (a.gn_gamma && (40 % a.gn_cpg || 80 % a.gn_cpg)) return WD_EINVAL;
@@ -2166,6 +2189,7 @@
         if (a.ksplit == 0) a.ksplit = a.ws ? wd_auto_ksplit(a.tile, a.m, a.n, nk64, a.ws_floats) : 1;
         if (a.ksplit > 1 && (nk64 < a.ksplit || (long)a.ksplit * a.m * a.n > a.ws_floats)) a.ksplit = 1;
         if (a.gn_gamma && a.ksplit <= 1) return WD_EINVAL;
+        if (f32 && a.ksplit > 1) return WD_EINVAL;
         r.a = a, r.kernel = K_GEMMW;
         return WD_OK;
     }
diff --git a/worddiffusion_amd/csrc/wd_gemmq.hip b/worddiffusion_amd/csrc/wd_gemmq.hip
--- a/worddiffusion_amd/csrc/wd_gemmq.hip
+++ b/worddiffusion_amd/csrc/wd_gemmq.hip
@@ -100,7 +100,7 @@
     bf16x8 xb[5][2], yb[5][2];
     bool first_pass = true;
 
-    auto run_source = [&](const wd_src& q, const bool conv, const int kbase) {
+    auto run_source = [&](const wd_src& q, const bool conv, const int kbase, const bool f32) {
         const int cpt = q.c >> 6;
         const int slr = conv ? NR * SW : QBM;
         const int cpl = slr * 128, chb = 2 * cpl;
@@ -165,7 +165,46 @@
                 }
             }
             const int nitems = nch * ntok * 8;
-            for (int i0 = 0; i0 < nitems; i0 += 8 * QNT) {
+            if (f32) {
+                static_assert(QNT == 8 * QBM, "one (token, piece) per thread and chunk");
+                const int tq = tid >> 3, pc = tid & 7;
+                const int ca = a.f32_c[0];
+                const int p = m0 - bsm * a.hw_out + tq;
+                const int r0 = a.f32_perm[0] ? a.f32_perm[0][p] : p, r1 = a.f32_perm[1] ? a.f32_perm[1][p] : p;
+                const uint32_t vo0 = (uint32_t)(bsm * a.hw_out + r0) * (uint32_t)(a.f32_ld[0] * 4) + (uint32_t)(pc * 32);
+                const uint32_t vo1 = (uint32_t)(bsm * a.hw_out + r1) * (uint32_t)(a.f32_ld[1] * 4) + (uint32_t)(pc * 32);
+                const __amdgpu_buffer_rsrc_t srd_m0 = make_srd(a.f32_x[0]), srd_m1 = make_srd(a.f32_x[1] ? a.f32_x[1] : a.f32_x[0]);
+                const int dst0 = q_lds_off(tq, pc);
+                for (int c0 = 0; c0 < nch; c0 += 8) {
+                    q_u32x4 v[2][8];
+#pragma unroll
+                    for (int k = 0; k < 8; ++k) {
+                        const int cb = (c_lo + c0 + k) * 64;
+                        const bool live = c0 + k < nch;
+                        const bool second = cb >= ca;
+                        const uint32_t so = live ? (uint32_t)((second ? cb - ca : cb) * 4) : 0u;
+                        const uint32_t vo = live ? (second ? vo1 : vo0) : Q_OOB;
+                        if (second) {
+                            v[0][k] = __builtin_amdgcn_raw_buffer_load_b128(srd_m1, vo, so, 0);
+                            v[1][k] = __builtin_amdgcn_raw_buffer_load_b128(srd_m1, vo + 16, so, 0);
+                        } else {
+                            v[0][k] = __builtin_amdgcn_raw_buffer_load_b128(srd_m0, vo, so, 0);
+                            v[1][k] = __builtin_amdgcn_raw_buffer_load_b128(srd_m0, vo + 16, so, 0);
+                        }
+                    }
+#pragma unroll
+                    for (int k = 0; k < 8; ++k)
+                        if (c0 + k < nch) {
+                            uint2 h0, l0, h1, l1;
+                            wd_split4(__builtin_bit_cast(float4, v[0][k]), h0, l0);
+                            wd_split4(__builtin_bit_cast(float4, v[1][k]), h1, l1);
+                            char* d = smem + (c0 + k) * chb + dst0;
+                            *reinterpret_cast<q_u32x4*>(d) = q_u32x4{h0.x, h0.y, h1.x, h1.y};
+                            *reinterpret_cast<q_u32x4*>(d + cpl) = q_u32x4{l0.x, l0.y, l1.x, l1.y};
+                        }
+                }
+            }
+            for (int i0 = 0; i0 < (f32 ? 0 : nitems); i0 += 8 * QNT) {
                 q_u32x4 v[2][8];
                 int dst[8];
 #pragma unroll
@@ -217,8 +256,8 @@
         }
     };
     const bool conv0 = a.src[0].ntaps == 9;
-    run_source(a.src[0], conv0, 0);
-    if (a.nsrc > 1) run_source(a.src[1], false, 2 * a.src[0].ntaps * (a.src[0].c >> 6));
+    run_source(a.src[0], conv0, 0, false);
+    if (a.nsrc > 1) run_source(a.src[1], false, 2 * a.src[0].ntaps * (a.src[0].c >> 6), a.f32_x[0] != nullptr);
 
     Q_STAMP(4);
     __syncthreads();
@@ -278,6 +317,10 @@
         return false;
     for (int s = 0; s < a.nsrc; ++s) {
         const wd_src& q = a.src[s];
+        if (s == 1 && a.f32_x[0]) {
+            if (q.c % 64 || q.ntaps != 1 || q.gather) return false;
+            continue;
+        }
         if (!q.hi || !q.lo || q.c % 64 || (q.ld & 7)) return false;
         const bool conv = s == 0 && q.ntaps == 9 && q.gather && a.hw_out == 64 &&
                           (((W == 16 || W == 32) && q.hw_src == 64) || (W == 16 && q.hw_src == 256));
diff --git a/worddiffusion_amd/csrc/wd_gemmw.hip b/worddiffusion_amd/csrc/wd_gemmw.hip
--- a/worddiffusion_amd/csrc/wd_gemmw.hip
+++ b/worddiffusion_amd/csrc/wd_gemmw.hip
@@ -9,7 +9,7 @@
 
 __device__ __forceinline__ int w_lds_off(int row, int ch) { return row * 128 + ((ch ^ ((row >> 1) & 7)) << 4); }
 
-template <int NPASS, int RH, bool A32>
+template <int NPASS, int RH, bool A32, bool S32>
 __global__ void __launch_bounds__(WNT, 1) wd_gemmw_kernel(const wd_gemm_args a, const int nbn, const int nbm) {
 #if defined(__HIP_DEVICE_COMPILE__)
     constexpr int NPL = (NPASS == 1) ? 1 : 2;
@@ -68,6 +68,18 @@
             }
             s_tab[idx] = v;
         }
+        if constexpr (S32) {
+            for (int idx = tid; idx < 2 * BM; idx += WNT) {
+                const int i = idx / BM, row = idx - i * BM;
+                const int m = m0 + row;
+                int v = -1;
+                if (m < a.m) {
+                    const int b = m / a.hw_out, p = m - b * a.hw_out;
+                    v = a.f32_perm[i] ? b * a.hw_out + a.f32_perm[i][p] : m;
+                }
+                s_tab[9 * BM + idx] = v;
+            }
+        }
     }
     float* s_aff = reinterpret_cast<float*>(s_tab + 9 * BM);
     if constexpr (A32) {
@@ -134,10 +146,16 @@
         cur_cpt = a.src[1].c >> 6;
         left = cur_cpt - kc;
     }
+    const int cptm = S32 ? a.f32_c[0] >> 6 : 0;
+    if (S32 && s == 1) {
+        tap = kc >= cptm ? 10 : 9;
+        cur_ld = a.f32_ld[kc >= cptm ? 1 : 0];
+    }
     const __amdgpu_buffer_rsrc_t srd0_hi = make_srd(A32 ? reinterpret_cast<const wd_bf16*>(a.a32) : a.src[0].hi),
                                  srd0_lo = make_srd(A32 ? reinterpret_cast<const wd_bf16*>(a.a32) : (a.src[0].lo ? a.src[0].lo : a.src[0].hi));
-    const wd_bf16* p1h = a.nsrc > 1 ? a.src[1].hi : a.src[0].hi;
-    const wd_bf16* p1l = a.nsrc > 1 ? (a.src[1].lo ? a.src[1].lo : a.src[1].hi) : p1h;
+    const wd_bf16* p1h = S32 ? reinterpret_cast<const wd_bf16*>(a.f32_x[0]) : a.nsrc > 1 ? a.src[1].hi : a.src[0].hi;
+    const wd_bf16* p1l = S32 ? reinterpret_cast<const wd_bf16*>(a.f32_x[1] ? a.f32_x[1] : a.f32_x[0])
+                             : a.nsrc > 1 ? (a.src[1].lo ? a.src[1].lo : a.src[1].hi) : p1h;
     const __amdgpu_buffer_rsrc_t srd1_hi = make_srd(p1h), srd1_lo = make_srd(p1l);
     uint32_t a_voff[RH];
     auto locate = [&]() {
@@ -147,9 +165,10 @@
         for (int j = 0; j < RH; ++j) {
             const int row = wave * 8 + (ln >> 3) + 64 * j;
             int r;
-            if (s == 0) r = s_tab[tap * BM + row];
+            if (s == 0 || S32) r = s_tab[tap * BM + row];
             else r = (m0 + row < a.m) ? m0 + row : -1;
-            if (A32 && s == 0) a_voff[j] = r >= 0 ? (uint32_t)r * (uint32_t)(a.a32_ld * 4) + (uint32_t)(ach * 32) : WD_OOB;
+            if (S32 && s == 1) a_voff[j] = r >= 0 ? (uint32_t)r * (uint32_t)(cur_ld * 4) + (uint32_t)(ach * 32) : WD_OOB;
+            else if (A32 && s == 0) a_voff[j] = r >= 0 ? (uint32_t)r * (uint32_t)(a.a32_ld * 4) + (uint32_t)(ach * 32) : WD_OOB;
             else a_voff[j] = r >= 0 ? (uint32_t)r * (uint32_t)(cur_ld * 2) + (uint32_t)(ach * 16) : WD_OOB;
         }
     };
@@ -167,13 +186,21 @@
         }
         if (sw1) {
             s = 1;
-            tap = 0;
+            tap = S32 ? 9 : 0;
             kc = 0;
-            cur_ld = a.src[1].ld;
+            cur_ld = S32 ? a.f32_ld[0] : a.src[1].ld;
             cur_cpt = a.src[1].c >> 6;
             left = cur_cpt;
             relocate = true;
         }
+        if constexpr (S32) {
+            if (s == 1 && kc == cptm && left > 0) {
+                tap = 10;
+                cur_ld = a.f32_ld[1];
+                relocate = true;
+            }
+            if (tap > 10) tap = 10;
+        }
         if (relocate) locate();
     };
     int kb = 0;
@@ -181,13 +208,26 @@
     w_u32x4 ra[RH][NPL];
     int ra_ch = 0;
     bool ra_ok[RH];
+    bool ra_f32 = false;
     auto load_a = [&](const bool live) {
         if (A32) ra_ch = (s == 0) ? kc * 64 + ach * 8 : -1;
+        if (S32) ra_f32 = s == 1;
 #pragma unroll
         for (int j = 0; j < RH; ++j) {
             const uint32_t vo = live ? a_voff[j] : WD_OOB;
             if (A32) ra_ok[j] = vo != WD_OOB;
-            if (A32 && s == 0) {
+            if (S32 && s == 1) {
+                static_assert(!S32 || NPL == 2, "the fp32 source path holds eight floats in the two plane registers");
+                const bool fm = kc >= cptm;
+                const int so = (kc - (fm ? cptm : 0)) * 256;
+                if (fm) {
+                    ra[j][0] = __builtin_amdgcn_raw_buffer_load_b128(srd1_lo, vo, so, 0);
+                    ra[j][NPL - 1] = __builtin_amdgcn_raw_buffer_load_b128(srd1_lo, vo + 16, so, 0);
+                } else {
+                    ra[j][0] = __builtin_amdgcn_raw_buffer_load_b128(srd1_hi, vo, so, 0);
+                    ra[j][NPL - 1] = __builtin_amdgcn_raw_buffer_load_b128(srd1_hi, vo + 16, so, 0);
+                }
+            } else if (A32 && s == 0) {
                 static_assert(!A32 || NPL == 2, "the fp32 source path holds eight floats in the two plane registers");
                 ra[j][0] = __builtin_amdgcn_raw_buffer_load_b128(srd0_hi, vo, kc * 256, 0);
                 ra[j][NPL - 1] = __builtin_amdgcn_raw_buffer_load_b128(srd0_hi, vo + 16, kc * 256, 0);
@@ -219,6 +259,15 @@
                 uint2 h0, l0, h1, l1;
                 wd_split4(y0, h0, l0);
                 wd_split4(y1, h1, l1);
+                *reinterpret_cast<w_u32x4*>(base + j * 8192 + a_dst) = w_u32x4{h0.x, h0.y, h1.x, h1.y};
+                *reinterpret_cast<w_u32x4*>(base + (NPL - 1) * A_PL + j * 8192 + a_dst) = w_u32x4{l0.x, l0.y, l1.x, l1.y};
+            }
+        } else if (S32 && ra_f32) {
+#pragma unroll
+            for (int j = 0; j < RH; ++j) {
+                uint2 h0, l0, h1, l1;
+                wd_split4(__builtin_bit_cast(float4, ra[j][0]), h0, l0);
+                wd_split4(__builtin_bit_cast(float4, ra[j][NPL - 1]), h1, l1);
                 *reinterpret_cast<w_u32x4*>(base + j * 8192 + a_dst) = w_u32x4{h0.x, h0.y, h1.x, h1.y};
                 *reinterpret_cast<w_u32x4*>(base + (NPL - 1) * A_PL + j * 8192 + a_dst) = w_u32x4{l0.x, l0.y, l1.x, l1.y};
             }
@@ -404,16 +453,17 @@
     if (lo) reinterpret_cast<uint4*>(out_lo)[i] = *reinterpret_cast<const uint4*>(lo + src);
 }
 
-template <int NPASS, int RH, bool A32 = false>
+template <int NPASS, int RH, bool A32 = false, bool S32 = false>
 int launchw(const wd_gemm_args& a, hipStream_t st) {
     constexpr int NPL = (NPASS == 1) ? 1 : 2;
     constexpr int BM = 64 * RH, BN = 320 / RH;
-    constexpr int loop_smem = 2 * NPL * BM * 128 + 9 * BM * 4 + (A32 ? 2 * 1024 * 4 : 0);
+    static_assert(!(A32 && S32), "the scale / shift table and the maps' row tables share the space behind s_tab");
+    constexpr int loop_smem = 2 * NPL * BM * 128 + 9 * BM * 4 + (A32 ? 2 * 1024 * 4 : 0) + (S32 ? 2 * BM * 4 : 0);
     constexpr int red_smem = BM * (BN + 4) * 4 + WD_STAT_SCRATCH;
     constexpr int smem = loop_smem > red_smem ? loop_smem : red_smem;
     static bool attr_done = false;
     if (!attr_done) {
-        if (hipFuncSetAttribute(reinterpret_cast<const void*>(&wd_gemmw_kernel<NPASS, RH, A32>), hipFuncAttributeMaxDynamicSharedMemorySize,
+        if (hipFuncSetAttribute(reinterpret_cast<const void*>(&wd_gemmw_kernel<NPASS, RH, A32, S32>), hipFuncAttributeMaxDynamicSharedMemorySize,
                                 smem) != hipSuccess)
             return WD_ELAUNCH;
         attr_done = true;
@@ -421,7 +471,7 @@
     const int nbn = a.n / BN, nbm = (a.m + BM - 1) / BM;
     {
         WdLaunchScope scope(WD_CLS_GEMM_WDIRECT, st, 2.0 * (double)a.m * (double)a.n * (double)a.ktot);
-        hipLaunchKernelGGL((wd_gemmw_kernel<NPASS, RH, A32>), dim3(nbn * nbm * a.ksplit), dim3(WNT), smem, st, a, nbn, nbm);
+        hipLaunchKernelGGL((wd_gemmw_kernel<NPASS, RH, A32, S32>), dim3(nbn * nbm * a.ksplit), dim3(WNT), smem, st, a, nbn, nbm);
     }
     if (a.ksplit > 1) return wd_gemm_launch_reduce(a, st, BM);
     return wd_check_launch();
@@ -431,6 +481,7 @@
 
 int wd_gemmw_launch(const wd_gemm_args& a, hipStream_t st) {
     if (a.a32) return launchw<3, 1, true>(a, st);
+    if (a.f32_x[0]) return launchw<3, 1, false, true>(a, st);
     if (a.tile == 128160) return a.npass == 3 ? launchw<3, 2>(a, st) : launchw<1, 2>(a, st);
     return a.npass == 3 ? launchw<3, 1>(a, st) : launchw<1, 1>(a, st);
 }
diff --git a/worddiffusion_amd/engine.py b/worddiffusion_amd/engine.py
--- a/worddiffusion_amd/engine.py
+++ b/worddiffusion_amd/engine.py
@@ -325,6 +325,7 @@
         self.fuse_gn2 = os.environ.get("WDIFF_FUSE_GN2", "1") != "0"
         self.fuse_gn = os.environ.get("WDIFF_FUSE_GN", "1") != "0"
         self.fuse_split = os.environ.get("WDIFF_FUSE_SPLIT", "1") != "0"
+        self.skip_f32 = os.environ.get("WDIFF_SKIP_F32", "1") != "0"
         self._plans: Dict[tuple, Plan] = {}
         self._tabs: Dict[tuple, torch.Tensor] = {}
         self._tab_np: Dict[int, np.ndarray] = {}
@@ -572,7 +573,7 @@
 
     def _gemm(self, ops, what, srcs, wname, m, hw_out, bias=None, rowvec=None, rowvec_ld=0, resid=None,
               resid_ld=0, resid_rows=None, act=N.ACT_NONE, out_f32=None, out_ld=0, out_pl=None, n=None, tile=0,
-              w_row_off=0, want_stats=False, a32=None, ln=None, w_groups=None):
+              w_row_off=0, want_stats=False, a32=None, ln=None, w_groups=None, skip32=None):
         a = N.WdGemmArgs()
         for i, s in enumerate(srcs):
             a.src[i] = s
@@ -596,6 +597,8 @@
             self._set_a32(a, *a32)
         if w_groups is not None:
             a.w_ngroups, a.w_group_stride = w_groups
+        if skip32 is not None:
+            self._set_f32(a, skip32)
         a.tile = tile
         if self._ws is None:
             self._ws = torch.empty(128 * 128 * 160 * 8, dtype=torch.float32, device=self.device)
@@ -615,6 +618,8 @@
         smallmap = (frag and not wdirect and self.use_smallmap and hw_out == 64 and 128 <= (m // 64) * (nrows // 80) <= 512 and
                     self._legal(a, w_layout=3, tile=64080, slab_rows=width))
         assert (a32 is None and w_groups is None) or wdirect, what
+        if skip32 is not None and not (wdirect or smallmap):
+            raise N.NativeError(f"{what}: no kernel takes the fp32 skip source that _skip_f32_ok promised")
         if wdirect or smallmap:
             wf = self._wfrag(wname)
             a.w_hi, a.w_lo = wf[0].data_ptr(), wf[1].data_ptr()
@@ -676,6 +681,29 @@
         a.a32_gamma, a.a32_beta = self._w[gname + ".g"].data_ptr(), self._w[gname + ".b"].data_ptr()
         a.a32_eps, a.a32_silu = float(eps), int(silu)
 
+    @staticmethod
+    def _set_f32(a, maps: List["Act"]):
+        for i, x in enumerate(maps):
+            a.f32_x[i], a.f32_ld[i], a.f32_c[i] = x.t.data_ptr(), x.c, x.c
+            a.f32_perm[i] = x.perm.data_ptr() if x.perm is not None else None
+
+    def _skip_f32_ok(self, srcs: List["Act"], cout, M, hw, gather, width) -> bool:
+        if not self.skip_f32 or self.npass != 3 or self.use_slab or self.use_conv3 or self.fuse_gn_in >= 2 or len(srcs) > 2:
+            return False
+        a = N.WdGemmArgs()
+        a.src[0] = self._src32(Act(None, cout, 0, 0), 9, gather, hw)
+        a.src[0].hi = a.src[0].lo = 16
+        a.src[1] = self._src32(Act(None, sum(s.c for s in srcs), 0, 0))
+        a.nsrc, a.npass, a.m, a.n, a.ktot, a.hw_out = 2, self.npass, M, cout, 9 * cout + a.src[1].c, hw
+        a.w_hi = a.w_lo = a.out_f32 = a.ws = 16
+        a.out_ld, a.ws_floats = cout, 128 * 128 * 160 * 8
+        self._set_f32(a, srcs)
+        if self.use_wdirect and wdirect_fills_chip(M, cout):
+            return self._legal(a, apply=False, w_layout=3, tile=64320, slab_rows=width)
+        if self.use_smallmap and hw == 64 and 128 <= (M // 64) * (cout // 80) <= 512:
+            return self._legal(a, apply=False, w_layout=3, tile=64080, slab_rows=width)
+        return False
+
     def _wdirect_ok(self, srcs, m, n, hw_out, a32=None, **fields) -> bool:
         a = N.WdGemmArgs()
         for i, s in enumerate(srcs):
@@ -701,7 +729,7 @@
         a.tickets, a.ntickets = tk.data_ptr() + 4 * P._ticket_off, ntick
         P._ticket_off += ntick
 
-    def _gn(self, P, ops, what, srcs: List[Act], gname, eps, silu, want_raw=False, dropout=None):
+    def _gn(self, P, ops, what, srcs: List[Act], gname, eps, silu, want_raw=False, dropout=None, own_launch=False):
         B = self._B
         h, w = srcs[0].h, srcs[0].w
         hw = h * w
@@ -735,7 +763,7 @@
                 ops.append((self.lib.wd_gn_fold_chunks, (part.data_ptr(), B, nchunk, ngs, folded.data_ptr()), what + ":fold chunks"))
                 part, nchunk = folded, 1
                 s.stats = (part, nchunk, pc)
-            if has_perm or dropout is not None or not self._gn_in_combine(s, raw, gam, bet, eps, silu, cpg, pl, coff):
+            if has_perm or dropout is not None or own_launch or not self._gn_in_combine(s, raw, gam, bet, eps, silu, cpg, pl, coff):
                 todo.append((s, part, nchunk, pc, coff))
             coff += s.c
         hi, lo = self._hilo(pl)
@@ -818,11 +846,14 @@
         tab, _, _ = self._table(h, w, "same")
         need_raw = cin != cout
         h1 = self._f32(P, M, cout)
+        skip32 = None
         if self._gn_in_consumer(P, ops, name + ".gn1", srcs, need_raw, M, hw, cout, taps=9, gather=tab):
             s1, in1 = self._src32(srcs[0], 9, tab, hw), (srcs[0], name + ".gn1", 1e-5, True)
             raw = None
         else:
-            a1, raw = self._gn(P, ops, name + ".gn1", srcs, name + ".gn1", 1e-5, True, want_raw=need_raw)
+            skip32 = srcs if need_raw and self._skip_f32_ok(srcs, cout, M, hw, tab, self._same_w.get(tab.data_ptr(), 0)) else None
+            a1, raw = self._gn(P, ops, name + ".gn1", srcs, name + ".gn1", 1e-5, True, want_raw=need_raw and skip32 is None,
+                               own_launch=skip32 is not None)
             s1, in1 = self._src(a1, cin, 9, tab, hw), None
         g1 = self._gemm(ops, name + ".conv1", [s1], name + ".c1.w", M, hw,
                         bias=self._w[name + ".c1.b"], rowvec=self._film.data_ptr() + 4 * self.film_off[name],
@@ -835,9 +866,9 @@
             s2, in2 = self._src(a2, cout, 9, tab, hw), None
         out = self._f32(P, M, cout)
         if need_raw:
-            g2 = self._gemm(ops, name + ".conv2+skip", [s2, self._src(raw, cin)],
+            g2 = self._gemm(ops, name + ".conv2+skip", [s2, self._src(raw, cin) if skip32 is None else self._src32(Act(None, cin, h, w))],
                             name + ".c2.w", M, hw, bias=self._w[name + ".c2.b"], out_f32=out, out_ld=cout,
-                            want_stats=True, a32=in2)
+                            want_stats=True, a32=in2, skip32=skip32)
         else:
             g2 = self._gemm(ops, name + ".conv2", [s2], name + ".c2.w", M, hw,
                             bias=self._w[name + ".c2.b"], resid=srcs[0].t.data_ptr(), resid_ld=cout, out_f32=out,
```

Measured after the change: 35.32 images/s, median of 6. About the same (+0.4%).
